# smolGura/fish-tts

Measured on AMD Instinct MI355X. Metric: semantic tokens/sec, higher is better.
Workload: dtype bf16; 1 GPU; openaudio-s1-mini shapes (BASELINE configs[1]): batch=1 per GPU, 48-token prompt, 215 frames (10 s), top-p sampling, hipGraph-captured frame step, + DAC codec decode; prompt_len=48, parallelism=replica x1, frame_engine=3

## Files before the change

### fish-tts_amd/csrc/engine.hip

```cpp
#include "engine.h"
#include "ar_kernels.h"
#include "frame_engine.h"
#include "wide_kernels.h"
#include "gemm_kernels.h"
#include "codec_kernels.h"
#include "stage_kernels.h"

#include <math.h>

#include <algorithm>
#include <mutex>
#include <stdarg.h>
#include <stdio.h>
#include <stdlib.h>
#include <string.h>

using namespace ft;

static std::string g_create_err;
static void eng_release(ft_ctx* ctx);

ft_status ft_fail(ft_ctx* ctx, ft_status code, const std::string& msg) {
    if (ctx) ctx->err = msg; else g_create_err = msg;
    return code;
// ... 134 lines not shown
    FT_TRY(dmalloc(ctx, &ctx->part_o, M * c.n_head * ctx->nsplit_max * c.head_dim));
    FT_TRY(dmalloc(ctx, &ctx->part_ml, M * c.n_head * ctx->nsplit_max * 2));
    ctx->cache_m_stride = (size_t)c.n_local_heads * ctx->n_slots * c.head_dim;
    ctx->fcache_m_stride = (size_t)c.fast_n_local_heads * c.num_codebooks * c.fast_head_dim;
    ctx->layers.resize(c.n_layer);
    ctx->flayers.resize(c.n_fast_layer);
    for (auto& l : ctx->layers) {
        FT_TRY(dmalloc(ctx, (char**)&l.kc, M * ctx->cache_m_stride * ctx->esz));
        FT_TRY(dmalloc(ctx, (char**)&l.vc, M * ctx->cache_m_stride * ctx->esz));
    }
    for (auto& l : ctx->flayers) {
        FT_TRY(dmalloc(ctx, (char**)&l.kc, M * ctx->fcache_m_stride * ctx->esz));
        FT_TRY(dmalloc(ctx, (char**)&l.vc, M * ctx->fcache_m_stride * ctx->esz));
    }
    const size_t R = c.num_codebooks + 1;
    FT_TRY(dmalloc(ctx, &ctx->d_pos, M));
    FT_TRY(dmalloc(ctx, &ctx->d_tok, M * R));
    FT_TRY(dmalloc(ctx, &ctx->d_tokn, M * R));
    FT_TRY(dmalloc(ctx, &ctx->d_seq, M * R * ctx->cap));
    FT_TRY(dmalloc(ctx, &ctx->d_nf, M));
    FT_TRY(dmalloc(ctx, &ctx->d_done, M));
    FT_TRY(dmalloc(ctx, &ctx->d_prompt, R * (size_t)c.max_seq_len));
    FT_TRY(dmalloc(ctx, &ctx->d_ctl, M));
    ctx->prefill_gemm_mode = getenv("FT_PREFILL_GEMM") ? atoi(getenv("FT_PREFILL_GEMM")) : 2;
    ctx->prefill_v0 = getenv("FT_PREFILL_V0") != nullptr || c.dtype != FT_BF16 || c.dim % 32 || (c.n_head * c.head_dim) % 32 ||
                      c.intermediate_size % 32;
    if (!ctx->prefill_v0) {
        const size_t S = c.max_seq_len;
        FT_TRY(dmalloc(ctx, &ctx->pf_x, S * c.dim));
        FT_TRY(dmalloc(ctx, &ctx->pf_qkv, S * qkvN));
        FT_TRY(dmalloc(ctx, &ctx->pf_y, S * c.n_head * c.head_dim));
        FT_TRY(dmalloc(ctx, &ctx->pf_xn, S * c.dim));
        FT_TRY(dmalloc(ctx, &ctx->pf_ybf, S * c.n_head * c.head_dim));
        FT_TRY(dmalloc(ctx, &ctx->pf_g, S * c.intermediate_size));
        FT_TRY(dmalloc(ctx, &ctx->pf_qbf, S * c.n_head * c.head_dim));
        FT_TRY(dmalloc(ctx, &ctx->pf_seqs, M));
        FT_TRY(dmalloc(ctx, &ctx->pf_rows, S));
    }
    if (c.dtype == FT_F16 || !ctx->prefill_v0) {
        const int HD = c.n_head * c.head_dim, HDf = c.fast_n_head * c.fast_head_dim;
        ctx->wide_ok = !getenv("FT_NO_WIDE") && !c.fast_attention_qkv_bias && !c.fast_attention_o_bias && c.fast_dim == c.dim &&
                       wide_k_ok(c.dim) && wide_k_ok(HD) && wide_k_ok(c.intermediate_size) && wide_k_ok(HDf) && wide_k_ok(c.fast_intermediate_size) &&
                       qkvN % 32 == 0 && fqkvN % 32 == 0 && c.intermediate_size % 16 == 0 && c.fast_intermediate_size % 16 == 0 &&
                       c.dim % 16 == 0 && c.vocab_size % 32 == 0 && ctx->fastV % 16 == 0;
        if (ctx->wide_ok) {
            ctx->xo_pair = (int)((M + 15) / 16 * 16);
            ctx->no_pair = getenv("FT_NO_PAIR") != nullptr;
            ctx->no_attn_wide = getenv("FT_NO_ATTN_WIDE") != nullptr;
            ctx->no_head_stream = getenv("FT_NO_HEAD_STREAM") != nullptr;
            ctx->xo_ldm = 2 * ctx->xo_pair;
            const size_t P = ctx->xo_ldm;
            FT_TRY(dmalloc(ctx, &ctx->xo_x, P * c.dim));
            FT_TRY(dmalloc(ctx, &ctx->xo_xf, P * c.fast_dim));
            FT_TRY(dmalloc(ctx, &ctx->xo_femb, P * c.fast_dim));
            FT_TRY(dmalloc(ctx, &ctx->xo_y, P * (size_t)std::max(HD, HDf)));
            FT_TRY(dmalloc(ctx, &ctx->xo_g, P * (size_t)std::max(c.intermediate_size, c.fast_intermediate_size)));
        }
    }
    const size_t nchunk = ((size_t)c.vocab_size + 1023) / 1024;
    FT_TRY(dmalloc(ctx, &ctx->samp_cut, M));
    FT_TRY(dmalloc(ctx, &ctx->samp_chunk_cnt, M * nchunk));
    FT_TRY(dmalloc(ctx, &ctx->samp_part_score, M * nchunk));
    FT_TRY(dmalloc(ctx, &ctx->samp_part_idx, M * nchunk));
    FT_HIP(ctx, hipHostMalloc((void**)&ctx->h_pin, (3 * M + 8) * sizeof(int), hipHostMallocDefault));
    return FT_OK;
}

extern "C" ft_status ft_create(const ft_ar_config* ar, const ft_codec_config* codec, int32_t device, ft_ctx** out) {
    if (!out || (!ar && !codec)) return ft_fail(nullptr, FT_ERR_ARG, "ft_create: need a config and an out pointer");
    int ndev = 0;
    if (hipGetDeviceCount(&ndev) != hipSuccess || ndev == 0)
        return ft_fail(nullptr, FT_ERR_HIP, "ft_create: no HIP device visible (the MI355X path has no CPU fallback)");
    if (device < 0 || device >= ndev) return ft_fail(nullptr, FT_ERR_ARG, "ft_create: bad device index");
    ft_ctx* ctx = new ft_ctx();
    ctx->device = device;
    ft_status st = FT_OK;
    do {
        if (hipSetDevice(device) != hipSuccess) { st = ft_fail(ctx, FT_ERR_HIP, "hipSetDevice failed"); break; }
        if (hipStreamCreateWithFlags(&ctx->stream, hipStreamNonBlocking) != hipSuccess) {
            st = ft_fail(ctx, FT_ERR_HIP, "hipStreamCreate failed"); break;
        }
        if (ar) {
            ctx->c = *ar;
            ctx->has_ar = true;
            if ((st = ar_validate(ctx)) != FT_OK) break;
            if ((st = ar_alloc(ctx)) != FT_OK) break;
            ar_expected(ctx);
        }
        if (codec) {
            ctx->cc = *codec;
            ctx->has_codec = true;
            if ((st = codec_create(ctx)) != FT_OK) break;
            codec_expected(ctx);
        }
    } while (0);
    if (st != FT_OK) {
        g_create_err = ctx->err;
        ft_destroy(ctx);
        return st;
    }
    *out = ctx;
    return FT_OK;
}

extern "C" void ft_destroy(ft_ctx* ctx) {
    if (!ctx) return;
    hipSetDevice(ctx->device);
    if (ctx->stream) hipStreamSynchronize(ctx->stream);
    for (auto& kv : ctx->graphs) hipGraphExecDestroy(kv.second);
    for (auto& kv : ctx->expected) if (kv.second.p) hipFree(kv.second.p);
    for (auto& l : ctx->layers) { hipFree(l.kc); hipFree(l.vc); if (l.w13) hipFree(l.w13); }
    for (auto& l : ctx->flayers) { hipFree(l.kc); hipFree(l.vc); if (l.w13) hipFree(l.w13); }
    float* bufs[] = {ctx->x, ctx->qkv, ctx->y, ctx->g, ctx->logits, ctx->femb, ctx->xf, ctx->qkvf, ctx->gf,
                     ctx->flog, ctx->part_o, ctx->part_ml, ctx->noise};
    for (float* b : bufs) if (b) hipFree(b);
    if (ctx->hid && ctx->hid != ctx->x) hipFree(ctx->hid);
    int* ibufs[] = {ctx->d_pos, ctx->d_tok, ctx->d_tokn, ctx->d_seq, ctx->d_nf, ctx->d_done, ctx->d_prompt};
    for (int* b : ibufs) if (b) hipFree(b);
    if (ctx->d_ctl) hipFree(ctx->d_ctl);
    if (ctx->wide_qkv0_tab) hipFree(ctx->wide_qkv0_tab);
    { void* pf[] = {ctx->pf_x, ctx->pf_qkv, ctx->pf_y, ctx->pf_xn, ctx->pf_ybf, ctx->pf_g, ctx->xo_x, ctx->xo_xf, ctx->xo_femb, ctx->xo_y, ctx->xo_g, ctx->pf_qbf}; for (void* q : pf) if (q) hipFree(q); }
    for (auto& l : ctx->layers) { if (l.bqkv_f32) hipFree(l.bqkv_f32); if (l.bo_f32) hipFree(l.bo_f32); }
    if (ctx->samp_cut) hipFree(ctx->samp_cut);
    if (ctx->samp_chunk_cnt) hipFree(ctx->samp_chunk_cnt);
    if (ctx->samp_part_score) hipFree(ctx->samp_part_score);
    if (ctx->samp_part_idx) hipFree(ctx->samp_part_idx);
    eng_release(ctx);
    if (ctx->h_pin) hipHostFree(ctx->h_pin);
    for (auto e : ctx->prof_ev) hipEventDestroy(e);
    codec_destroy(ctx);
    if (ctx->stream) hipStreamDestroy(ctx->stream);
    delete ctx;
}

extern "C" const char* ft_last_error(const ft_ctx* ctx) { return ctx ? ctx->err.c_str() : g_create_err.c_str(); }

extern "C" ft_status ft_sync(ft_ctx* ctx) {
    if (!ctx) return FT_ERR_ARG;
    FT_HIP(ctx, hipSetDevice(ctx->device));
    FT_HIP(ctx, hipStreamSynchronize(ctx->stream));
    return FT_OK;
}

extern "C" ft_status ft_load_weight(ft_ctx* ctx, const char* name, const void* src, int32_t src_dtype,
                                    const int64_t* shape, int32_t ndim) {
    if (!ctx || !name || !src || !shape) return ft_fail(ctx, FT_ERR_ARG, "ft_load_weight: null argument");
    if (ctx->finalized) return ft_fail(ctx, FT_ERR_STATE, "ft_load_weight: weights already finalized");
    auto it = ctx->expected.find(name);
    if (it == ctx->expected.end()) return ft_fail(ctx, FT_ERR_ARG, std::string("unknown weight name: ") + name);
    FtTensor& t = it->second;
    if ((int)t.shape.size() != ndim) return ft_fail(ctx, FT_ERR_ARG, std::string("rank mismatch for ") + name);
    for (int i = 0; i < ndim; ++i)
        if (t.shape[i] != shape[i]) {
            char buf[256];
            snprintf(buf, sizeof buf, "shape mismatch for %s: dim %d is %lld, expected %lld", name, i,
                     (long long)shape[i], (long long)t.shape[i]);
            return ft_fail(ctx, FT_ERR_ARG, buf);
        }
    if (src_dtype != FT_F32 && src_dtype != FT_BF16 && src_dtype != FT_F16)
        return ft_fail(ctx, FT_ERR_ARG, "src_dtype must be FT_F32, FT_BF16 or FT_F16");
    FT_HIP(ctx, hipSetDevice(ctx->device));
    const int64_t n = t.numel();
    const size_t ssz = src_dtype == FT_F32 ? 4 : 2, dsz = t.dtype == FT_F32 ? 4 : 2;
    if (!t.p) FT_HIP(ctx, hipMalloc(&t.p, (size_t)n * dsz + 64));
    if (src_dtype == t.dtype) {
        FT_HIP(ctx, hipMemcpy(t.p, src, (size_t)n * dsz, hipMemcpyDefault));
        return FT_OK;
    }
    void* stage = nullptr;
    FT_HIP(ctx, hipMalloc(&stage, (size_t)n * ssz));
    hipError_t e = hipMemcpy(stage, src, (size_t)n * ssz, hipMemcpyDefault);
    if (e == hipSuccess) {
        const int blocks = (int)((n + 255) / 256 < 4096 ? (n + 255) / 256 : 4096);
        auto to = [&](auto* sp) {
            if (t.dtype == FT_F32) convert_kernel<<<blocks, 256, 0, ctx->stream>>>(sp, (float*)t.p, n);
            else if (t.dtype == FT_BF16) convert_kernel<<<blocks, 256, 0, ctx->stream>>>(sp, (bf16_t*)t.p, n);
            else convert_kernel<<<blocks, 256, 0, ctx->stream>>>(sp, (f16_t*)t.p, n);
        };
        if (src_dtype == FT_F32) to((const float*)stage);
        else if (src_dtype == FT_BF16) to((const bf16_t*)stage);
        else to((const f16_t*)stage);
        e = hipStreamSynchronize(ctx->stream);
    }
    hipFree(stage);
    if (e != hipSuccess) return ft_fail(ctx, FT_ERR_HIP, std::string("ft_load_weight copy: ") + hipGetErrorString(e));
    return FT_OK;
}

static void* wp(ft_ctx* ctx, const std::string& n) {
    auto it = ctx->expected.find(n);
    return it == ctx->expected.end() ? nullptr : it->second.p;
}

static ft_status eng_setup(ft_ctx* ctx);
static ft_status wide_qkv0_build(ft_ctx* ctx);

static ft_status ar_finalize(ft_ctx* ctx) {
    const ft_ar_config& c = ctx->c;
    ctx->emb = wp(ctx, "embeddings.weight");
    ctx->cb_emb = wp(ctx, "codebook_embeddings.weight");
    ctx->norm = wp(ctx, "norm.weight");
    ctx->head = c.tie_word_embeddings ? ctx->emb : wp(ctx, "output.weight");
    ctx->fproj_w = wp(ctx, "fast_project_in.weight");
    ctx->fproj_b = wp(ctx, "fast_project_in.bias");
    ctx->fast_emb = wp(ctx, "fast_embeddings.weight");
    ctx->fast_norm = wp(ctx, "fast_norm.weight");
    ctx->fast_out = wp(ctx, "fast_output.weight");
    ctx->rope = (float*)wp(ctx, "rope.slow");
    ctx->frope = (float*)wp(ctx, "rope.fast");
    auto fill = [&](std::vector<FtLayer>& ls, const char* pre, int ffn, int dim) -> ft_status {
        for (size_t i = 0; i < ls.size(); ++i) {
            const std::string p = std::string(pre) + std::to_string(i);
            FtLayer& l = ls[i];
            l.attn_norm = wp(ctx, p + ".attention_norm.weight");
            l.wqkv = wp(ctx, p + ".attention.wqkv.weight");
            l.bqkv = wp(ctx, p + ".attention.wqkv.bias");
            l.qn = wp(ctx, p + ".attention.q_norm.weight");
            l.kn = wp(ctx, p + ".attention.k_norm.weight");
            l.wo = wp(ctx, p + ".attention.wo.weight");
            l.bo = wp(ctx, p + ".attention.wo.bias");
            l.ffn_norm = wp(ctx, p + ".ffn_norm.weight");
            l.w2 = wp(ctx, p + ".feed_forward.w2.weight");
            FtTensor& w1 = ctx->expected[p + ".feed_forward.w1.weight"];
            FtTensor& w3 = ctx->expected[p + ".feed_forward.w3.weight"];
            FT_HIP(ctx, hipMalloc(&l.w13, (size_t)2 * ffn * dim * ctx->esz));
            const int64_t n = (int64_t)ffn * dim;
            const int blocks = (int)((n + 255) / 256 < 4096 ? (n + 255) / 256 : 4096);
            if (ctx->esz == 2)
                interleave_rows_kernel<bf16_t><<<blocks, 256, 0, ctx->stream>>>((bf16_t*)w1.p, (bf16_t*)w3.p, (bf16_t*)l.w13, ffn, dim);
            else
                interleave_rows_kernel<float><<<blocks, 256, 0, ctx->stream>>>((float*)w1.p, (float*)w3.p, (float*)l.w13, ffn, dim);
            FT_HIP(ctx, hipStreamSynchronize(ctx->stream));
            hipFree(w1.p); w1.p = nullptr;
            hipFree(w3.p); w3.p = nullptr;
        }
        return FT_OK;
    };
    FT_TRY(fill(ctx->layers, "layers.", c.intermediate_size, c.dim));
    if (!ctx->prefill_v0 || ctx->wide_ok) {
        const int qkvN = (c.n_head + 2 * c.n_local_heads) * c.head_dim;
        auto to_f32 = [&](const void* b, float* o, int n) {
            if (c.dtype == FT_F16) convert_kernel<f16_t, float><<<(n + 255) / 256, 256, 0, ctx->stream>>>((const f16_t*)b, o, n);
            else convert_kernel<bf16_t, float><<<(n + 255) / 256, 256, 0, ctx->stream>>>((const bf16_t*)b, o, n);
        };
        for (auto& l : ctx->layers) {
            if (l.bqkv) {
                FT_HIP(ctx, hipMalloc((void**)&l.bqkv_f32, qkvN * sizeof(float)));
                to_f32(l.bqkv, l.bqkv_f32, qkvN);
            }
            if (l.bo) {
                FT_HIP(ctx, hipMalloc((void**)&l.bo_f32, c.dim * sizeof(float)));
                to_f32(l.bo, l.bo_f32, c.dim);
            }
        }
        FT_HIP(ctx, hipStreamSynchronize(ctx->stream));
    }
    FT_TRY(fill(ctx->flayers, "fast_layers.", c.fast_intermediate_size, c.fast_dim));
    FT_TRY(eng_setup(ctx));
    FT_TRY(wide_qkv0_build(ctx));
    return FT_OK;
}

constexpr int ENG_MAX_STRIKES = 2;
static std::mutex g_eng_mu;
static std::map<int, ft_ctx*> g_eng_owner;

static void eng_release(ft_ctx* ctx) {
    void* eb[] = {ctx->eng_layers, ctx->eng_flayers, ctx->eng_gx ,
                  ctx->eng_gpart, ctx->eng_fast_g, ctx->eng_ctl, ctx->eng_qkv0_tab};
    for (void* q : eb) if (q) hipFree(q);
    ctx->eng_layers = ctx->eng_flayers = nullptr;
    ctx->eng_gx = ctx->eng_gqkv = ctx->eng_gy = ctx->eng_gxb = ctx->eng_gg = ctx->eng_fast_g = ctx->eng_ctl = nullptr;
    ctx->eng_gpart = nullptr;
    ctx->eng_qkv0_tab = nullptr;
    ctx->eng_on = ctx->eng_fast_on = false;
    if (ctx->eng_owner) {
        std::lock_guard<std::mutex> lk(g_eng_mu);
        auto it = g_eng_owner.find(ctx->device);
        if (it != g_eng_owner.end() && it->second == ctx) g_eng_owner.erase(it);
        ctx->eng_owner = false;
    }
}

static bool eng_fits_cu(const void* fn, size_t lds, size_t lds_cap, const char* name, std::string& why) {
    hipFuncAttributes fa{};
    const hipError_t fe = hipFuncGetAttributes(&fa, fn);
    if (fe != hipSuccess) { (void)hipGetLastError(); why = std::string("hipFuncGetAttributes: ") + hipGetErrorString(fe); return false; }
    const int regs = std::max(fa.numRegs, 1), per_simd = 512 / (((regs + 7) / 8) * 8);
    const bool fits = per_simd * 4 >= ENG_THREADS / 64 && lds + fa.sharedSizeBytes <= lds_cap && fa.maxThreadsPerBlock >= ENG_THREADS;
    if (getenv("FT_LOG")) {
        int occ = -1;
        const hipError_t oe = hipOccupancyMaxActiveBlocksPerMultiprocessor(&occ, fn, ENG_THREADS, lds);
        if (oe != hipSuccess) (void)hipGetLastError();
        fprintf(stderr, "fish_tts_amd: %s engine kernel: %d registers (%d waves per SIMD), %zu B of LDS of %zu: %s (the occupancy query says %d)\n",
                name, fa.numRegs, per_simd, lds + fa.sharedSizeBytes, lds_cap, fits ? "fits a CU" : "does not fit a CU", occ);
    }
    if (!fits) why = std::string("a ") + name + " workgroup does not fit one CU (registers / LDS)";
    return fits;
}

typedef void (*eng_slow_fn_t)(SlowEngP);
typedef void (*eng_fast_fn_t)(FastEngP);
typedef void (*eng_qkv0_fn_t)(const bf16_t*, const bf16_t*, const bf16_t*, const bf16_t*, bf16_t*, int, int, int, float);
struct EngSlowEntry { int D, H, HKV, HDIM, F, SQ, SF, SO; eng_slow_fn_t xl, plain; };
struct EngFastEntry { int D, H, HKV, HDIM, F, V, SQ, SF, SO; eng_fast_fn_t loop; eng_qkv0_fn_t qkv0; eng_fast_fn_t resident; int resf, resl; };
template <typename S, bool WITH_XL>
static EngSlowEntry eng_slow_entry() {
    eng_slow_fn_t xl = nullptr;
    if constexpr (WITH_XL) xl = slow_engine_kernel<S, true>;
    return EngSlowEntry{S::D, S::H, S::HKV, S::HDIM, S::F, S::SQ, S::SF, S::SO, xl, slow_engine_kernel<S, false>};
}
template <typename S>
static EngFastEntry eng_fast_entry() {
    eng_fast_fn_t res = nullptr;
    if constexpr (S::RESF > 0) res = fast_engine_kernel<S, 10, true>;
    return EngFastEntry{S::D, S::H, S::HKV, S::HDIM, S::F, S::V, S::SQ, S::SF, S::SO, fast_engine_kernel<S, 10, false>, eng_qkv0_table_kernel<S>,
                        res, S::RESF, S::RESL};
}
static const EngSlowEntry* eng_slow_shapes(int* n) {
    static const EngSlowEntry tab[] = {eng_slow_entry<EngSlowS1, true>(), eng_slow_entry<EngSlowShape<1024, 16, 8, 128, 4096>, true>(),
                                       eng_slow_entry<EngSlowShape<1024, 16, 4, 128, 3072>, false>()};
    *n = (int)(sizeof tab / sizeof tab[0]);
    return tab;
}
static const EngFastEntry* eng_fast_shapes(int* n) {
    static const EngFastEntry tab[] = {eng_fast_entry<EngFastS1>(), eng_fast_entry<EngFastShape<1024, 16, 8, 64, 4096, 1024>>()};
    *n = (int)(sizeof tab / sizeof tab[0]);
    return tab;
}

static bool eng_setup_try(ft_ctx* ctx, std::string& why) {
    const ft_ar_config& c = ctx->c;
    auto hip_ok = [&](hipError_t e, const char* what) {
        if (e == hipSuccess) return true;
        why = std::string(what) + ": " + hipGetErrorString(e);
        (void)hipGetLastError();
        return false;
    };
    if (getenv("FT_NO_ENGINE")) { why = "FT_NO_ENGINE is set"; return false; }
    if (c.dtype != FT_BF16) { why = "precision is not bf16"; return false; }
    hipDeviceProp_t prop;
    if (!hip_ok(hipGetDeviceProperties(&prop, ctx->device), "hipGetDeviceProperties")) return false;
    const int nb = prop.multiProcessorCount;
    const int HD = c.n_head * c.head_dim;
    const int qkvN = (c.n_head + 2 * c.n_local_heads) * c.head_dim;
    auto per = [&](int units) { return (units + nb - 1) / nb; };
    const EngSlowEntry* se = nullptr;
    {
        int n = 0;
        const EngSlowEntry* tab = eng_slow_shapes(&n);
        for (int i = 0; i < n && !se; ++i)
            if (c.dim == tab[i].D && c.n_head == tab[i].H && c.n_local_heads == tab[i].HKV && c.head_dim == tab[i].HDIM && c.intermediate_size == tab[i].F)
                se = &tab[i];
    }
    const bool shape_ok = se && c.fast_dim == c.dim && c.n_layer >= 1 && c.n_layer < ENG_EPOCH_STEP &&
                          per(qkvN) <= se->SQ * ENG_CW && per(c.dim) <= se->SO * ENG_CW && per(c.intermediate_size) <= se->SF * ENG_CW &&
                          qkvN % (4 * nb) == 0 && c.dim % (4 * nb) == 0 && c.intermediate_size % (4 * nb) == 0 && per(qkvN) <= ENG_LINE &&
                          per(c.intermediate_size) <= ENG_LINE && c.n_local_heads * ctx->nsplit_max <= nb && c.head_dim % (4 * ctx->nsplit_max) == 0 && nb == ENG_NB;
    if (!shape_ok) {
        char buf[320];
        snprintf(buf, sizeof buf, "widths outside the engine's instantiations (dim %d, heads %d / %d x %d, ffn %d, fast_dim %d on %d CUs; "
                 "built for dim 1024, 16 heads x 128 with 8 kv heads and ffn 3072 or 4096, or 4 kv heads and ffn 3072, on 256 CUs)", c.dim, c.n_head,
                 c.n_local_heads, c.head_dim, c.intermediate_size, c.fast_dim, nb);
        why = buf;
        return false;
    }
    {
        std::lock_guard<std::mutex> lk(g_eng_mu);
        auto it = g_eng_owner.find(ctx->device);
        if (it != g_eng_owner.end() && it->second != ctx) {
            why = "another context of this process already runs the frame engine on this device (its workgroups need every CU)";
            return false;
        }
        g_eng_owner[ctx->device] = ctx;
        ctx->eng_owner = true;
    }
    ctx->eng_nb = nb;
    std::vector<EngLayer> h(c.n_layer);
    for (int i = 0; i < c.n_layer; ++i) {
        const FtLayer& l = ctx->layers[i];
        h[i] = EngLayer{(const bf16_t*)l.wqkv, (const bf16_t*)l.bqkv, (const bf16_t*)l.attn_norm, (const bf16_t*)l.qn,
                        (const bf16_t*)l.kn, (const bf16_t*)l.wo, (const bf16_t*)l.bo, (const bf16_t*)l.ffn_norm,
                        (const bf16_t*)l.w13, (const bf16_t*)l.w2, (bf16_t*)l.kc, (bf16_t*)l.vc};
    }
    if (!hip_ok(hipMalloc((void**)&ctx->eng_layers, h.size() * sizeof(EngLayer)), "hipMalloc(engine layer table)")) return false;
    if (!hip_ok(hipMemcpy(ctx->eng_layers, h.data(), h.size() * sizeof(EngLayer), hipMemcpyHostToDevice), "hipMemcpy(engine layer table)")) return false;
    auto zalloc = [&](void** q, size_t bytes, const char* what) {
        return hip_ok(hipMalloc(q, bytes), what) && hip_ok(hipMemset(*q, 0, bytes), what);
    };
    const size_t L = c.n_layer;
    const size_t VB = (size_t)nb * ENG_LINE * 4;
    const size_t pool_words = ((L + 1) * VB + 3 * L * VB + L * HD * 4) / 4;
    ctx->eng_relay = getenv("FT_NO_RELAY") == nullptr;
    ctx->eng_pool_bytes = pool_words * 4 * (ctx->eng_relay ? 9 : 1);
    if (!zalloc((void**)&ctx->eng_gx, ctx->eng_pool_bytes, "hipMalloc(engine hand-off pool)")) return false;
    ctx->eng_pool_words = pool_words;
    ctx->eng_gxb = ctx->eng_gx + (L + 1) * (VB / 4);
    ctx->eng_gg = ctx->eng_gxb + L * (VB / 4);
    ctx->eng_gy = ctx->eng_gg + L * (VB / 4);
    ctx->eng_gqkv = ctx->eng_gy + L * HD;
    ctx->eng_gpart_bytes = L * c.n_head * ctx->nsplit_max * (size_t)(c.head_dim + 2) * 8;
    if (!zalloc((void**)&ctx->eng_gpart, ctx->eng_gpart_bytes, "hipMalloc(engine split partials)")) return false;
    if (!zalloc((void**)&ctx->eng_ctl, ENG_CTL_WORDS * 4, "hipMalloc(engine control words)")) return false;
    const int G = c.n_head / c.n_local_heads, hd = c.head_dim, NSLOT = 4 * (64 / (hd >> 3));
    size_t fl = (size_t)c.dim * 2 + HD + c.intermediate_size + (size_t)(G + 2) * hd + (size_t)G * hd + 2 * hd +
                (size_t)NSLOT * G * 2 + (size_t)NSLOT * G * hd + 64 * 6 + ENG_MAX_OUT + 8;
    ctx->eng_lds_slow = std::max(fl * sizeof(float), (size_t)82 * 1024);
    const size_t lds_cap = prop.maxSharedMemoryPerMultiProcessor;
    if (ctx->eng_lds_slow > lds_cap) { why = "the slow stack's LDS need exceeds the CU's"; return false; }
    ctx->eng_xl = ctx->xl_shape && nb == 256 && ctx->nsplit_max == 32 && c.n_local_heads * 32 == nb;
    ctx->eng_xl = ctx->eng_xl && se->xl != nullptr;
    ctx->eng_slow_fn = (const void*)(ctx->eng_xl ? se->xl : se->plain);
    const void* slow_fn = ctx->eng_slow_fn;
    if (!hip_ok(hipFuncSetAttribute(slow_fn, hipFuncAttributeMaxDynamicSharedMemorySize, (int)ctx->eng_lds_slow),
                "hipFuncSetAttribute(slow_engine_kernel)")) return false;
    if (!eng_fits_cu(slow_fn, ctx->eng_lds_slow, lds_cap, "slow-stack", why)) return false;
    ctx->eng_on = true;
    why = ctx->eng_xl ? "slow stack on the frame engine (one kv head per XCD)" : "slow stack on the frame engine";

    const int HDf = c.fast_n_head * c.fast_head_dim;
    const int fqkvN = (c.fast_n_head + 2 * c.fast_n_local_heads) * c.fast_head_dim;
    const EngFastEntry* fe = nullptr;
    {
        int n = 0;
        const EngFastEntry* tab = eng_fast_shapes(&n);
        for (int i = 0; i < n && !fe; ++i)
            if (c.fast_dim == tab[i].D && c.fast_n_head == tab[i].H && c.fast_n_local_heads == tab[i].HKV && c.fast_head_dim == tab[i].HDIM &&
                c.fast_intermediate_size == tab[i].F && ctx->fastV == tab[i].V)
                fe = &tab[i];
    }
    const bool fast_ok = !getenv("FT_NO_FAST_ENGINE") && fe && HDf == c.fast_dim && c.n_fast_layer >= 1 &&
                         c.num_codebooks >= 2 && c.num_codebooks <= 10 && fqkvN % (4 * nb) == 0 && ctx->fastV % (4 * nb) == 0 &&
                         per(fqkvN) <= fe->SQ * ENG_CW && per(c.fast_dim) <= fe->SO * ENG_CW && per(c.fast_intermediate_size) <= fe->SF * ENG_CW &&
                         per(ctx->fastV) <= fe->SO * ENG_CW && per(fqkvN) <= ENG_LINE && per(c.fast_intermediate_size) <= ENG_LINE && ctx->fastV <= 1024 &&
                         c.codebook_size <= 65536;
    if (!fast_ok) { why += "; fast loop on launches (FT_NO_FAST_ENGINE, or fast widths outside the instantiations: 1024 / 16 + 8 heads x 64 / ffn 3072 or 4096 / 1024 codes used, <= 10 codebooks)"; return true; }
    const bool fast_res = fe->resident != nullptr && c.n_fast_layer <= fe->resl && getenv("FT_NO_RESIDENT") == nullptr;
    ctx->eng_fast_fn = (const void*)(fast_res ? fe->resident : fe->loop);
    auto fast_off = [&](const std::string& w2) { why += "; fast loop on launches (" + w2 + ")"; return true; };
    std::vector<EngLayer> hf(c.n_fast_layer);
    for (int i = 0; i < c.n_fast_layer; ++i) {
        const FtLayer& l = ctx->flayers[i];
        hf[i] = EngLayer{(const bf16_t*)l.wqkv, (const bf16_t*)l.bqkv, (const bf16_t*)l.attn_norm, (const bf16_t*)l.qn,
                         (const bf16_t*)l.kn, (const bf16_t*)l.wo, (const bf16_t*)l.bo, (const bf16_t*)l.ffn_norm,
                         (const bf16_t*)l.w13, (const bf16_t*)l.w2, nullptr, nullptr};
    }
    std::string w2;
    auto hip_ok2 = [&](hipError_t e, const char* what) {
        if (e == hipSuccess) return true;
        w2 = std::string(what) + ": " + hipGetErrorString(e);
        (void)hipGetLastError();
        return false;
    };
    if (!hip_ok2(hipMalloc((void**)&ctx->eng_flayers, hf.size() * sizeof(EngLayer)), "hipMalloc(fast layer table)")) return fast_off(w2);
    if (!hip_ok2(hipMemcpy(ctx->eng_flayers, hf.data(), hf.size() * sizeof(EngLayer), hipMemcpyHostToDevice), "hipMemcpy(fast layer table)")) return fast_off(w2);
    const size_t nLf = c.n_fast_layer;
    ctx->eng_fast_words = (2 * ((nLf + 1) + 3 * nLf + 1)) * (VB / 4) + (size_t)c.num_codebooks * ENG_LINE;
    ctx->eng_fast_bytes = ctx->eng_fast_words * 4 * (ctx->eng_relay ? 9 : 1);
    if (!hip_ok2(hipMalloc((void**)&ctx->eng_fast_g, ctx->eng_fast_bytes), "hipMalloc(fast hand-off pool)") ||
        !hip_ok2(hipMemset(ctx->eng_fast_g, 0, ctx->eng_fast_bytes), "hipMemset(fast hand-off pool)")) return fast_off(w2);
    const int kvw = c.fast_n_local_heads * c.fast_head_dim;
    ctx->eng_pair = getenv("FT_NO_PAIR") == nullptr &&
                    eng_fast_lds_bytes(c.fast_dim, fqkvN, HDf, c.fast_intermediate_size, ctx->fastV, (int)nLf, c.num_codebooks, kvw, true) <= lds_cap;
    ctx->eng_lds_fast = eng_fast_lds_bytes(c.fast_dim, fqkvN, HDf, c.fast_intermediate_size, ctx->fastV, (int)nLf, c.num_codebooks, kvw, ctx->eng_pair);
    if (ctx->eng_lds_fast > lds_cap) return fast_off("the codebook loop's LDS need exceeds the CU's");
    ctx->eng_lds_fast = std::max(ctx->eng_lds_fast, (size_t)82 * 1024);
    if (!hip_ok2(hipFuncSetAttribute(ctx->eng_fast_fn, hipFuncAttributeMaxDynamicSharedMemorySize,
                                     (int)ctx->eng_lds_fast), "hipFuncSetAttribute(fast_engine_kernel)")) return fast_off(w2);
    if (!eng_fits_cu(ctx->eng_fast_fn, ctx->eng_lds_fast, lds_cap, "codebook-loop", w2)) return fast_off(w2);
    if (getenv("FT_NO_QKV0") == nullptr && c.num_codebooks > 2) {
        const size_t tb = (size_t)ctx->fastV * fqkvN * sizeof(bf16_t);
        if (!hip_ok2(hipMalloc((void**)&ctx->eng_qkv0_tab, tb), "hipMalloc(layer-0 q k v table)")) return fast_off(w2);
        const FtLayer& l0 = ctx->flayers[0];
        const size_t lds = ((size_t)c.fast_dim + ENG_MAX_OUT) * sizeof(float);
        fe->qkv0<<<dim3(fqkvN / (fe->SQ * ENG_CW), 16), ENG_CW * 64, lds, ctx->stream>>>(
            (const bf16_t*)l0.wqkv, (const bf16_t*)l0.bqkv, (const bf16_t*)l0.attn_norm, (const bf16_t*)ctx->fast_emb,
            (bf16_t*)ctx->eng_qkv0_tab, c.fast_dim, fqkvN, ctx->fastV, c.norm_eps);
        if (!hip_ok2(hipGetLastError(), "eng_qkv0_table_kernel") || !hip_ok2(hipStreamSynchronize(ctx->stream), "eng_qkv0_table_kernel")) {
            hipFree(ctx->eng_qkv0_tab); ctx->eng_qkv0_tab = nullptr;
            return fast_off(w2);
        }
    }
    ctx->eng_fast_on = true;
    why = ctx->eng_xl ? "slow stack (one kv head per XCD) and codebook loop on the frame engine" : "slow stack and codebook loop on the frame engine";
    {
        char buf[160];
        if (fast_res)
            snprintf(buf, sizeof buf, "; codebook loop: %d of %d W13 pairs per CU of %d layers resident in the gathering waves' registers",
                     fe->resf * ENG_GW, per(c.fast_intermediate_size), c.n_fast_layer);
        else
            snprintf(buf, sizeof buf, "; codebook loop: all weights streamed (%s)", fe->resident == nullptr ? "no resident set fits this shape class" :
                     c.n_fast_layer > fe->resl ? "more layers than the resident set holds" : "FT_NO_RESIDENT is set");
        why += buf;
    }
    return true;
}

static ft_status eng_setup(ft_ctx* ctx) {
    ctx->eng_on = ctx->eng_fast_on = false;
    std::string why;
    if (!eng_setup_try(ctx, why)) {
        eng_release(ctx);
        ctx->eng_why = "launch path: " + why;
    } else {
        char buf[64];
        snprintf(buf, sizeof buf, " (%d workgroups)", ctx->eng_nb);
        ctx->eng_why = why + buf;
    }
    if (getenv("FT_LOG")) fprintf(stderr, "fish_tts_amd: batch-1 decode frames: %s\n", ctx->eng_why.c_str());
    return FT_OK;
}

extern "C" ft_status ft_finalize_weights(ft_ctx* ctx) {
    if (!ctx) return FT_ERR_ARG;
    if (ctx->finalized) return FT_OK;
    FT_HIP(ctx, hipSetDevice(ctx->device));
    for (auto& kv : ctx->expected)
        if (!kv.second.p) return ft_fail(ctx, FT_ERR_MISSING_WEIGHT, "missing weight: " + kv.first);
    if (ctx->has_ar) FT_TRY(ar_finalize(ctx));
    if (ctx->has_codec) FT_TRY(codec_finalize(ctx));
    ctx->finalized = true;
    return FT_OK;
}

struct Launch {
    ft_ctx* ctx;
    hipStream_t s;
    int m0, M;
    int pos_off;
    hipError_t err = hipSuccess;
    bool gemv_only = false;
    bool tail_only = false;
    void chk() { hipError_t e = hipGetLastError(); if (e != hipSuccess && err == hipSuccess) err = e; }
};

template <typename W, int R> struct DType { typedef W WT; static constexpr int ROUND = R; };
template <typename F>
static auto by_dtype(const ft_ctx* ctx, F&& f) {
    if (ctx->c.dtype == FT_BF16) return f(DType<bf16_t, RND_BF16>{});
    if (ctx->c.dtype == FT_F16) return f(DType<f16_t, RND_F16>{});
    return f(DType<float, RND_NONE>{});
}

enum { TB_X = 0, TB_QKV, TB_Y, TB_G, TB_LOGITS, TB_HID, TB_FEMB, TB_XF, TB_QKVF, TB_GF, TB_FLOG, TB_PART_O, TB_PART_ML,
       TB_PF_X = 13, TB_PF_QKV, TB_PF_Y,
       TB_XO_X = 20, TB_XO_XF, TB_XO_FEMB, TB_XO_Y, TB_XO_G,
       TB_PF_XN = 25, TB_PF_YBF, TB_PF_QBF, TB_PF_G,
       TB_TOKN = 30, TB_TOK, TB_POS, TB_NF, TB_DONE, TB_SEQ, TB_CUT, TB_CHUNK_CNT, TB_PART_IDX,
       TB_PROMPT = 39, TB_PF_SEQS, TB_PF_ROWS };
static const void* tr_buf(const ft_ctx* ctx, int id, int* esz, int* rows, int* cols) {
    const ft_ar_config& c = ctx->c;
    const int MB = c.max_batch, R = c.num_codebooks + 1, ldm = ctx->xo_ldm;
    const int qkvN = (c.n_head + 2 * c.n_local_heads) * c.head_dim, fqkvN = (c.fast_n_head + 2 * c.fast_n_local_heads) * c.fast_head_dim;
    const int HD = c.n_head * c.head_dim, HDf = c.fast_n_head * c.fast_head_dim, nchunk = (c.vocab_size + 1023) / 1024;
    *esz = 4;
    auto f = [&](const void* p, int r, int k) { *rows = r; *cols = k; return p; };
    auto o = [&](const void* p, int width) { *esz = 2; *rows = width / 8; *cols = ldm * 8; return p; };
    switch (id) {
        case TB_X: return f(ctx->x, MB, c.dim);
        case TB_QKV: return f(ctx->qkv, MB, qkvN);
        case TB_Y: return f(ctx->y, MB, ctx->y_ld);
        case TB_G: return f(ctx->g, MB, c.intermediate_size);
        case TB_LOGITS: return f(ctx->logits, MB, c.vocab_size);
        case TB_HID: return f(ctx->hid, MB, c.fast_dim);
        case TB_FEMB: return f(ctx->femb, MB, c.fast_dim);
        case TB_XF: return f(ctx->xf, MB, c.fast_dim);
        case TB_QKVF: return f(ctx->qkvf, 2 * ((MB + 15) / 16 * 16), fqkvN);
        case TB_GF: return f(ctx->gf, MB, c.fast_intermediate_size);
        case TB_FLOG: return f(ctx->flog, MB, ctx->fastV);
        case TB_PART_O: return f(ctx->part_o, 1, MB * c.n_head * ctx->nsplit_max * c.head_dim);
        case TB_PART_ML: return f(ctx->part_ml, 1, MB * c.n_head * ctx->nsplit_max * 2);
        case TB_XO_X: return o(ctx->xo_x, c.dim);
        case TB_XO_XF: return o(ctx->xo_xf, c.fast_dim);
        case TB_XO_FEMB: return o(ctx->xo_femb, c.fast_dim);
        case TB_XO_Y: return o(ctx->xo_y, std::max(HD, HDf));
        case TB_XO_G: return o(ctx->xo_g, std::max(c.intermediate_size, c.fast_intermediate_size));
        case TB_TOKN: return f(ctx->d_tokn, MB, R);
        case TB_TOK: return f(ctx->d_tok, MB, R);
        case TB_POS: return f(ctx->d_pos, 1, MB);
        case TB_NF: return f(ctx->d_nf, 1, MB);
        case TB_DONE: return f(ctx->d_done, 1, MB);
        case TB_SEQ: return f(ctx->d_seq, MB, R * ctx->cap);
        case TB_CUT: return f(ctx->samp_cut, MB, (int)(sizeof(SampCut) / 4));
        case TB_CHUNK_CNT: return f(ctx->samp_chunk_cnt, 1, MB * nchunk);
        case TB_PART_IDX: return f(ctx->samp_part_idx, 1, MB * nchunk);
        case TB_PF_X: return f(ctx->pf_x, c.max_seq_len, c.dim);
        case TB_PF_QKV: return f(ctx->pf_qkv, c.max_seq_len, qkvN);
        case TB_PF_Y: return f(ctx->pf_y, c.max_seq_len, HD);
        case TB_PF_XN: *esz = 2; return f(ctx->pf_xn, c.max_seq_len, c.dim);
        case TB_PF_YBF: *esz = 2; return f(ctx->pf_ybf, c.max_seq_len, HD);
        case TB_PF_QBF: *esz = 2; return f(ctx->pf_qbf, c.max_seq_len, HD);
        case TB_PF_G: *esz = 2; return f(ctx->pf_g, c.max_seq_len, c.intermediate_size);
        case TB_PROMPT: return f(ctx->d_prompt, 1, R * c.max_seq_len);
        case TB_PF_SEQS: return f(ctx->pf_seqs, MB, 4);
        case TB_PF_ROWS: return f(ctx->pf_rows, c.max_seq_len, 2);
    }
    return nullptr;
}
struct TrCls { int a = -1, b = -1, c = -1, d = -1; };
static void tr_rec(Launch& L, const std::string& name, int rows, int cols, TrCls cls, std::initializer_list<int> bufs) {
    ft_ctx* ctx = L.ctx;
    ArTrace& t = *ctx->trace;
    const int idx = (int)t.recs.size();
    t.recs.emplace_back();
    ArTraceRec& r = t.recs.back();
    r.name = t.pass_prefix + (name == "embed" || name.compare(0, 5, "slow.") == 0 ? t.pos_prefix : std::string()) + name;
    r.m0 = L.m0; r.rows = rows; r.cols = cols; r.pos_off = L.pos_off;
    r.cls[0] = cls.a; r.cls[1] = cls.b; r.cls[2] = cls.c; r.cls[3] = cls.d;
    r.held = idx >= t.first && idx < t.first + t.count;
    std::vector<int> ids(bufs);
    ids.insert(ids.end(), t.uploaded.begin(), t.uploaded.end());
    t.uploaded.clear();
    for (int id : ids) {
        ArTraceBuf b;
        const void* p = tr_buf(ctx, id, &b.esz, &b.rows, &b.cols);
        if (!p) continue;
        b.id = id;
        if (r.held) {
            b.data.resize((size_t)b.rows * b.cols * b.esz);
            if (hipMemcpyAsync(b.data.data(), p, b.data.size(), hipMemcpyDeviceToHost, L.s) != hipSuccess) t.failed = true;
        }
        r.bufs.push_back(std::move(b));
    }
    if (r.held && hipStreamSynchronize(L.s) != hipSuccess) t.failed = true;
}
static std::string tr_name(const char* fmt, ...) {
    char buf[64];
    va_list ap;
    va_start(ap, fmt);
    vsnprintf(buf, sizeof buf, fmt, ap);
    va_end(ap);
    return buf;
}
struct TrName {
    const char* stack; int n; const char* op;
    std::string str() const { return stack ? tr_name("%s.%d.%s", stack, n, op) : std::string(op); }
};
struct RowBuf { float* p; int id; };
struct XoBuf { bf16_t* p; int id; };
static void tr_state(ft_ctx* ctx, int which) {
    ArTrace& t = *ctx->trace;
    ArTraceState& s = t.st[which];
    const size_t MB = ctx->c.max_batch, R = ctx->c.num_codebooks + 1;
    s.tok.resize(MB * R); s.pos.resize(MB); s.nf.resize(MB); s.done.resize(MB); s.seq.resize(MB * R * ctx->cap);
    bool ok = hipStreamSynchronize(ctx->stream) == hipSuccess;
    ok = ok && hipMemcpy(s.tok.data(), ctx->d_tok, s.tok.size() * 4, hipMemcpyDeviceToHost) == hipSuccess;
    ok = ok && hipMemcpy(s.pos.data(), ctx->d_pos, MB * 4, hipMemcpyDeviceToHost) == hipSuccess;
    ok = ok && hipMemcpy(s.nf.data(), ctx->d_nf, MB * 4, hipMemcpyDeviceToHost) == hipSuccess;
    ok = ok && hipMemcpy(s.done.data(), ctx->d_done, MB * 4, hipMemcpyDeviceToHost) == hipSuccess;
    ok = ok && hipMemcpy(s.seq.data(), ctx->d_seq, s.seq.size() * 4, hipMemcpyDeviceToHost) == hipSuccess;
    if (which == 0) {
        static const int ids[] = {TB_X, TB_QKV, TB_Y, TB_G, TB_LOGITS, TB_HID, TB_FEMB, TB_XF, TB_QKVF, TB_GF, TB_FLOG, TB_PART_O, TB_PART_ML,
                                  TB_XO_X, TB_XO_XF, TB_XO_FEMB, TB_XO_Y, TB_XO_G, TB_TOKN, TB_TOK, TB_POS, TB_NF, TB_DONE, TB_SEQ, TB_CUT,
                                  TB_CHUNK_CNT, TB_PART_IDX};
        static const int pf_ids[] = {TB_PF_X, TB_PF_QKV, TB_PF_Y, TB_PF_XN, TB_PF_YBF, TB_PF_QBF, TB_PF_G, TB_PROMPT, TB_PF_SEQS, TB_PF_ROWS};
        std::vector<int> all(std::begin(ids), std::end(ids));
        if (t.kind >= 3) all.insert(all.end(), std::begin(pf_ids), std::end(pf_ids));
        t.begin.clear();
        for (int id : all) {
            ArTraceBuf b;
            const void* p = tr_buf(ctx, id, &b.esz, &b.rows, &b.cols);
            if (!p) continue;
            b.id = id;
            b.data.resize((size_t)b.rows * b.cols * b.esz);
            ok = ok && hipMemcpy(b.data.data(), p, b.data.size(), hipMemcpyDeviceToHost) == hipSuccess;
            t.begin.push_back(std::move(b));
        }
    }
    if (!ok) t.failed = true;
}
struct ArTraceScope {
    ft_ctx* ctx;
    bool own = false;
    ArTraceScope(ft_ctx* c, bool eligible, int kind, int m0, int M) : ctx(c) {
        ArTrace& t = ctx->tstore;
        if (ctx->trace || !t.armed) return;
        t.armed = false;
        if (!eligible) return;
        t.recs.clear(); t.uploaded.clear(); t.pass_prefix.clear(); t.pos_prefix.clear();
        t.failed = false; t.kind = kind; t.m0 = m0; t.M = M;
        ctx->trace = &t;
        own = true;
    }
    ~ArTraceScope() { if (own) ctx->trace = nullptr; }
};
static void tr_uploaded(ft_ctx* ctx, std::initializer_list<int> ids) { if (ctx->trace) ctx->trace->uploaded.assign(ids); }
static void tr_pos(ft_ctx* ctx, int t) { if (ctx->trace) ctx->trace->pos_prefix = tr_name("t%d.", t); }

struct PfX {
    const void* gain = nullptr;
    const float* ss_in = nullptr;
    int nblk = 0;
    float* ss_out = nullptr;
};
enum { PF_ID_NONE = -1, PF_ID_SKINNY1 = 0, PF_ID_SKINNY2 = 1, PF_ID_SKINNY4 = 2, PF_ID_LIN128 = 3, PF_ID_LIN64 = 4, PF_ID_TAP64_128 = 5,
       PF_ID_TAP64_64 = 6, PF_ID_TAP_128 = 7, PF_ID_TAP_64 = 8 };
static int pf_gemm(Launch& L, const bf16_t* X, long ldx, int S, const void* W, const float* bias, int N, int K,
                   int act, const float* resid, float* out_f32, bf16_t* out_bf, long ldo, int round_out,
                   const PfX& fx = PfX());
static bool wide_batch(const Launch& L) {
    return L.ctx->wide_ok && L.M >= L.ctx->wide_min && L.M <= 64 && !L.gemv_only && !L.ctx->prof;
}

static bool wide_pair(const Launch& L) {
    const ft_ctx* ctx = L.ctx;
    return wide_batch(L) && !ctx->no_pair && ctx->c.num_codebooks >= 2 && ctx->c.n_fast_layer > 0 && ctx->xo_pair + L.M <= 64;
}

enum { WIDE_ID_S11 = 0, WIDE_ID_S12 = 1, WIDE_ID_S22 = 2, WIDE_ID_G12 = 3, WIDE_ID_G22 = 4, WIDE_ID_R11 = 5, WIDE_ID_HEAD = 6 };
template <typename WT>
static int wide_gemm(Launch& L, const bf16_t* X, const void* W, const float* bias, int N, int K, const void* gain, int epi,
                      float* out_f32, long ldo, bf16_t* out_xo, const bf16_t* resid_xo, int rows = 0, bool vocab_head = false) {
    const int M = rows > 0 ? rows : L.M;
    WidePT<WT> p{};
    p.X = (const WT*)X; p.ldm = L.ctx->xo_ldm; p.W = (const WT*)W; p.ldw = K; p.gain = (const WT*)gain; p.eps = L.ctx->c.norm_eps;
    p.bias = bias; p.M = M; p.N = N; p.K = K; p.out_f32 = out_f32; p.ldo = ldo; p.out_xo = (WT*)out_xo; p.ldm_o = L.ctx->xo_ldm;
    p.resid_xo = (const WT*)resid_xo;
    bool ok;
    int id;
    if (epi == WEPI_RESID) { id = WIDE_ID_R11; ok = wide_gemm_launch<1, 1, false, WEPI_RESID>(p, L.s); }
    else if (epi == WEPI_SWIGLU) {
        id = M > 16 ? WIDE_ID_G22 : WIDE_ID_G12;
        ok = M > 16 ? wide_gemm_launch<2, 2, true, WEPI_SWIGLU>(p, L.s) : wide_gemm_launch<1, 2, true, WEPI_SWIGLU>(p, L.s);
    }
    else if (vocab_head && M <= 32 && K == 1024 && N % 16 == 0 && N >= 4096 && !L.ctx->no_head_stream) {
        static DevOnce once;
        once.run([] { hipFuncSetAttribute((const void*)wide_head_kernel<1024, WT>, hipFuncAttributeMaxDynamicSharedMemorySize, (int)wide_head_lds<1024>()); });
        wide_head_kernel<1024, WT><<<256, 512, wide_head_lds<1024>(), L.s>>>(p);
        id = WIDE_ID_HEAD;
        ok = true;
    }
    else if (N >= 32768) {
        id = M > 16 ? WIDE_ID_S22 : WIDE_ID_S12;
        ok = M > 16 ? wide_gemm_launch<2, 2, true, WEPI_STORE>(p, L.s) : wide_gemm_launch<1, 2, true, WEPI_STORE>(p, L.s);
    }
    else if (N >= 4096 && M > 16) { id = WIDE_ID_S12; ok = wide_gemm_launch<1, 2, true, WEPI_STORE>(p, L.s); }
    else { id = WIDE_ID_S11; ok = wide_gemm_launch<1, 1, true, WEPI_STORE>(p, L.s); }
    if (!ok && L.err == hipSuccess) L.err = hipErrorInvalidValue;
    L.chk();
    return id;
}
template <typename WT>
static void wide_linear(Launch& L, const TrName& nm, const bf16_t* X, const void* W, const float* bias, const void* gain, int N, int K,
                        int epi, RowBuf out_f32, long ldo, XoBuf out_xo, const bf16_t* resid_xo, int rows = 0, bool vocab_head = false) {
    const int id = wide_gemm<WT>(L, X, W, bias, N, K, gain, epi, out_f32.p, ldo, out_xo.p, resid_xo, rows, vocab_head);
    if (L.ctx->trace) tr_rec(L, nm.str(), rows > 0 ? rows : L.M, epi == WEPI_SWIGLU ? N / 2 : N, TrCls{id}, {out_xo.p ? out_xo.id : out_f32.id});
}

template <typename WT>
static __global__ __launch_bounds__(256) void xo_from_rows_kernel(const float* x, int ldx, int D, bf16_t* xo, int ldm) {
    const int m = blockIdx.y;
    for (int d = blockIdx.x * 256 + threadIdx.x; d < D; d += gridDim.x * 256) xo[xo_index(m, d, ldm)] = h16_bits<WT>(x[(size_t)m * ldx + d]);
}

static __global__ __launch_bounds__(256) void xo_from_h16_rows_kernel(const bf16_t* x, int D, bf16_t* xo, int ldm, int rows) {
    const int m = blockIdx.y;
    if (m >= rows) return;
    for (int d = blockIdx.x * 256 + threadIdx.x; d < D; d += gridDim.x * 256) xo[xo_index(m, d, ldm)] = x[(size_t)m * D + d];
}
template <typename WT>
static __global__ void f32_to_h16_kernel(const float* x, bf16_t* o, long n) {
    for (long i = (long)blockIdx.x * blockDim.x + threadIdx.x; i < n; i += (long)gridDim.x * blockDim.x) o[i] = h16_bits<WT>(x[i]);
}

template <typename WT>
static ft_status wide_qkv0_build_t(ft_ctx* ctx) {
    const ft_ar_config& c = ctx->c;
    if (!ctx->wide_ok || getenv("FT_NO_QKV0") || c.num_codebooks <= 2 || c.n_fast_layer < 1) return FT_OK;
    const int Df = c.fast_dim, qkvN = (c.fast_n_head + 2 * c.fast_n_local_heads) * c.fast_head_dim, V = ctx->fastV;
    const FtLayer& l0 = ctx->flayers[0];
    if (l0.bqkv) return FT_OK;
    constexpr int CH = 64;
    bf16_t* xo = nullptr; float* out = nullptr;
    if (hipMalloc((void**)&xo, (size_t)Df * CH * sizeof(bf16_t)) != hipSuccess || hipMalloc((void**)&out, (size_t)CH * qkvN * sizeof(float)) != hipSuccess ||
        hipMalloc((void**)&ctx->wide_qkv0_tab, (size_t)V * qkvN * sizeof(bf16_t)) != hipSuccess) {
        (void)hipGetLastError();
        if (xo) hipFree(xo);
        if (out) hipFree(out);
        if (ctx->wide_qkv0_tab) { hipFree(ctx->wide_qkv0_tab); ctx->wide_qkv0_tab = nullptr; }
        return FT_OK;
    }
    bool ok = true;
    for (int c0 = 0; c0 < V && ok; c0 += CH) {
        const int rows = std::min(CH, V - c0);
        xo_from_h16_rows_kernel<<<dim3((Df + 255) / 256, rows), 256, 0, ctx->stream>>>((const bf16_t*)ctx->fast_emb + (size_t)c0 * Df, Df, xo, CH, rows);
        WidePT<WT> p{};
        p.X = (const WT*)xo; p.ldm = CH; p.W = (const WT*)l0.wqkv; p.ldw = Df; p.gain = (const WT*)l0.attn_norm; p.eps = c.norm_eps;
// ... 2444 lines not shown
```

### fish-tts_amd/csrc/frame_engine.h

```cpp
#pragma once
#include "ar_kernels.h"

namespace ft {

constexpr int ENG_NB = 256;
constexpr int ENG_WAVES = 8;
constexpr int ENG_THREADS = ENG_WAVES * 64;
constexpr int ENG_CW = 4;
constexpr int ENG_GW = 4;

template <int D_, int H_, int HKV_, int HDIM_, int F_>
struct EngSlowShape {
    static constexpr int D = D_, H = H_, HKV = HKV_, HDIM = HDIM_, F = F_;
    static constexpr int HD = H * HDIM, QKVN = (H + 2 * HKV) * HDIM, G = H / HKV;
    static constexpr int NTD = D / 512, NTA = HD / 512, NTF = F / 512;
    static constexpr int SQ = (QKVN / ENG_NB + ENG_CW - 1) / ENG_CW, SF = (F / ENG_NB + ENG_CW - 1) / ENG_CW, SO = (D / ENG_NB + ENG_CW - 1) / ENG_CW;
    static constexpr bool PK3 = F % 384 == 0 && (F / ENG_NB) % 3 == 0;
    static_assert(D % 512 == 0 && HD % 512 == 0 && F % 512 == 0, "weight rows are read as whole 16-byte pieces by 64 lanes");
    static_assert(QKVN % (4 * ENG_NB) == 0 && D % (4 * ENG_NB) == 0 && F % (4 * ENG_NB) == 0, "whole 16-byte granule groups per workgroup");
    static_assert(H % HKV == 0 && HDIM % 8 == 0 && HDIM <= 128, "grouped-query attention, 16-byte K/V pieces");
};
template <int D_, int H_, int HKV_, int HDIM_, int F_, int V_>
struct EngFastShape {
    static constexpr int D = D_, H = H_, HKV = HKV_, HDIM = HDIM_, F = F_, V = V_;
// ... 35 lines not shown
    bf16_t *kc, *vc;
};

__device__ __forceinline__ void eng_barrier() {
    __builtin_amdgcn_fence(__ATOMIC_RELEASE, "workgroup", "local");
    __builtin_amdgcn_s_barrier();
    __builtin_amdgcn_fence(__ATOMIC_ACQUIRE, "workgroup", "local");
}

typedef const __attribute__((address_space(1))) U4* eng_gU4;
template <bool NT> __device__ __forceinline__ U4 eng_ldg16(const void* p) {
    if constexpr (NT) return __builtin_nontemporal_load((eng_gU4)p);
    else return *(eng_gU4)p;
}
__device__ __forceinline__ float eng_ldg_bf16(const bf16_t* p, size_t i) {
    return bf16_bits_to_f32(((const __attribute__((address_space(1))) bf16_t*)p)[i]);
}
typedef const __attribute__((address_space(4))) unsigned long long* eng_c64;
__device__ __forceinline__ EngLayer eng_layer(const EngLayer* table, int i) {
    static_assert(sizeof(EngLayer) == 12 * sizeof(unsigned long long), "EngLayer is twelve pointers");
    eng_c64 q = (eng_c64)(unsigned long long)(table + i);
    EngLayer l;
    l.wqkv = (const bf16_t*)q[0]; l.bqkv = (const bf16_t*)q[1]; l.attn_norm = (const bf16_t*)q[2]; l.qn = (const bf16_t*)q[3];
    l.kn = (const bf16_t*)q[4]; l.wo = (const bf16_t*)q[5]; l.bo = (const bf16_t*)q[6]; l.ffn_norm = (const bf16_t*)q[7];
    l.w13 = (const bf16_t*)q[8]; l.w2 = (const bf16_t*)q[9]; l.kc = (bf16_t*)q[10]; l.vc = (bf16_t*)q[11];
    return l;
}

__device__ __forceinline__ unsigned eng_tag16(unsigned e) { return (e & 0x7fffu) | 0x8000u; }
__device__ __forceinline__ unsigned eng_tag32(unsigned e) { return e | 0x80000000u; }
__device__ __forceinline__ unsigned long long eng_rt() { return __builtin_amdgcn_s_memrealtime(); }

__device__ __forceinline__ void eng_put(unsigned* g, int i, float v, unsigned tag16) {
    __hip_atomic_store((eng_gu32*)(g + i), (tag16 << 16) | (__float_as_uint(v) >> 16), ENG_RLX);
}
__device__ __forceinline__ void eng_put_raw(unsigned* g, int i, unsigned v16, unsigned tag16) {
    __hip_atomic_store((eng_gu32*)(g + i), (tag16 << 16) | (v16 & 0xffffu), ENG_RLX);
}
__device__ __forceinline__ void eng_put4(unsigned* g, float v0, float v1, float v2, float v3, unsigned tag16) {
    U4 w;
    w.x = (tag16 << 16) | (__float_as_uint(v0) >> 16); w.y = (tag16 << 16) | (__float_as_uint(v1) >> 16);
    w.z = (tag16 << 16) | (__float_as_uint(v2) >> 16); w.w = (tag16 << 16) | (__float_as_uint(v3) >> 16);
    asm volatile("global_store_dwordx4 %0, %1, off sc1" :: "v"(g), "v"(w) : "memory");
}
__device__ __forceinline__ void eng_put64(unsigned long long* g, size_t i, float v, unsigned tag32) {
    __hip_atomic_store((eng_gu64*)(g + i), ((unsigned long long)tag32 << 32) | __float_as_uint(v), ENG_RLX);
}

template <int FL = 0>
__device__ __forceinline__ void eng_ld3_sc1(const void* p0, const void* p1, const void* p2, U4& a, U4& b, U4& c) {
    asm volatile("global_load_dwordx4 %0, %3, off sc1\n\tglobal_load_dwordx4 %1, %4, off sc1\n\t"
                 "global_load_dwordx4 %2, %5, off sc1\n\ts_waitcnt vmcnt(0)"
                 : "=&v"(a), "=&v"(b), "=&v"(c) : "v"(p0), "v"(p1), "v"(p2) : "memory");
}
template <int FL = 0>
__device__ __forceinline__ void eng_ld1_sc1(const void* p0, U4& a) {
    asm volatile("global_load_dwordx4 %0, %1, off sc1\n\ts_waitcnt vmcnt(0)" : "=&v"(a) : "v"(p0) : "memory");
}

__device__ __forceinline__ bool eng_tags_ok(const U4& v, unsigned tag) {
    return (v.x >> 16) == tag && (v.y >> 16) == tag && (v.z >> 16) == tag && (v.w >> 16) == tag;
}
__device__ __forceinline__ void eng_unpack_to_lds(float* dst, const U4& v) {
    float4 f;
    f.x = __uint_as_float(v.x << 16); f.y = __uint_as_float(v.y << 16);
    f.z = __uint_as_float(v.z << 16); f.w = __uint_as_float(v.w << 16);
    *reinterpret_cast<float4*>(dst) = f;
}

struct EngSpin {
    unsigned* ctl;
    int* dead;
    unsigned spins = 0;
    unsigned long long t0 = 0;
    int where;
    __device__ __forceinline__ bool give_up(int lane) {
        if ((++spins & 255u) != 0u) return false;
        const unsigned long long t = eng_rt();
        if (t0 == 0) t0 = t;
        if (t - t0 > ENG_TIMEOUT_TICKS || __hip_atomic_load((eng_gu32*)(ctl + ENG_CTL_ABORT), ENG_RLX)) {
            if (lane == 0) {
                if (!__hip_atomic_load((eng_gu32*)(ctl + ENG_CTL_ABORT), ENG_RLX))
                    __hip_atomic_store((eng_gu32*)(ctl + ENG_CTL_WHERE), (unsigned)where, ENG_RLX);
                __hip_atomic_store((eng_gu32*)(ctl + ENG_CTL_ABORT), 1u, ENG_RLX);
                *dead = 1;
            }
            return true;
        }
        return false;
    }
};

constexpr int ENG_LINE = 32;
__device__ __forceinline__ size_t eng_pub(int b, int u_lo) { (void)b; return (size_t)u_lo; }
struct EngLayout {
    int per;
    __device__ __forceinline__ int off(int u) const { return u; }
};
struct EngIdent { __device__ __forceinline__ int operator()(int i) const { return i; } };

template <typename DMap = EngIdent, int FL = 0>
__device__ __forceinline__ void eng_gather(const unsigned* g, EngLayout lay, int u0, int n, unsigned tag, float* dst, int gw, int ngw,
                                           int lane, unsigned* ctl, int* dead, int where, DMap dmap = DMap(),
                                           unsigned long long* dbg = nullptr) {
    const int npiece = (n + 255) >> 8;
    EngSpin sp{ctl, dead, 0, 0, where};
    unsigned long long n_full = 0, t_first = 0;
    for (int p0 = gw; p0 < npiece; p0 += 3 * ngw) {
        const int c0 = p0;
        const int c1 = p0 + ngw < npiece ? p0 + ngw : c0;
        const int c2 = p0 + 2 * ngw < npiece ? p0 + 2 * ngw : c0;
        const int i0 = c0 * 256 + lane * 4 < n ? c0 * 256 + lane * 4 : c0 * 256;
        const int i1 = c1 * 256 + lane * 4 < n ? c1 * 256 + lane * 4 : c1 * 256;
        const int i2 = c2 * 256 + lane * 4 < n ? c2 * 256 + lane * 4 : c2 * 256;
        const int o0 = lay.off(u0 + i0), o1 = lay.off(u0 + i1), o2 = lay.off(u0 + i2);
        U4 a, b, c;
        for (;;) {
            if (c1 == c0) { eng_ld1_sc1<FL>(g + o0, a); b = a; c = a; }
            else eng_ld3_sc1<FL>(g + o0, g + o1, g + o2, a, b, c);
            const bool oa = eng_tags_ok(a, tag), ob = eng_tags_ok(b, tag), oc = eng_tags_ok(c, tag);
            if (dbg && n_full == 0) t_first = eng_rt();
            ++n_full;
            if (__all(oa && ob && oc)) break;
            if (sp.give_up(lane)) return;
        }
        if (c0 * 256 + lane * 4 < n) eng_unpack_to_lds(dst + dmap(i0), a);
        if (c1 != c0 && c1 * 256 + lane * 4 < n) eng_unpack_to_lds(dst + dmap(i1), b);
        if (c2 != c0 && c2 * 256 + lane * 4 < n) eng_unpack_to_lds(dst + dmap(i2), c);
    }
    if (dbg && lane == 0) { dbg[0] = t_first; dbg[1] = n_full; dbg[2] = 0; }
}

struct EngRelay {
    int on;
    int rank, nr;
    long delta;
};

__device__ __forceinline__ void eng_register(unsigned* ctl, int nb, int* r, int* dead) {
    const int xcd = (int)(__builtin_amdgcn_s_getreg(20 | (0 << 6) | (3 << 11)) & 7u);
    const unsigned rank = atomicAdd(ctl + ENG_CTL_XCD + xcd, 1u);
    atomicAdd(ctl + ENG_CTL_ARRIVED, 1u);
    EngSpin sp{ctl, dead, 0, 0, 9999};
    bool ok = true;
    while (__hip_atomic_load((eng_gu32*)(ctl + ENG_CTL_ARRIVED), ENG_RLX) < (unsigned)nb) {
        if (sp.give_up(0)) { ok = false; break; }
        __builtin_amdgcn_s_sleep(2);
    }
    r[0] = xcd; r[1] = (int)rank;
    r[2] = ok ? (int)__hip_atomic_load((eng_gu32*)(ctl + ENG_CTL_XCD + xcd), ENG_RLX) : 1;
}

template <typename DMap = EngIdent>
__device__ __forceinline__ void eng_gather_x(const EngRelay& rl, const unsigned* g, EngLayout lay, int u0, int n, unsigned tag, float* dst,
                                             int gw, int ngw, int lane, unsigned* ctl, int* dead, int where, DMap dmap = DMap(),
                                             unsigned long long* dbg = nullptr) {
    if (!rl.on) { eng_gather(g, lay, u0, n, tag, dst, gw, ngw, lane, ctl, dead, where, dmap, dbg); return; }
    unsigned* rep = const_cast<unsigned*>(g) + rl.delta;
    const int npiece = (n + 255) >> 8;
    for (int p = rl.rank; p < npiece; p += rl.nr) {
        if (p % ngw != gw) continue;
        const int i = p * 256 + lane * 4 < n ? p * 256 + lane * 4 : p * 256;
        const int o = lay.off(u0 + i);
        EngSpin sp{ctl, dead, 0, 0, where};
        U4 a;
        for (;;) {
            eng_ld1_sc1(g + o, a);
            if (__all(eng_tags_ok(a, tag))) break;
            if (sp.give_up(lane)) return;
        }
        if (p * 256 + lane * 4 < n) *reinterpret_cast<U4*>(rep + o) = a;
    }
    eng_gather<DMap, 1>(rep, lay, u0, n, tag, dst, gw, ngw, lane, ctl, dead, where, dmap, dbg);
}

__device__ __forceinline__ bool eng_tags3_ok(const U4& v, unsigned tag) { return (v.y >> 16) == tag && (v.w >> 16) == tag; }
__device__ __forceinline__ void eng_unpack3_to_lds(float* dst, const U4& v) {
    float2 a, b, c;
    a.x = __uint_as_float(v.x << 16); a.y = __uint_as_float(v.x & 0xffff0000u);
    b.x = __uint_as_float(v.y << 16); b.y = __uint_as_float(v.z << 16);
    c.x = __uint_as_float(v.z & 0xffff0000u); c.y = __uint_as_float(v.w << 16);
    reinterpret_cast<float2*>(dst)[0] = a; reinterpret_cast<float2*>(dst)[1] = b; reinterpret_cast<float2*>(dst)[2] = c;
}
template <int FL = 0>
__device__ __forceinline__ void eng_gather3(const unsigned* g, int n, unsigned tag, float* dst, int gw, int ngw, int lane, unsigned* ctl,
                                            int* dead, int where) {
    const int npiece = n / 384;
    EngSpin sp{ctl, dead, 0, 0, where};
    for (int p0 = gw; p0 < npiece; p0 += 3 * ngw) {
        const int c0 = p0;
        const int c1 = p0 + ngw < npiece ? p0 + ngw : c0;
        const int c2 = p0 + 2 * ngw < npiece ? p0 + 2 * ngw : c0;
        const unsigned* a0 = g + c0 * 256 + lane * 4;
        const unsigned* a1 = g + c1 * 256 + lane * 4;
        const unsigned* a2 = g + c2 * 256 + lane * 4;
        U4 a, b, c;
        for (;;) {
            if (c1 == c0) { eng_ld1_sc1<FL>(a0, a); b = a; c = a; }
            else eng_ld3_sc1<FL>(a0, a1, a2, a, b, c);
            if (__all(eng_tags3_ok(a, tag) && eng_tags3_ok(b, tag) && eng_tags3_ok(c, tag))) break;
            if (sp.give_up(lane)) return;
        }
        eng_unpack3_to_lds(dst + c0 * 384 + lane * 6, a);
        if (c1 != c0) eng_unpack3_to_lds(dst + c1 * 384 + lane * 6, b);
        if (c2 != c0) eng_unpack3_to_lds(dst + c2 * 384 + lane * 6, c);
    }
}
__device__ __forceinline__ void eng_gather3_x(const EngRelay& rl, const unsigned* g, int n, unsigned tag, float* dst, int gw, int ngw,
                                              int lane, unsigned* ctl, int* dead, int where) {
    if (!rl.on) { eng_gather3(g, n, tag, dst, gw, ngw, lane, ctl, dead, where); return; }
    unsigned* rep = const_cast<unsigned*>(g) + rl.delta;
    const int npiece = n / 384;
    for (int p = rl.rank; p < npiece; p += rl.nr) {
        if (p % ngw != gw) continue;
        const int o = p * 256 + lane * 4;
        EngSpin sp{ctl, dead, 0, 0, where};
        U4 a;
        for (;;) {
            eng_ld1_sc1(g + o, a);
            if (__all(eng_tags3_ok(a, tag))) break;
            if (sp.give_up(lane)) return;
        }
        *reinterpret_cast<U4*>(rep + o) = a;
    }
    eng_gather3<1>(rep, n, tag, dst, gw, ngw, lane, ctl, dead, where);
}

struct EngSrc2 { const unsigned* g[2]; float* dst[2]; unsigned tag[2]; };
template <int FL = 0>
__device__ __forceinline__ void eng_gather2(const EngSrc2& S, long delta, int n, int gw, int ngw, int lane, unsigned* ctl, int* dead,
                                            int where) {
    const int npiece = n >> 8, NP = 2 * npiece;
    EngSpin sp{ctl, dead, 0, 0, where};
    for (int p0 = gw; p0 < NP; p0 += 3 * ngw) {
        const int c0 = p0;
        const int c1 = p0 + ngw < NP ? p0 + ngw : c0;
        const int c2 = p0 + 2 * ngw < NP ? p0 + 2 * ngw : c0;
        const int s0 = c0 >= npiece, s1 = c1 >= npiece, s2 = c2 >= npiece;
        const int i0 = (c0 - s0 * npiece) * 256 + lane * 4, i1 = (c1 - s1 * npiece) * 256 + lane * 4, i2 = (c2 - s2 * npiece) * 256 + lane * 4;
        const unsigned* a0 = S.g[s0] + delta + i0;
        const unsigned* a1 = S.g[s1] + delta + i1;
        const unsigned* a2 = S.g[s2] + delta + i2;
        const unsigned t0 = S.tag[s0], t1 = S.tag[s1], t2 = S.tag[s2];
        U4 a, b, c;
        for (;;) {
            if (c1 == c0) { eng_ld1_sc1<FL>(a0, a); b = a; c = a; }
            else eng_ld3_sc1<FL>(a0, a1, a2, a, b, c);
            const bool oa = eng_tags_ok(a, t0), ob = c1 == c0 || eng_tags_ok(b, t1), oc = c2 == c0 || eng_tags_ok(c, t2);
            if (__all(oa && ob && oc)) break;
            if (sp.give_up(lane)) return;
        }
        eng_unpack_to_lds(S.dst[s0] + i0, a);
        if (c1 != c0) eng_unpack_to_lds(S.dst[s1] + i1, b);
        if (c2 != c0) eng_unpack_to_lds(S.dst[s2] + i2, c);
    }
}
__device__ __forceinline__ void eng_gather_x2(const EngRelay& rl, const EngSrc2& S, int n, int gw, int ngw, int lane, unsigned* ctl,
                                              int* dead, int where) {
    if (!rl.on) { eng_gather2(S, 0, n, gw, ngw, lane, ctl, dead, where); return; }
    const int npiece = n >> 8, NP = 2 * npiece;
    for (int p = rl.rank; p < NP; p += rl.nr) {
        if (p % ngw != gw) continue;
        const int s = p >= npiece;
        const int i = (p - s * npiece) * 256 + lane * 4;
        const unsigned* src = S.g[s] + i;
        const unsigned tg = S.tag[s];
        EngSpin sp{ctl, dead, 0, 0, where};
        U4 a;
        for (;;) {
            eng_ld1_sc1(src, a);
            if (__all(eng_tags_ok(a, tg))) break;
            if (sp.give_up(lane)) return;
        }
        *reinterpret_cast<U4*>(const_cast<unsigned*>(src) + rl.delta) = a;
    }
    eng_gather2<1>(S, rl.delta, n, gw, ngw, lane, ctl, dead, where);
}

template <int NT, int RPU, int MAXS>
struct EngW {
    U4 w[MAXS][RPU][NT];
    U4 gain[NT];
};

struct EngRowIdent { __device__ __forceinline__ int operator()(int u) const { return u; } };
struct EngRowQkvX {
    int q0, k0, v0, nq, nk;
    __device__ __forceinline__ int operator()(int u) const { return u < nq ? q0 + u : (u < nq + nk ? k0 + (u - nq) : v0 + (u - nq - nk)); }
};

template <int NT, int RPU, int MAXS>
__device__ __forceinline__ void eng_res_pin(EngW<NT, RPU, MAXS>& r) {
#pragma unroll
    for (int s = 0; s < MAXS; ++s)
#pragma unroll
        for (int rr = 0; rr < RPU; ++rr)
#pragma unroll
            for (int t = 0; t < NT; ++t) {
                U4& w = r.w[s][rr][t];
                asm volatile("" : "+v"(w.x), "+v"(w.y), "+v"(w.z), "+v"(w.w));
            }
}

template <bool NTL = true, int NT, int RPU, int MAXS, typename RM = EngRowIdent>
__device__ __forceinline__ void eng_issue(EngW<NT, RPU, MAXS>& r, const bf16_t* W, const bf16_t* gain, int K, int u_lo, int u_hi,
                                          int cw, int lane, int nt, RM rm = RM()) {
#pragma unroll
    for (int s = 0; s < MAXS; ++s) {
        int u = u_lo + cw + s * ENG_CW;
        u = u < u_hi ? u : u_hi - 1;
#pragma unroll
        for (int rr = 0; rr < RPU; ++rr)
#pragma unroll
            for (int t = 0; t < NT; ++t) {
                r.w[s][rr][t] = (nt & 2) ? U4{0u, 0u, 0u, 0u} : eng_ldg16<NTL>(W + (size_t)(rm(u) * RPU + rr) * K + t * 512 + lane * 8);
            }
    }
    if (gain) {
#pragma unroll
        for (int t = 0; t < NT; ++t) r.gain[t] = eng_ldg16<false>(gain + t * 512 + lane * 8);
    }
}

struct EngOut {
    float* vals;
    int* count;
    int seq;
};
constexpr int ENG_MAX_OUT = 64;
typedef __attribute__((address_space(3))) int* eng_lds_int;

template <int NT, int RPU, int MAXS, int PRO, int EPI, typename RM = EngRowIdent>
__device__ __forceinline__ void eng_gemv_rows(const EngW<NT, RPU, MAXS>& r, const float* xs, int K, float eps, const bf16_t* bias,
                                              const float* resid, float* vals, int u_lo, int u_hi, int cw, int lane, RM rm = RM()) {
    static_assert(EPI == EPI_SWIGLU ? RPU == 2 : RPU == 1, "a unit is a (w1, w3) pair for SwiGLU, one row otherwise");
    if (u_lo + cw < u_hi) {
        float xv[NT][8];
#pragma unroll
        for (int t = 0; t < NT; ++t) {
            const float4 f0 = *reinterpret_cast<const float4*>(xs + t * 512 + lane * 8);
            const float4 f1 = *reinterpret_cast<const float4*>(xs + t * 512 + lane * 8 + 4);
            xv[t][0] = f0.x; xv[t][1] = f0.y; xv[t][2] = f0.z; xv[t][3] = f0.w;
            xv[t][4] = f1.x; xv[t][5] = f1.y; xv[t][6] = f1.z; xv[t][7] = f1.w;
        }
        if (PRO == PRO_RMSNORM) {
            float ss = 0.f;
#pragma unroll
            for (int t = 0; t < NT; ++t)
#pragma unroll
                for (int j = 0; j < 8; ++j) ss = fmaf(xv[t][j], xv[t][j], ss);
            ss = wave_sum(ss);
            const float inv = rsqrt_exact(ss / (float)K + eps);
#pragma unroll
            for (int t = 0; t < NT; ++t) {
                float gv[8];
                Vec<bf16_t>::unpack(r.gain[t], gv);
#pragma unroll
                for (int j = 0; j < 8; ++j) xv[t][j] = round_bf16(round_bf16(xv[t][j] * inv) * gv[j]);
            }
        }
#pragma unroll
        for (int s = 0; s < MAXS; ++s) {
            const int u = u_lo + cw + s * ENG_CW;
            if (u >= u_hi) break;
            float acc[RPU];
#pragma unroll
            for (int rr = 0; rr < RPU; ++rr) {
                float a = 0.f;
#pragma unroll
                for (int t = 0; t < NT; ++t) {
                    float wv[8];
                    Vec<bf16_t>::unpack(r.w[s][rr][t], wv);
#pragma unroll
                    for (int j = 0; j < 8; ++j) a = fmaf(wv[j], xv[t][j], a);
                }
                acc[rr] = wave_sum(a);
            }
            float o;
            if (EPI == EPI_SWIGLU) {
                const float a = round_bf16(acc[0]);
                const float b = round_bf16(acc[RPU - 1]);
                const float sg = round_bf16(a / (1.0f + expf(-a)));
                o = round_bf16(sg * b);
            } else {
                float v = acc[0];
                if (bias) v += eng_ldg_bf16(bias, rm(u));
                v = round_bf16(v);
                if (EPI == EPI_RESID) v = round_bf16(resid[rm(u)] + v);
                o = v;
            }
            if (lane == 0) vals[u - u_lo] = o;
        }
    }
}

__device__ __forceinline__ void eng_put_local(unsigned* g, int i, float v, unsigned tag16) {
    __hip_atomic_store((eng_gu32*)(g + i), (tag16 << 16) | (__float_as_uint(v) >> 16), __ATOMIC_RELAXED, __HIP_MEMORY_SCOPE_WORKGROUP);
}
__device__ __forceinline__ void eng_put64_local(unsigned long long* g, size_t i, float v, unsigned tag32) {
    __hip_atomic_store((eng_gu64*)(g + i), ((unsigned long long)tag32 << 32) | __float_as_uint(v), __ATOMIC_RELAXED, __HIP_MEMORY_SCOPE_WORKGROUP);
}

template <int NT, int MAXS, typename RM>
__device__ __forceinline__ void eng_gemv_qkv_local(const EngW<NT, 1, MAXS>& r, const float* xs, int K, float eps, const bf16_t* bias,
                                                   unsigned* gvec, unsigned tag, int n, int cw, int lane, EngOut& eo, RM rm) {
    eng_gemv_rows<NT, 1, MAXS, PRO_RMSNORM, EPI_STORE>(r, xs, K, eps, bias, nullptr, eo.vals, 0, n, cw, lane, rm);
    __builtin_amdgcn_fence(__ATOMIC_RELEASE, "workgroup", "local");
    int old = 0;
    if (lane == 0) old = __hip_atomic_fetch_add((eng_lds_int)eo.count, 1, __ATOMIC_RELAXED, __HIP_MEMORY_SCOPE_WORKGROUP);
    old = __builtin_amdgcn_readfirstlane(old);
    eo.seq += 1;
    if (old + 1 == eo.seq * ENG_CW) {
        __builtin_amdgcn_fence(__ATOMIC_ACQUIRE, "workgroup", "local");
        if (lane < n) eng_put_local(gvec, rm(lane), eo.vals[lane], tag);
    }
}

template <int NT, int RPU, int MAXS, int PRO, int EPI, bool PK3 = false, int ARR = ENG_CW>
__device__ __forceinline__ void eng_gemv_part(const EngW<NT, RPU, MAXS>& r, const float* xs, int K, float eps, const bf16_t* bias,
                                              const float* resid, unsigned* gout, unsigned tag, float* plain, int u_lo, int u_hi,
                                              int r_lo, int r_hi, int cw, int lane, EngOut& eo) {
    eng_gemv_rows<NT, RPU, MAXS, PRO, EPI>(r, xs, K, eps, bias, resid, eo.vals + (r_lo - u_lo), r_lo, r_hi, cw, lane);
    __builtin_amdgcn_fence(__ATOMIC_RELEASE, "workgroup", "local");
    int old = 0;
    if (lane == 0) old = __hip_atomic_fetch_add((eng_lds_int)eo.count, 1, __ATOMIC_RELAXED, __HIP_MEMORY_SCOPE_WORKGROUP);
    old = __builtin_amdgcn_readfirstlane(old);
    eo.seq += 1;
    if (old + 1 == eo.seq * ARR) {
        __builtin_amdgcn_fence(__ATOMIC_ACQUIRE, "workgroup", "local");
        const int n = u_hi - u_lo;
        if constexpr (PK3) {
            if (lane * 3 < n) {
                const unsigned w0 = (__float_as_uint(eo.vals[3 * lane]) >> 16) | (__float_as_uint(eo.vals[3 * lane + 1]) & 0xffff0000u);
                const unsigned w1 = (__float_as_uint(eo.vals[3 * lane + 2]) >> 16) | (tag << 16);
                __hip_atomic_store((eng_gu64*)(reinterpret_cast<unsigned long long*>(gout) + (u_lo / 3 + lane)),
                                   ((unsigned long long)w1 << 32) | w0, ENG_RLX);
            }
        } else if (lane < n) {
            const float o = eo.vals[lane];
            eng_put(gout, lane, o, tag);
            if (plain) plain[u_lo + lane] = o;
        }
    }
}
template <int NT, int RPU, int MAXS, int PRO, int EPI, bool PK3 = false>
__device__ __forceinline__ void eng_gemv(const EngW<NT, RPU, MAXS>& r, const float* xs, int K, float eps, const bf16_t* bias,
                                         const float* resid, unsigned* gout, unsigned tag, float* plain, int u_lo, int u_hi,
                                         int cw, int lane, EngOut& eo) {
    eng_gemv_part<NT, RPU, MAXS, PRO, EPI, PK3, ENG_CW>(r, xs, K, eps, bias, resid, gout, tag, plain, u_lo, u_hi, u_lo, u_hi, cw, lane, eo);
}

template <int NT, int RPU, int MAXS, int PRO, int EPI>
__device__ __forceinline__ void eng_gemv_rows2(const EngW<NT, RPU, MAXS>& r, const float* xs0, const float* xs1, int K, float eps,
                                               const bf16_t* bias, const float* resid0, const float* resid1, float* vals0, float* vals1,
                                               int u_lo, int u_hi, int cw, int lane) {
    static_assert(EPI == EPI_SWIGLU ? RPU == 2 : RPU == 1, "a unit is a (w1, w3) pair for SwiGLU, one row otherwise");
    if (u_lo + cw < u_hi) {
        float xv[2][NT][8];
#pragma unroll
        for (int q = 0; q < 2; ++q) {
            const float* xs = q ? xs1 : xs0;
#pragma unroll
            for (int t = 0; t < NT; ++t) {
                const float4 f0 = *reinterpret_cast<const float4*>(xs + t * 512 + lane * 8);
                const float4 f1 = *reinterpret_cast<const float4*>(xs + t * 512 + lane * 8 + 4);
                xv[q][t][0] = f0.x; xv[q][t][1] = f0.y; xv[q][t][2] = f0.z; xv[q][t][3] = f0.w;
                xv[q][t][4] = f1.x; xv[q][t][5] = f1.y; xv[q][t][6] = f1.z; xv[q][t][7] = f1.w;
            }
        }
        if (PRO == PRO_RMSNORM) {
#pragma unroll
            for (int q = 0; q < 2; ++q) {
                float ss = 0.f;
#pragma unroll
                for (int t = 0; t < NT; ++t)
#pragma unroll
                    for (int j = 0; j < 8; ++j) ss = fmaf(xv[q][t][j], xv[q][t][j], ss);
                ss = wave_sum(ss);
                const float inv = rsqrt_exact(ss / (float)K + eps);
#pragma unroll
                for (int t = 0; t < NT; ++t) {
                    float gv[8];
                    Vec<bf16_t>::unpack(r.gain[t], gv);
#pragma unroll
                    for (int j = 0; j < 8; ++j) xv[q][t][j] = round_bf16(round_bf16(xv[q][t][j] * inv) * gv[j]);
                }
            }
        }
#pragma unroll
        for (int s = 0; s < MAXS; ++s) {
            const int u = u_lo + cw + s * ENG_CW;
            if (u >= u_hi) break;
            float acc[2][RPU];
#pragma unroll
            for (int rr = 0; rr < RPU; ++rr) {
                float a0 = 0.f, a1 = 0.f;
#pragma unroll
                for (int t = 0; t < NT; ++t) {
                    float wv[8];
                    Vec<bf16_t>::unpack(r.w[s][rr][t], wv);
#pragma unroll
                    for (int j = 0; j < 8; ++j) { a0 = fmaf(wv[j], xv[0][t][j], a0); a1 = fmaf(wv[j], xv[1][t][j], a1); }
                }
                acc[0][rr] = wave_sum(a0);
                acc[1][rr] = wave_sum(a1);
            }
#pragma unroll
            for (int q = 0; q < 2; ++q) {
                float o;
                if (EPI == EPI_SWIGLU) {
                    const float a = round_bf16(acc[q][0]);
                    const float bb = round_bf16(acc[q][RPU - 1]);
                    const float sg = round_bf16(a / (1.0f + expf(-a)));
                    o = round_bf16(sg * bb);
                } else {
                    float v = acc[q][0];
                    if (bias) v += eng_ldg_bf16(bias, u);
                    v = round_bf16(v);
                    if (EPI == EPI_RESID) v = round_bf16((q ? resid1 : resid0)[u] + v);
                    o = v;
                }
                if (lane == 0) (q ? vals1 : vals0)[u - u_lo] = o;
            }
        }
    }
}

template <int NT, int RPU, int MAXS, int PRO, int EPI, int ARR = ENG_CW>
__device__ __forceinline__ void eng_gemv2_part(const EngW<NT, RPU, MAXS>& r, const float* xs0, const float* xs1, int K, float eps,
                                               const bf16_t* bias, const float* resid0, const float* resid1, unsigned* gout0, unsigned* gout1,
                                               unsigned tag0, unsigned tag1, int u_lo, int u_hi, int r_lo, int r_hi, int cw, int lane, EngOut& eo) {
    float* const v0 = eo.vals + (r_lo - u_lo);
    if (NT <= 2) {
        eng_gemv_rows2<NT, RPU, MAXS, PRO, EPI>(r, xs0, xs1, K, eps, bias, resid0, resid1, v0, v0 + 32, r_lo, r_hi, cw, lane);
    } else {
        eng_gemv_rows<NT, RPU, MAXS, PRO, EPI>(r, xs0, K, eps, bias, resid0, v0, r_lo, r_hi, cw, lane);
        __builtin_amdgcn_sched_barrier(0);
        eng_gemv_rows<NT, RPU, MAXS, PRO, EPI>(r, xs1, K, eps, bias, resid1, v0 + 32, r_lo, r_hi, cw, lane);
    }
    __builtin_amdgcn_fence(__ATOMIC_RELEASE, "workgroup", "local");
    int old = 0;
    if (lane == 0) old = __hip_atomic_fetch_add((eng_lds_int)eo.count, 1, __ATOMIC_RELAXED, __HIP_MEMORY_SCOPE_WORKGROUP);
    old = __builtin_amdgcn_readfirstlane(old);
    eo.seq += 1;
    if (old + 1 == eo.seq * ARR) {
        __builtin_amdgcn_fence(__ATOMIC_ACQUIRE, "workgroup", "local");
        const int n = u_hi - u_lo;
        const int i = lane & 31;
        if (i < n) {
            const float o = eo.vals[lane];
            eng_put(lane < 32 ? gout0 : gout1, i, o, lane < 32 ? tag0 : tag1);
        }
    }
}
template <int NT, int RPU, int MAXS, int PRO, int EPI>
__device__ __forceinline__ void eng_gemv2(const EngW<NT, RPU, MAXS>& r, const float* xs0, const float* xs1, int K, float eps,
                                          const bf16_t* bias, const float* resid0, const float* resid1, unsigned* gout0, unsigned* gout1,
                                          unsigned tag0, unsigned tag1, int u_lo, int u_hi, int cw, int lane, EngOut& eo) {
    eng_gemv2_part<NT, RPU, MAXS, PRO, EPI, ENG_CW>(r, xs0, xs1, K, eps, bias, resid0, resid1, gout0, gout1, tag0, tag1, u_lo, u_hi, u_lo, u_hi,
                                                    cw, lane, eo);
}

__device__ __forceinline__ void eng_units(int U, int b, int nb, int& lo, int& hi) {
    lo = (int)((long)U * b / nb);
    hi = (int)((long)U * (b + 1) / nb);
}

struct SlowEngP {
    const EngLayer* layers;
    int n_layer;
    int D, H, Hkv, hd, F, qkvN;
    float eps, scale;
    const bf16_t* emb; const bf16_t* cb_emb; const int* toks; long tok_row_stride;
    int ncb, cbsize, vocab, sem_begin, sem_end, scale_cb; float inv_div;
    const float* rope; const int* pos; int pos_off; int n_slots, nsplit;
    size_t cache_off;
    unsigned* gx;
    unsigned* gqkv;
    unsigned long long* gpart;
    unsigned* gy;
    unsigned* gxb;
    unsigned* gg;
    unsigned* ctl;
    long rep_delta0, rep_stride;
    float* x_out;
    int nt;
    unsigned long long* stamps;
};
#define ENG_STAMP(k) do { if (p.stamps && tid == 0) p.stamps[((size_t)b * p.n_layer + li) * 16 + (k)] = eng_rt(); } while (0)
#define ENG_ASTAMP(wv, k) do { if (p.stamps && gw == (wv) && lane == 0) \
    p.stamps[((size_t)nb * p.n_layer + (size_t)b * p.n_layer + li) * 16 + (k)] = eng_rt(); } while (0)

constexpr int ENG_KVST = 6;

__device__ __forceinline__ int eng_att_role(int b, int nb, int li, int natt) {
    int a = b - (int)(((unsigned)li * (unsigned)natt) % (unsigned)nb);
    if (a < 0) a += nb;
    return a < natt ? a : -1;
}

template <typename S, bool XL = false>
__global__ __launch_bounds__(ENG_THREADS) void slow_engine_kernel(SlowEngP p) {
    constexpr int NTD = S::NTD, NTA = S::NTA, NTF = S::NTF, G = S::G;
    constexpr int SQ = S::SQ, SF = S::SF, SO = S::SO;
    extern __shared__ __attribute__((aligned(16))) float smem[];
    const int tid = threadIdx.x, lane = tid & 63, wave = __builtin_amdgcn_readfirstlane(tid >> 6);
    const int b = blockIdx.x;
    constexpr int nb = ENG_NB;
    const int cw = wave;
    const int gw = wave - ENG_CW;
    const int atid = tid - ENG_CW * 64;
    constexpr int D = S::D, F = S::F, hd = S::HDIM, hp = hd >> 1, H = S::H, Hkv = S::HKV, HD = H * hd, QKVN = (H + 2 * Hkv) * hd;
    static_assert(!XL || (ENG_NB % Hkv == 0 && QKVN % ENG_NB == 0), "XCD-local attention: the workgroups of an XCD share one kv head's rows");
    float* xA = smem;
    float* yS = xA + D;
    float* xB = yS + HD;
    float* gS = xB + D;
    float* qS = gS + F;
    float* q_s = qS + (G + 2) * hd;
    float* k_new = q_s + G * hd;
    float* v_new = k_new + hd;
    constexpr int LPP = hd >> 3, PPW = 64 / LPP, NSLOT = 4 * PPW;
    float* ml_s = v_new + hd;
    float* acc_s = ml_s + NSLOT * G * 2;
    float* mscr = acc_s + NSLOT * G * hd;
    float* outS = mscr + 64 * 6;
    int* dead = reinterpret_cast<int*>(outS + ENG_MAX_OUT);
    int* out_count = dead + 1;
    int* reg_s = dead + 4;
    if (tid == 0) { *dead = eng_fault_here(p.ctl, 0u, b) ? 1 : 0; *out_count = 0; }
    if (tid == ENG_CW * 64) {
        reg_s[0] = 0; reg_s[1] = 0; reg_s[2] = 1;
        if (XL || p.rep_stride) eng_register(p.ctl, nb, reg_s, dead);
        if (XL && (reg_s[2] * Hkv != nb || reg_s[0] >= Hkv || reg_s[1] >= reg_s[2] || p.nsplit != reg_s[2])) {
            if (!__hip_atomic_load((eng_gu32*)(p.ctl + ENG_CTL_ABORT), ENG_RLX)) __hip_atomic_store((eng_gu32*)(p.ctl + ENG_CTL_WHERE), 9998u, ENG_RLX);
            __hip_atomic_store((eng_gu32*)(p.ctl + ENG_CTL_ABORT), 1u, ENG_RLX);
            reg_s[0] = 0; reg_s[1] = 0;
            *dead = 1;
        }
    }
    const unsigned epoch = __hip_atomic_load((eng_gu32*)(p.ctl + ENG_CTL_EPOCH), ENG_RLX);
    const int pos = p.pos[0] + p.pos_off;
    unsigned long long clk0 = 0, rt0 = 0;
    if (p.stamps) { clk0 = __builtin_amdgcn_s_memtime(); rt0 = eng_rt(); }
    const size_t VSTR = (size_t)nb * ENG_LINE;
    const EngLayout layD{D / nb}, layF{F / nb}, layQ{QKVN / nb}, layLin{0};
    const int nsplit = XL ? nb / Hkv : p.nsplit;
    const int natt = Hkv * nsplit;
    const int chunk = (pos + nsplit) / nsplit;
    const int grp = lane / LPP, gl = lane % LPP;

    {
        const int* tk = p.toks;
        int t0 = tk[0];
        const bool is_vq = t0 >= p.sem_begin && t0 <= p.sem_end;
        t0 = min(max(t0, 0), p.vocab - 1);
        for (int d = tid; d < D; d += ENG_THREADS) {
            float vq = 0.f;
            if (is_vq) {
                constexpr int MAXCB = 16;
                for (int i0 = 0; i0 < p.ncb; i0 += MAXCB) {
                    int c[MAXCB];
                    float e[MAXCB];
#pragma unroll
                    for (int i = 0; i < MAXCB; ++i) c[i] = i0 + i < p.ncb ? tk[(size_t)(i0 + i + 1) * p.tok_row_stride] : 0;
#pragma unroll
                    for (int i = 0; i < MAXCB; ++i) {
                        const int cc = min(max(c[i], 0), p.cbsize - 1);
                        e[i] = i0 + i < p.ncb ? ld_elem(p.cb_emb, (size_t)(cc + (i0 + i) * p.cbsize) * D + d) : 0.f;
                    }
#pragma unroll
                    for (int i = 0; i < MAXCB; ++i) if (i0 + i < p.ncb) vq += e[i];
                }
                vq = round_bf16(vq);
            }
            float x = round_bf16(ld_elem(p.emb, (size_t)t0 * D + d) + vq);
            if (p.scale_cb && is_vq) x = round_bf16(x / p.inv_div);
            xA[d] = x;
        }
    }

    if (wave < ENG_CW) {
        int q_lo, q_hi, o_lo, o_hi, f_lo, f_hi, d_lo, d_hi;
        eng_units(QKVN, b, nb, q_lo, q_hi);
        if (XL) { q_lo = 0; q_hi = QKVN / nb; }
        eng_units(D, b, nb, o_lo, o_hi);
        eng_units(F, b, nb, f_lo, f_hi);
        eng_units(D, b, nb, d_lo, d_hi);
        EngW<NTD, 1, SQ> wq;
        EngW<NTA, 1, SO> wo;
        EngW<NTD, 2, SF> wf;
        EngW<NTF, 1, SO> wd;
        EngOut eo{outS, out_count, 0};
        {
            const EngLayer l0 = eng_layer(p.layers, 0);
            if (!XL) eng_issue(wq, l0.wqkv, l0.attn_norm, D, q_lo, q_hi, cw, lane, p.nt);
            eng_issue(wo, l0.wo, (const bf16_t*)nullptr, HD, o_lo, o_hi, cw, lane, p.nt);
            eng_issue(wf, l0.w13, l0.ffn_norm, D, f_lo, f_hi, cw, lane, p.nt);
            eng_issue(wd, l0.w2, (const bf16_t*)nullptr, F, d_lo, d_hi, cw, lane, p.nt);
            __builtin_amdgcn_sched_barrier(0);
        }
        eng_barrier();
        const int xnq = G * hd * Hkv / nb, xnk = hd * Hkv / nb;
        const EngRowQkvX rmq{reg_s[0] * G * hd + reg_s[1] * xnq, (H + reg_s[0]) * hd + reg_s[1] * xnk,
                             (H + Hkv + reg_s[0]) * hd + reg_s[1] * xnk, xnq, xnk};
        if (XL) {
            const EngLayer l0 = eng_layer(p.layers, 0);
            eng_issue(wq, l0.wqkv, l0.attn_norm, D, q_lo, q_hi, cw, lane, p.nt, rmq);
            __builtin_amdgcn_sched_barrier(0);
        }
        eng_barrier();
        for (int li = 0; li < p.n_layer; ++li) {
            const int par = li & 1, parn = (li + 1) & 1;
            const unsigned tag = eng_tag16(epoch + (unsigned)li);
            const unsigned tagn = eng_tag16(epoch + (unsigned)li + 1u);
            const EngLayer l = eng_layer(p.layers, li);
            const bool more = li + 1 < p.n_layer;
            const EngLayer ln = eng_layer(p.layers, more ? li + 1 : li);
            if (li > 0) { eng_barrier(); if (*dead) break; }
            ENG_STAMP(0);
            if (XL)
                eng_gemv_qkv_local<NTD, SQ>(wq, xA, D, p.eps, l.bqkv, p.gqkv + (size_t)par * VSTR, tag, q_hi, cw, lane, eo, rmq);
            else
                eng_gemv<NTD, 1, SQ, PRO_RMSNORM, EPI_STORE>(wq, xA, D, p.eps, l.bqkv, nullptr, p.gqkv + (size_t)par * VSTR + eng_pub(b, q_lo), tag, nullptr,
                                                             q_lo, q_hi, cw, lane, eo);
            __builtin_amdgcn_sched_barrier(0);
            ENG_STAMP(1);
            if (more) {
                if (XL) eng_issue(wq, ln.wqkv, ln.attn_norm, D, q_lo, q_hi, cw, lane, p.nt, rmq);
                else eng_issue(wq, ln.wqkv, ln.attn_norm, D, q_lo, q_hi, cw, lane, p.nt);
            }
            __builtin_amdgcn_sched_barrier(0);
            if (XL || eng_att_role(b, nb, li, natt) >= 0) {
                eng_barrier(); if (*dead) break;
                eng_barrier();
                eng_barrier();
            }
            ENG_STAMP(2);
            eng_barrier(); if (*dead) break;
            ENG_STAMP(3);
            eng_gemv<NTA, 1, SO, PRO_NONE, EPI_RESID>(wo, yS, HD, p.eps, l.bo, xA, p.gxb + (size_t)par * VSTR + eng_pub(b, o_lo), tag, nullptr, o_lo, o_hi, cw, lane, eo);
            __builtin_amdgcn_sched_barrier(0);
            ENG_STAMP(4);
            if (p.stamps && (p.nt & 2)) { asm volatile("s_waitcnt vmcnt(0)" ::: "memory"); ENG_STAMP(9); }
            if (more) eng_issue(wo, ln.wo, (const bf16_t*)nullptr, HD, o_lo, o_hi, cw, lane, p.nt);
            __builtin_amdgcn_sched_barrier(0);
            eng_barrier(); if (*dead) break;
            ENG_STAMP(5);
            eng_gemv<NTD, 2, SF, PRO_RMSNORM, EPI_SWIGLU, S::PK3>(wf, xB, D, p.eps, nullptr, nullptr,
                                                                   p.gg + (size_t)par * VSTR + (S::PK3 ? 0 : eng_pub(b, f_lo)), tag, nullptr, f_lo, f_hi, cw, lane, eo);
            __builtin_amdgcn_sched_barrier(0);
            ENG_STAMP(6);
            if (more) eng_issue(wf, ln.w13, ln.ffn_norm, D, f_lo, f_hi, cw, lane, p.nt);
            __builtin_amdgcn_sched_barrier(0);
            eng_barrier(); if (*dead) break;
            ENG_STAMP(7);
            eng_gemv<NTF, 1, SO, PRO_NONE, EPI_RESID>(wd, gS, F, p.eps, nullptr, xB, p.gx + (size_t)parn * VSTR + eng_pub(b, d_lo), tagn,
                                                      li == p.n_layer - 1 ? p.x_out : nullptr, d_lo, d_hi, cw, lane, eo);
            __builtin_amdgcn_sched_barrier(0);
            ENG_STAMP(8);
            if (more) eng_issue(wd, ln.w2, (const bf16_t*)nullptr, F, d_lo, d_hi, cw, lane, p.nt);
            __builtin_amdgcn_sched_barrier(0);
            if (!(p.nt & 2)) ENG_STAMP(9);
        }
    } else {
        U4 kpf[ENG_KVST], vpf[ENG_KVST];
        float gq0 = 1.f, gq1 = 1.f, gk0 = 1.f, gk1 = 1.f;
        int att_next = -1;
        int plan_layer = -1;
        const bf16_t *plan_kc = nullptr, *plan_vc = nullptr, *plan_qn = nullptr, *plan_kn = nullptr;
        const int period = (natt > 0 && nb % natt == 0) ? nb / natt : 0;
        int x_role = 0;
        auto role = [&](int layer) { return XL ? x_role : eng_att_role(b, nb, layer, natt); };
        auto kv_plan = [&](int from_layer) {
            plan_layer = -1;
            if (from_layer >= p.n_layer) return;
            if (XL) {
                plan_layer = from_layer;
            } else if (period > 0) {
                const int phase = b / natt;
                int d = phase - from_layer % period;
                if (d < 0) d += period;
                if (from_layer + d < p.n_layer) plan_layer = from_layer + d;
            } else {
                for (int l2 = from_layer; l2 < p.n_layer; ++l2)
                    if (role(l2) >= 0) { plan_layer = l2; break; }
            }
            if (plan_layer < 0) return;
            const EngLayer l2 = eng_layer(p.layers, plan_layer);
            plan_kc = l2.kc; plan_vc = l2.vc; plan_qn = l2.qn; plan_kn = l2.kn;
        };
        auto kv_issue = [&]() {
            att_next = plan_layer;
#pragma unroll
            for (int st = 0; st < ENG_KVST; ++st) { kpf[st] = U4{0u, 0u, 0u, 0u}; vpf[st] = U4{0u, 0u, 0u, 0u}; }
            if (att_next < 0) return;
            const int a = role(att_next);
            const int kvh = a / nsplit, split = a % nsplit;
            const int lo = split * chunk, hi = min(lo + chunk, pos + 1);
            if (lane < hp) {
                if (plan_qn) { gq0 = eng_ldg_bf16(plan_qn, 2 * lane); gq1 = eng_ldg_bf16(plan_qn, 2 * lane + 1); }
                if (plan_kn) { gk0 = eng_ldg_bf16(plan_kn, 2 * lane); gk1 = eng_ldg_bf16(plan_kn, 2 * lane + 1); }
            }
            const bf16_t* kc = plan_kc + p.cache_off + (size_t)kvh * p.n_slots * hd;
            const bf16_t* vc = plan_vc + p.cache_off + (size_t)kvh * p.n_slots * hd;
#pragma unroll
            for (int st = 0; st < ENG_KVST; ++st) {
                const int j = lo + st * NSLOT + gw * PPW + grp;
                if (j < hi && j != pos) {
                    kpf[st] = eng_ldg16<false>(kc + (size_t)j * hd + gl * 8);
                    vpf[st] = eng_ldg16<false>(vc + (size_t)j * hd + gl * 8);
                }
            }
        };
        if (!XL) { kv_plan(0); kv_issue(); }
        eng_barrier();
        const EngRelay rl{p.rep_stride != 0, reg_s[1], reg_s[2], p.rep_delta0 + (long)reg_s[0] * p.rep_stride};
        if (XL) { x_role = reg_s[0] * nsplit + reg_s[1]; kv_plan(0); kv_issue(); }
        float rope_c = 1.f, rope_s = 0.f;
        if (lane < hp) { rope_c = p.rope[((size_t)pos * hp + lane) * 2]; rope_s = p.rope[((size_t)pos * hp + lane) * 2 + 1]; }
        eng_barrier();
        for (int li = 0; li < p.n_layer; ++li) {
            const int par = li & 1;
            const unsigned tag = eng_tag16(epoch + (unsigned)li), tag32 = eng_tag32(epoch + (unsigned)li);
            const EngLayer l = eng_layer(p.layers, li);
            if (li > 0) {
                eng_gather_x(rl, p.gx + (size_t)par * VSTR, layD, 0, D, tag, xA, gw, ENG_GW, lane, p.ctl, dead, li * 8 + 0);
                eng_barrier(); if (*dead) break;
            }
            const int a = role(li);
            if (a >= 0) {
                kv_plan(li + 1);
                const int kvh = a / nsplit, split = a % nsplit;
                const int lo = split * chunk;
                const int hi = min(lo + chunk, pos + 1);
                bf16_t* kc = l.kc + p.cache_off + (size_t)kvh * p.n_slots * hd;
                bf16_t* vc = l.vc + p.cache_off + (size_t)kvh * p.n_slots * hd;
                const int slot = gw * PPW + grp;
                const unsigned* gq = p.gqkv + (size_t)par * VSTR;
                ENG_ASTAMP(0, 0);
                constexpr int QFL = XL ? 2 : 0;
                if (gw == 0) eng_gather<EngIdent, QFL>(gq, layQ, kvh * G * hd, G * hd, tag, qS, 0, 1, lane, p.ctl, dead, li * 8 + 1);
                if (gw == 1) eng_gather<EngIdent, QFL>(gq, layQ, (H + kvh) * hd, hd, tag, qS + G * hd, 0, 1, lane, p.ctl, dead, li * 8 + 1);
                if (gw == 2) eng_gather<EngIdent, QFL>(gq, layQ, (H + Hkv + kvh) * hd, hd, tag, qS + (G + 1) * hd, 0, 1, lane, p.ctl, dead, li * 8 + 1);
                eng_barrier(); if (*dead) break;
                ENG_ASTAMP(0, 1);
                if (gw >= 0) {
                    for (int item = gw; item < G + 2; item += 4) {
                        const float* src = qS + item * hd;
                        const bf16_t* gain = item < G ? l.qn : (item == G ? l.kn : nullptr);
                        float* dst = item < G ? q_s + item * hd : (item == G ? k_new : v_new);
                        if (item == G + 1) {
                            for (int e = lane; e < hd; e += 64) dst[e] = src[e];
                        } else {
                            float x0 = 0.f, x1 = 0.f;
                            if (lane < hp) { x0 = src[2 * lane]; x1 = src[2 * lane + 1]; }
                            if (gain) {
                                const float ss = wave_sum(x0 * x0 + x1 * x1);
                                const float inv = rsqrt_exact(ss / (float)hd + p.eps);
                                if (lane < hp) {
                                    const bool have = att_next == li;
                                    const float g0 = have ? (item < G ? gq0 : gk0) : eng_ldg_bf16(gain, 2 * lane);
                                    const float g1 = have ? (item < G ? gq1 : gk1) : eng_ldg_bf16(gain, 2 * lane + 1);
                                    x0 = round_bf16((x0 * inv) * g0);
                                    x1 = round_bf16((x1 * inv) * g1);
                                }
                            }
                            if (lane < hp) {
                                dst[2 * lane] = round_bf16(x0 * rope_c - x1 * rope_s);
                                dst[2 * lane + 1] = round_bf16(x1 * rope_c + x0 * rope_s);
                            }
                        }
                    }
                }
                eng_barrier();
                ENG_ASTAMP(0, 2);
                if (gw >= 0) {
                    if (pos >= lo && pos < hi) {
                        for (int e = atid; e < hd; e += 256) {
                            st_elem(kc, (size_t)pos * hd + e, k_new[e]);
                            st_elem(vc, (size_t)pos * hd + e, v_new[e]);
                        }
                    }
                    float qr[G][8];
#pragma unroll
                    for (int g = 0; g < G; ++g)
#pragma unroll
                        for (int e = 0; e < 8; ++e) qr[g][e] = q_s[g * hd + gl * 8 + e];
                    float mrun[G], lrun[G], acc[G][8];
#pragma unroll
                    for (int g = 0; g < G; ++g) {
                        mrun[g] = -INFINITY; lrun[g] = 0.f;
#pragma unroll
                        for (int e = 0; e < 8; ++e) acc[g][e] = 0.f;
                    }
                    auto step = [&](const int j, const float (&kv)[8], const float (&vv)[8]) {
                        const bool valid = j < hi;
#pragma unroll
                        for (int g = 0; g < G; ++g) {
                            float d = 0.f;
#pragma unroll
                            for (int e = 0; e < 8; ++e) d = fmaf(qr[g][e], kv[e], d);
                            if (LPP > 1) d = group_sum_rt(d, LPP);
                            if (valid) {
                                const float s = d * p.scale;
                                const float mn = fmaxf(mrun[g], s);
                                const float corr = expf(mrun[g] - mn);
                                const float pj = expf(s - mn);
                                lrun[g] = lrun[g] * corr + pj;
#pragma unroll
                                for (int e = 0; e < 8; ++e) acc[g][e] = acc[g][e] * corr + pj * vv[e];
                                mrun[g] = mn;
                            }
                        }
                    };
                    const bool pre = att_next == li;
                    for (int blk = 0; lo + gw * PPW + blk * (ENG_KVST * NSLOT) < hi; ++blk) {
#pragma unroll
                        for (int st = 0; st < ENG_KVST; ++st) {
                            const int base = lo + gw * PPW + (blk * ENG_KVST + st) * NSLOT;
                            if (base < hi) {
                                const int j = base + grp;
                                float kv[8], vv[8];
                                if (j < hi && j == pos) {
#pragma unroll
                                    for (int e = 0; e < 8; ++e) { kv[e] = k_new[gl * 8 + e]; vv[e] = v_new[gl * 8 + e]; }
                                } else if (pre || blk > 0) {
                                    Vec<bf16_t>::unpack(kpf[st], kv); Vec<bf16_t>::unpack(vpf[st], vv);
                                } else if (j < hi) {
                                    Vec<bf16_t>::unpack(eng_ldg16<false>(kc + (size_t)j * hd + gl * 8), kv);
                                    Vec<bf16_t>::unpack(eng_ldg16<false>(vc + (size_t)j * hd + gl * 8), vv);
                                } else {
#pragma unroll
                                    for (int e = 0; e < 8; ++e) { kv[e] = 0.f; vv[e] = 0.f; }
                                }
                                const int jn = j + ENG_KVST * NSLOT;
                                if (jn < hi && jn != pos) {
                                    kpf[st] = eng_ldg16<false>(kc + (size_t)jn * hd + gl * 8);
                                    vpf[st] = eng_ldg16<false>(vc + (size_t)jn * hd + gl * 8);
                                } else {
                                    kpf[st] = U4{0u, 0u, 0u, 0u}; vpf[st] = U4{0u, 0u, 0u, 0u};
                                }
                                step(j, kv, vv);
                            }
                        }
                    }
                    ENG_ASTAMP(0, 7);
#pragma unroll
                    for (int g = 0; g < G; ++g) {
                        if (gl == 0) { ml_s[(slot * G + g) * 2] = mrun[g]; ml_s[(slot * G + g) * 2 + 1] = lrun[g]; }
#pragma unroll
                        for (int e = 0; e < 8; ++e) acc_s[(size_t)(slot * G + g) * hd + gl * 8 + e] = acc[g][e];
                    }
                    ENG_ASTAMP(0, 8);
                }
                eng_barrier();
                ENG_ASTAMP(0, 3);
                if (gw >= 0) {
                    const bool quick = NSLOT == 16 && (hd & 63) == 0;
                    for (int idx0 = gw * 64; idx0 < G * hd; idx0 += 256) {
                        const int idx = idx0 + lane;
                        const int g = quick ? idx0 / hd : idx / hd, e = idx % hd;
                        float M = -INFINITY, L = 0.f, O = 0.f;
                        if (quick) {
                            const int sl = lane & 15;
                            const float m_l = ml_s[(sl * G + g) * 2], l_l = ml_s[(sl * G + g) * 2 + 1];
                            M = m_l;
                            M = fmaxf(M, dpp_f<DPP_XOR1>(M));
                            M = fmaxf(M, dpp_f<DPP_XOR2>(M));
                            M = fmaxf(M, dpp_f<DPP_HALF_MIRROR>(M));
                            M = fmaxf(M, dpp_f<DPP_MIRROR>(M));
                            if (M > -INFINITY) {
                                const float w_l = expf(m_l - M);
#pragma unroll
                                for (int s2 = 0; s2 < 16; ++s2) {
                                    const float w = lane_f(w_l, s2);
                                    L += lane_f(l_l, s2) * w;
                                    O += acc_s[(size_t)(s2 * G + g) * hd + e] * w;
                                }
                            }
                        } else if (idx < G * hd) {
                            for (int s2 = 0; s2 < NSLOT; ++s2) M = fmaxf(M, ml_s[(s2 * G + g) * 2]);
                            if (M > -INFINITY) {
                                for (int s2 = 0; s2 < NSLOT; ++s2) {
                                    const float w = expf(ml_s[(s2 * G + g) * 2] - M);
                                    L += ml_s[(s2 * G + g) * 2 + 1] * w;
                                    O += acc_s[(size_t)(s2 * G + g) * hd + e] * w;
                                }
                            }
                        }
                        if (idx < G * hd) {
                            const int head = kvh * G + g;
                            if (nsplit == 1) {
                                eng_put(p.gy + (size_t)par * HD, head * hd + e, round_bf16(O / L), tag);
                            } else {
                                unsigned long long* gp = p.gpart + (((size_t)par * H + head) * nsplit + split) * (hd + 2);
                                if (XL) {
                                    eng_put64_local(gp, e, O, tag32);
                                    if (e == 0) { eng_put64_local(gp, hd, M, tag32); eng_put64_local(gp, hd + 1, L, tag32); }
                                } else {
                                    eng_put64(gp, e, O, tag32);
                                    if (e == 0) { eng_put64(gp, hd, M, tag32); eng_put64(gp, hd + 1, L, tag32); }
                                }
                            }
                        }
                    }
                }
                ENG_ASTAMP(0, 4);
                if (XL && gw == 3 && nsplit == 32 && hd == 128 && G == 2) {
                    const int item = lane >> 5, s = lane & 31, e = split * 4;
                    const int head = kvh * G + item;
                    const unsigned long long* gs = p.gpart + (((size_t)par * H + head) * nsplit + s) * (hd + 2);
                    EngSpin sp{p.ctl, dead, 0, 0, li * 8 + 2};
                    U4 A, B, C;
                    bool alive = true;
                    for (;;) {
                        eng_ld3_sc1<2>(gs + e, gs + e + 2, gs + hd, A, B, C);
                        const bool ok = A.y == tag32 && A.w == tag32 && B.y == tag32 && B.w == tag32 && C.y == tag32 && C.w == tag32;
                        if (__all(ok)) break;
                        if (sp.give_up(lane)) { alive = false; break; }
                    }
                    ENG_ASTAMP(3, 5);
                    if (alive) {
                        const float m_ = __uint_as_float(C.x), l_ = __uint_as_float(C.z);
                        float Mc = m_;
                        Mc = fmaxf(Mc, dpp_f<DPP_XOR1>(Mc));
                        Mc = fmaxf(Mc, dpp_f<DPP_XOR2>(Mc));
                        Mc = fmaxf(Mc, dpp_f<DPP_HALF_MIRROR>(Mc));
                        float* mx = mscr;
                        float* pr = mscr + 8;
                        if ((lane & 7) == 0) mx[lane >> 3] = Mc;
                        __builtin_amdgcn_wave_barrier();
                        __builtin_amdgcn_fence(__ATOMIC_ACQ_REL, "wavefront");
                        float Mrun = -INFINITY;
                        const int ch = s >> 3;
#pragma unroll
                        for (int c = 0; c < 4; ++c) if (c <= ch) Mrun = fmaxf(Mrun, mx[item * 4 + c]);
                        const float w = m_ > -INFINITY ? expf(m_ - Mrun) : 0.f;
                        float* q5 = pr + (size_t)(item * 32 + s) * 5;
                        q5[0] = l_ * w;
                        q5[1] = __uint_as_float(A.x) * w; q5[2] = __uint_as_float(A.z) * w;
                        q5[3] = __uint_as_float(B.x) * w; q5[4] = __uint_as_float(B.z) * w;
                        __builtin_amdgcn_wave_barrier();
                        __builtin_amdgcn_fence(__ATOMIC_ACQ_REL, "wavefront");
                        const int ci = (lane >> 3) & 1, cq = lane & 7;
                        float acc = 0.f;
                        {
                            const float* src = pr + (size_t)ci * 32 * 5 + (cq < 5 ? cq : 0);
                            float v[32];
#pragma unroll
                            for (int k = 0; k < 32; ++k) v[k] = src[k * 5];
                            float mc[4], rr[4];
#pragma unroll
                            for (int c = 0; c < 4; ++c) mc[c] = mx[ci * 4 + c];
                            float M = -INFINITY;
#pragma unroll
                            for (int c = 0; c < 4; ++c) {
                                const float Mn = fmaxf(M, mc[c]);
                                rr[c] = (c > 0 && M > -INFINITY && mc[c] > -INFINITY) ? expf(M - Mn) : 1.0f;
                                M = Mn;
                            }
#pragma unroll
                            for (int c = 0; c < 4; ++c) {
                                acc *= rr[c];
#pragma unroll
                                for (int k = 0; k < 8; ++k) acc += v[c * 8 + k];
                            }
                        }
                        const float a0 = dpp_f<0x101>(acc), a1 = dpp_f<0x102>(acc), a2 = dpp_f<0x103>(acc), a3 = dpp_f<0x104>(acc);
                        if (lane == 0 || lane == 8) {
                            unsigned* gy = p.gy + (size_t)par * HD + (size_t)a * (G * 4) + ci * 4;
                            eng_put4(gy, round_bf16(a0 / acc), round_bf16(a1 / acc), round_bf16(a2 / acc), round_bf16(a3 / acc), tag);
                        }
                    }
                    ENG_ASTAMP(3, 6);
                } else
                if (nsplit > 1 && gw == 3) {
                    const int epb = hd / nsplit;
                    const int e4n = epb >> 2;
                    const int nitem = G * e4n;
                    EngSpin sp{p.ctl, dead, 0, 0, li * 8 + 2};
                    bool alive = true;
                    for (int ib = 0; ib < nitem && alive; ib += 8) {
                        const int it = ib + (lane >> 3), s8 = lane & 7;
                        const bool item_on = it < nitem;
                        const int g = item_on ? it / e4n : 0;
                        const int e = split * epb + (item_on ? (it % e4n) * 4 : 0);
                        const int head = kvh * G + g;
                        const unsigned long long* gp = p.gpart + ((size_t)par * H + head) * nsplit * (hd + 2);
                        float M = -INFINITY, L = 0.f, a0 = 0.f, a1 = 0.f, a2 = 0.f, a3 = 0.f;
                        for (int c0 = 0; c0 < nsplit && alive; c0 += 8) {
                            const bool son = item_on && c0 + s8 < nsplit;
                            const unsigned long long* gs = gp + (size_t)(son ? c0 + s8 : 0) * (hd + 2);
                            U4 A, B, C;
                            for (;;) {
                                eng_ld3_sc1(gs + e, gs + e + 2, gs + hd, A, B, C);
                                const bool ok = !son || (A.y == tag32 && A.w == tag32 && B.y == tag32 && B.w == tag32 &&
                                                         C.y == tag32 && C.w == tag32);
                                if (__all(ok)) break;
                                if (sp.give_up(lane)) { alive = false; break; }
                            }
                            if (!alive) break;
                            if (ib + 8 >= nitem && c0 + 8 >= nsplit) ENG_ASTAMP(3, 5);
                            const float m_ = son ? __uint_as_float(C.x) : -INFINITY;
                            const float l_ = son ? __uint_as_float(C.z) : 0.f;
                            float Mc = m_;
                            Mc = fmaxf(Mc, dpp_f<DPP_XOR1>(Mc));
                            Mc = fmaxf(Mc, dpp_f<DPP_XOR2>(Mc));
                            Mc = fmaxf(Mc, dpp_f<DPP_HALF_MIRROR>(Mc));
                            if (Mc > -INFINITY) {
                                const float Mn = fmaxf(M, Mc);
                                if (c0 > 0 && M > -INFINITY) {
                                    const float rr = expf(M - Mn);
                                    L *= rr; a0 *= rr; a1 *= rr; a2 *= rr; a3 *= rr;
                                }
                                M = Mn;
                                const float w = m_ > -INFINITY ? expf(m_ - M) : 0.f;
                                const float pl = l_ * w;
                                const float p0 = __uint_as_float(A.x) * w, p1 = __uint_as_float(A.z) * w;
                                const float p2 = __uint_as_float(B.x) * w, p3 = __uint_as_float(B.z) * w;
                                L += pl; a0 += p0; a1 += p1; a2 += p2; a3 += p3;
#define ENG_MSTEP(n) L += dpp_f<0x100 + n>(pl); a0 += dpp_f<0x100 + n>(p0); a1 += dpp_f<0x100 + n>(p1); \
                     a2 += dpp_f<0x100 + n>(p2); a3 += dpp_f<0x100 + n>(p3);
                                ENG_MSTEP(1) ENG_MSTEP(2) ENG_MSTEP(3) ENG_MSTEP(4) ENG_MSTEP(5) ENG_MSTEP(6) ENG_MSTEP(7)
#undef ENG_MSTEP
                            }
                        }
                        if (alive && s8 == 0 && item_on) {
                            unsigned* gy = p.gy + (size_t)par * HD + (size_t)a * (G * epb) + g * epb + (e - split * epb);
                            eng_put4(gy, round_bf16(a0 / L), round_bf16(a1 / L), round_bf16(a2 / L), round_bf16(a3 / L), tag);
                        }
                    }
                    ENG_ASTAMP(3, 6);
                }
            }
            {
                const int epb = hd / nsplit, ns = nsplit;
                auto ymap = [=](int i) { const int a2 = i / (G * epb), r2 = i % (G * epb), g2 = r2 / epb, eo = r2 % epb;
                                         return ((a2 / ns) * G + g2) * hd + (a2 % ns) * epb + eo; };
                eng_gather_x(rl, p.gy + (size_t)par * HD, layLin, 0, HD, tag, yS, gw, ENG_GW, lane, p.ctl, dead, li * 8 + 3, ymap);
            }
            eng_barrier(); if (*dead) break;
            if (a >= 0) kv_issue();
            const unsigned long long t_poll0 = p.stamps ? eng_rt() : 0ull;
            eng_gather_x(rl, p.gxb + (size_t)par * VSTR, layD, 0, D, tag, xB, gw, ENG_GW, lane, p.ctl, dead, li * 8 + 4, EngIdent(),
                       (p.stamps && gw == 0) ? p.stamps + ((size_t)b * p.n_layer + li) * 16 + 13 : nullptr);
            const unsigned long long t_poll1 = p.stamps ? eng_rt() : 0ull;
            eng_barrier(); if (*dead) break;
            if (p.stamps && tid == ENG_CW * 64) {
                unsigned long long* q = p.stamps + ((size_t)b * p.n_layer + li) * 16;
                q[10] = t_poll0; q[11] = t_poll1; q[12] = eng_rt();
            }
            if constexpr (S::PK3) eng_gather3_x(rl, p.gg + (size_t)par * VSTR, F, tag, gS, gw, ENG_GW, lane, p.ctl, dead, li * 8 + 5);
            else eng_gather_x(rl, p.gg + (size_t)par * VSTR, layF, 0, F, tag, gS, gw, ENG_GW, lane, p.ctl, dead, li * 8 + 5);
            eng_barrier(); if (*dead) break;
        }
    }

    eng_barrier();
    if (p.stamps && tid == 0 && b == 0) {
        p.stamps[14] = __builtin_amdgcn_s_memtime() - clk0; p.stamps[15] = eng_rt() - rt0;
    }
    if (tid == 0) {
        const unsigned old = atomicAdd(p.ctl + ENG_CTL_EXIT, 1u);
        if (old + 1 == (unsigned)nb) {
            __hip_atomic_store((eng_gu32*)(p.ctl + ENG_CTL_EXIT), 0u, ENG_RLX);
            __hip_atomic_store((eng_gu32*)(p.ctl + ENG_CTL_ARRIVED), 0u, ENG_RLX);
            for (int x = 0; x < 8; ++x) __hip_atomic_store((eng_gu32*)(p.ctl + ENG_CTL_XCD + x), 0u, ENG_RLX);
            __hip_atomic_store((eng_gu32*)(p.ctl + ENG_CTL_EPOCH), epoch + ENG_EPOCH_STEP, ENG_RLX);
        }
    }
}

struct FastEngP {
    const EngLayer* layers;
    int n_layer, ncb;
    int D, H, Hkv, hd, F, qkvN, V;
    float eps, scale;
    const float* rope;
    const bf16_t* fast_norm; const bf16_t* fast_out; const bf16_t* fast_emb;
    const float* hid;
    const float* femb;
    unsigned* gx;
    unsigned* gqkv;
    unsigned* gxb;
    unsigned* gg;
    unsigned* glog;
    unsigned* gcode;
    unsigned* ctl;
    long rep_delta0, rep_stride;
    SampP samp;
    long noise_cb_stride;
    long noise_off1;
    int pair;
    const bf16_t* qkv0_tab;
    unsigned long long* stamps;
    int nt;
};
#define ENG_FSTAMP(k) do { if (p.stamps && tid == 0) p.stamps[(((size_t)b * p.ncb + cb) * nL + li) * 16 + (k)] = eng_rt(); } while (0)

#define ENG_GSTAMP(k) do { if (p.stamps && atid == 0) p.stamps[(((size_t)b * p.ncb + cb) * nL + nL - 1) * 16 + (k)] = eng_rt(); } while (0)
constexpr int ENG_FV = 1024;

struct EngSub {
    int* end_at;
    int n;
    __device__ __forceinline__ void sync(int) { ++n; eng_barrier(); }
};
__device__ __forceinline__ void eng_draw_follow(const int* end_at) {
    for (int c = 1;; ++c) {
        eng_barrier();
        if (*reinterpret_cast<const volatile int*>(end_at) == c) break;
    }
}

template <int MAXCB, int HD>
__device__ __forceinline__ void eng_fast_attn(const float* qkvS, bf16_t* kS, bf16_t* vS, float* yS, const bf16_t* qn, const bf16_t* kn,
                                              const float (&cs)[2], const float (&sn)[2], int c, int ncb, int H, int Hkv, float eps, float scale,
                                              int w, int nw, int lane) {
    constexpr int EPL = HD > 64 ? 2 : 1;
    const int G = H / Hkv;
    for (int h = w; h < H; h += nw) {
        const int kvh = h / G;
        bf16_t* kh = kS + (size_t)kvh * ncb * HD + lane;
        bf16_t* vh = vS + (size_t)kvh * ncb * HD + lane;
        const float* qp = qkvS + h * HD + lane;
        const float* kp = qkvS + (H + kvh) * HD + lane;
        const float* vp = qkvS + (H + Hkv + kvh) * HD + lane;
        float q[EPL], kx[EPL], vx[EPL];
#pragma unroll
        for (int e = 0; e < EPL; ++e) { q[e] = qp[64 * e]; kx[e] = kp[64 * e]; vx[e] = vp[64 * e]; }
        if (c == 0) {
            if (h % G == 0) {
                if (kn) {
                    float ss = kx[0] * kx[0];
                    if (EPL > 1) ss = kx[0] * kx[0] + kx[EPL - 1] * kx[EPL - 1];
                    ss = wave_sum(ss);
                    const float inv = rsqrt_exact(ss / (float)HD + eps);
#pragma unroll
                    for (int e = 0; e < EPL; ++e) kx[e] = round_bf16((kx[e] * inv) * eng_ldg_bf16(kn, lane + 64 * e));
                }
#pragma unroll
                for (int e = 0; e < EPL; ++e) {
                    const float ko = dpp_f<DPP_XOR1>(kx[e]);
                    kx[e] = round_bf16((lane & 1) == 0 ? kx[e] * cs[e] - ko * sn[e] : kx[e] * cs[e] + ko * sn[e]);
                    kh[64 * e] = f32_to_bf16_bits(kx[e]); vh[64 * e] = f32_to_bf16_bits(vx[e]);
                }
            }
#pragma unroll
            for (int e = 0; e < EPL; ++e) yS[h * HD + lane + 64 * e] = round_bf16(vx[e]);
            continue;
        }
        if (qn) {
            float ss = q[0] * q[0];
            if (EPL > 1) ss = q[0] * q[0] + q[EPL - 1] * q[EPL - 1];
            ss = wave_sum(HD < 64 ? (lane < HD ? ss : 0.f) : ss);
            const float inv = rsqrt_exact(ss / (float)HD + eps);
#pragma unroll
            for (int e = 0; e < EPL; ++e) q[e] = round_bf16((q[e] * inv) * eng_ldg_bf16(qn, lane + 64 * e));
        }
        if (kn) {
            float ss = kx[0] * kx[0];
            if (EPL > 1) ss = kx[0] * kx[0] + kx[EPL - 1] * kx[EPL - 1];
            ss = wave_sum(ss);
            const float inv = rsqrt_exact(ss / (float)HD + eps);
#pragma unroll
            for (int e = 0; e < EPL; ++e) kx[e] = round_bf16((kx[e] * inv) * eng_ldg_bf16(kn, lane + 64 * e));
        }
#pragma unroll
        for (int e = 0; e < EPL; ++e) {
            const float qo = dpp_f<DPP_XOR1>(q[e]), ko = dpp_f<DPP_XOR1>(kx[e]);
            const bool even = (lane & 1) == 0;
            q[e] = round_bf16(even ? q[e] * cs[e] - qo * sn[e] : q[e] * cs[e] + qo * sn[e]);
            kx[e] = round_bf16(even ? kx[e] * cs[e] - ko * sn[e] : kx[e] * cs[e] + ko * sn[e]);
        }
        if (h % G == 0) {
#pragma unroll
            for (int e = 0; e < EPL; ++e) { kh[c * HD + 64 * e] = f32_to_bf16_bits(kx[e]); vh[c * HD + 64 * e] = f32_to_bf16_bits(vx[e]); }
        }
        float sl = -INFINITY;
        float mx = -INFINITY;
#pragma unroll
        for (int j = 0; j < MAXCB; ++j) {
            if (j <= c) {
                float pr;
                if (EPL > 1) {
                    const float k0 = j == c ? kx[0] : bf16_bits_to_f32(kh[j * HD]), k1 = j == c ? kx[EPL - 1] : bf16_bits_to_f32(kh[j * HD + 64 * (EPL - 1)]);
                    pr = fmaf(q[EPL - 1], k1, q[0] * k0);
                } else {
                    const float k0 = j == c ? kx[0] : bf16_bits_to_f32(kh[j * HD]);
                    pr = fmaf(0.f, 0.f, q[0] * k0);
                }
                const float d = wave_sum(pr);
                const float sj = round_bf16(round_bf16(d) * scale);
                mx = fmaxf(mx, sj);
                if (lane == j) sl = sj;
            }
        }
        const float el = lane <= c ? expf(sl - mx) : 0.f;
        float sum = 0.f;
#pragma unroll
        for (int j = 0; j < MAXCB; ++j)
            if (j <= c) sum += lane_f(el, j);
        const float pl = lane <= c ? round_bf16(el / sum) : 0.f;
        float o[EPL];
#pragma unroll
        for (int e = 0; e < EPL; ++e) o[e] = 0.f;
#pragma unroll
        for (int j = 0; j < MAXCB; ++j) {
            if (j <= c) {
                const float pj = lane_f(pl, j);
#pragma unroll
                for (int e = 0; e < EPL; ++e) o[e] = fmaf(pj, j == c ? vx[e] : bf16_bits_to_f32(vh[j * HD + 64 * e]), o[e]);
            }
        }
#pragma unroll
        for (int e = 0; e < EPL; ++e) yS[h * HD + lane + 64 * e] = round_bf16(o[e]);
    }
}

constexpr int DPP_ROW_SHL4 = 0x104, DPP_ROW_SHL8 = 0x108, DPP_ROW_SHL12 = 0x10C;
template <int MAXCB, int GQ>
__device__ __forceinline__ void eng_fast_attn64(const float* qkvS, bf16_t* kS, bf16_t* vS, float* yS, const bf16_t* qn, const bf16_t* kn,
                                                float cs, float sn, int c, int ncb, int H, int Hkv, float eps, float scale,
                                                int w, int nw, int lane) {
    constexpr int HD = 64;
    const bool even = (lane & 1) == 0;
    const int r = lane >> 4, k4 = (lane & 15) * 4;
    for (int kvh = w; kvh < Hkv; kvh += nw) {
        bf16_t* kh = kS + (size_t)kvh * ncb * HD;
        bf16_t* vh = vS + (size_t)kvh * ncb * HD;
        float kx = qkvS[(H + kvh) * HD + lane];
        const float vx = qkvS[(H + Hkv + kvh) * HD + lane];
        float* slot = yS + (size_t)kvh * GQ * HD;
        float q[GQ];
#pragma unroll
        for (int g = 0; g < GQ; ++g) q[g] = qkvS[(kvh * GQ + g) * HD + lane];
        if (kn) {
            const float ss = wave_sum(kx * kx);
            const float inv = rsqrt_exact(ss / (float)HD + eps);
            kx = round_bf16((kx * inv) * eng_ldg_bf16(kn, lane));
        }
        {
            const float ko = dpp_f<DPP_XOR1>(kx);
            kx = round_bf16(even ? kx * cs - ko * sn : kx * cs + ko * sn);
        }
        kh[c * HD + lane] = f32_to_bf16_bits(kx);
        vh[c * HD + lane] = f32_to_bf16_bits(vx);
        if (c == 0) {
#pragma unroll
            for (int g = 0; g < GQ; ++g) slot[g * HD + lane] = round_bf16(vx);
            continue;
        }
#pragma unroll
        for (int g = 0; g < GQ; ++g) {
            if (qn) {
                const float ss = wave_sum(q[g] * q[g]);
                const float inv = rsqrt_exact(ss / (float)HD + eps);
                q[g] = round_bf16((q[g] * inv) * eng_ldg_bf16(qn, lane));
            }
            const float qo = dpp_f<DPP_XOR1>(q[g]);
            q[g] = round_bf16(even ? q[g] * cs - qo * sn : q[g] * cs + qo * sn);
            slot[g * HD + lane] = q[g];
        }
        __builtin_amdgcn_wave_barrier();
        float4 q4[GQ];
#pragma unroll
        for (int g = 0; g < GQ; ++g) q4[g] = *reinterpret_cast<const float4*>(slot + g * HD + k4);
        __builtin_amdgcn_wave_barrier();
#pragma unroll
        for (int ps = 0; ps < (MAXCB + 3) / 4; ++ps) {
            if (ps * 4 <= c) {
                const int j = ps * 4 + r;
                const int jj = j <= c ? j : c;
                const uint2 kb = *reinterpret_cast<const uint2*>(kh + jj * HD + k4);
                const float k0 = __uint_as_float(kb.x << 16), k1 = __uint_as_float(kb.x & 0xffff0000u);
                const float k2 = __uint_as_float(kb.y << 16), k3 = __uint_as_float(kb.y & 0xffff0000u);
#pragma unroll
                for (int g = 0; g < GQ; ++g) {
                    const float p0 = fmaf(0.f, 0.f, q4[g].x * k0), p1 = fmaf(0.f, 0.f, q4[g].y * k1);
                    const float p2 = fmaf(0.f, 0.f, q4[g].z * k2), p3 = fmaf(0.f, 0.f, q4[g].w * k3);
                    float sdot = (p0 + p1) + (p2 + p3);
                    sdot += dpp_f<DPP_XOR1>(sdot);
                    sdot += dpp_f<DPP_XOR2>(sdot);
                    float a = sdot + dpp_f<DPP_ROW_SHL4>(sdot);
                    a = a + dpp_f<DPP_ROW_SHL8>(sdot);
                    a = a + dpp_f<DPP_ROW_SHL12>(sdot);
                    const float sj = round_bf16(round_bf16(a) * scale);
                    if ((lane & 15) == 0 && j <= c) slot[g * HD + j] = sj;
                }
            }
        }
        __builtin_amdgcn_wave_barrier();
        float sl[GQ], el[GQ], sum[GQ], pl[GQ], o[GQ];
#pragma unroll
        for (int g = 0; g < GQ; ++g) sl[g] = lane <= c ? slot[g * HD + lane] : -INFINITY;
        __builtin_amdgcn_wave_barrier();
#pragma unroll
        for (int g = 0; g < GQ; ++g) {
            float mx = sl[g];
            mx = fmaxf(mx, dpp_f<DPP_XOR1>(mx));
            mx = fmaxf(mx, dpp_f<DPP_XOR2>(mx));
            mx = fmaxf(mx, dpp_f<DPP_HALF_MIRROR>(mx));
            mx = fmaxf(mx, dpp_f<DPP_MIRROR>(mx));
            mx = lane_f(mx, 0);
            el[g] = lane <= c ? expf(sl[g] - mx) : 0.f;
            sum[g] = 0.f; o[g] = 0.f;
        }
#pragma unroll
        for (int j = 0; j < MAXCB; ++j)
            if (j <= c) {
#pragma unroll
                for (int g = 0; g < GQ; ++g) sum[g] += lane_f(el[g], j);
            }
#pragma unroll
        for (int g = 0; g < GQ; ++g) pl[g] = lane <= c ? round_bf16(el[g] / sum[g]) : 0.f;
#pragma unroll
        for (int j = 0; j < MAXCB; ++j)
            if (j <= c) {
                const float vj = bf16_bits_to_f32(vh[j * HD + lane]);
#pragma unroll
                for (int g = 0; g < GQ; ++g) o[g] = fmaf(lane_f(pl[g], j), vj, o[g]);
            }
#pragma unroll
        for (int g = 0; g < GQ; ++g) slot[g * HD + lane] = round_bf16(o[g]);
    }
}
template <int MAXCB, int HD>
__device__ __forceinline__ void eng_fast_attn_any(const float* qkvS, bf16_t* kS, bf16_t* vS, float* yS, const bf16_t* qn, const bf16_t* kn,
                                                  const float (&cs)[2], const float (&sn)[2], int c, int ncb, int H, int Hkv, float eps,
                                                  float scale, int w, int nw, int lane) {
    if constexpr (HD == 64 && MAXCB <= 16) {
        const int G = H / Hkv;
        if (G == 2) { eng_fast_attn64<MAXCB, 2>(qkvS, kS, vS, yS, qn, kn, cs[0], sn[0], c, ncb, H, Hkv, eps, scale, w, nw, lane); return; }
        if (G == 1) { eng_fast_attn64<MAXCB, 1>(qkvS, kS, vS, yS, qn, kn, cs[0], sn[0], c, ncb, H, Hkv, eps, scale, w, nw, lane); return; }
    }
    eng_fast_attn<MAXCB, HD>(qkvS, kS, vS, yS, qn, kn, cs, sn, c, ncb, H, Hkv, eps, scale, w, nw, lane);
}

struct EngSampLds {
    float* redbuf;
    int* pen_id;
    float* pen_val;
    float* amv;
    int* ami;
    int* wcnt;
    float* prL;
    uint32_t* keyL;
    uint32_t* cut;
};
struct EngDrawPre {
    RowCtl ctl;
    int nfv;
    int pen;
    float q4[4];
};
__device__ __forceinline__ EngDrawPre eng_draw_pre(const SampP& p, int tid) {
    EngDrawPre d;
// ... 9 lines not shown
    if (p.noise && d.nfv < p.noise_rows) qrow = p.noise + (size_t)d.nfv * p.noise_row_len + p.noise_off;
    draw_noise4(p, d.ctl, qrow, 4 * tid, d.nfv, 0, ENG_FV, d.q4);
    return d;
}
__device__ __forceinline__ int eng_sample_small(const SampP& p, const EngDrawPre& pre, const float* L, const EngSampLds& S, EngSub& sub, int tid, int lane, int wave,
                                                unsigned long long* stp = nullptr) {
    constexpr int V = ENG_FV;
    const RowCtl ctl = pre.ctl;
    const int nfv = pre.nfv;
    const int R = p.ncb + 1;
    const int* seq = p.seq;
    int red_phase = 0;
    auto red_sum = [&](float v) {
        v = wave_sum(v);
        float* slot = S.redbuf + 4 * (red_phase & 1);
        ++red_phase;
        if (lane == 0) slot[wave] = v;
        sub.sync(lane);
        return ((slot[0] + slot[1]) + slot[2]) + slot[3];
    };
    const int i0 = 4 * tid;
    float l[4];
#pragma unroll
    for (int e = 0; e < 4; ++e) l[e] = (i0 + e) < V ? L[i0 + e] : -INFINITY;
    if (nfv > 0) {
        const int it = nfv - 1;
        const int ws = it < 16 ? 0 : it - 16;
        const int npen = p.cb == 0 ? R : 16;
        (void)ws;
        if (tid < npen) {
            const int id = p.cb == 0 ? seq[(size_t)tid * p.cap + ws + 1] : pre.pen;
            S.pen_id[tid] = -1;
            if (id >= 0 && id < V) {
                const float sv = L[id];
                S.pen_id[tid] = id;
                S.pen_val[tid] = sv < 0.f ? round_bf16(sv * ctl.rep) : round_bf16(sv / ctl.rep);
            }
        }
        sub.sync(lane);
        if (p.cb != 0) {
            int ids[16]; float nvs[16];
#pragma unroll
            for (int k = 0; k < 16; k += 4) {
                const int4 a = *reinterpret_cast<const int4*>(S.pen_id + k);
                const float4 v = *reinterpret_cast<const float4*>(S.pen_val + k);
                ids[k] = a.x; ids[k + 1] = a.y; ids[k + 2] = a.z; ids[k + 3] = a.w;
                nvs[k] = v.x; nvs[k + 1] = v.y; nvs[k + 2] = v.z; nvs[k + 3] = v.w;
            }
#pragma unroll
            for (int k = 0; k < 16; ++k) {
                const unsigned d = (unsigned)(ids[k] - i0);
#pragma unroll
                for (int e = 0; e < 4; ++e) if (d == (unsigned)e) l[e] = nvs[k];
            }
        } else {
            for (int k = 0; k < npen; ++k) {
                const int id = S.pen_id[k];
                if (id >= i0 && id < i0 + 4) {
                    const float nv = S.pen_val[k];
#pragma unroll
                    for (int e = 0; e < 4; ++e) if (i0 + e == id) l[e] = nv;
                }
            }
        }
    }
    if (p.cb == 0 && ctl.ban_eos && p.im_end < V) {
#pragma unroll
        for (int e = 0; e < 4; ++e) if (i0 + e == p.im_end) l[e] = -INFINITY;
    }
    int bb_phase = 0;
    auto block_best = [&](ArgMax a) {
        a = wave_argmax(a);
        float* av = S.amv + 4 * (bb_phase & 1);
        int* ai = S.ami + 4 * (bb_phase & 1);
        ++bb_phase;
        if (lane == 0) { av[wave] = a.v; ai[wave] = a.i; }
        sub.sync(lane);
        ArgMax t{av[0], ai[0]};
#pragma unroll
        for (int w = 1; w < 4; ++w) t = better(t, ArgMax{av[w], ai[w]});
        return t;
    };
    ArgMax am{-INFINITY, 0x7fffffff};
#pragma unroll
    for (int e = 0; e < 4; ++e) if (i0 + e < V) am = better(am, ArgMax{l[e], i0 + e});
    am = block_best(am);
    if (stp && tid == 0) stp[12] = eng_rt();
    const float Lmax = am.v;
    float ex[4], z = 0.f;
#pragma unroll
    for (int e = 0; e < 4; ++e) { ex[e] = (i0 + e) < V ? expf(l[e] - Lmax) : 0.f; z += ex[e]; }
    const float Z = red_sum(z);
    if (stp && tid == 0) stp[-16 + 10] = eng_rt();
    const float tp = round_bf16(ctl.top_p);
    auto removed = [&](float cum) { return round_bf16(cum) > tp; };
    constexpr uint32_t cmask = 0xffff0000u;
    uint32_t key[4];
#pragma unroll
    for (int e = 0; e < 4; ++e) {
        const bool v = (i0 + e) < V;
        key[e] = v ? (order_key(l[e]) & cmask) : 0u;
        S.prL[i0 + e] = v ? round_bf16(ex[e] / Z) : 0.f;
        S.keyL[i0 + e] = key[e];
    }
    const bool only_top = removed(round_bf16(1.0f / Z));
    int winner = am.i;
    if (!only_top) {
        sub.sync(lane);
        const float Tc = fmaxf(ctl.temperature, 1e-5f);
        const float Mt = round_bf16(Lmax / Tc);
        float etp[4];
        if (wave != 0) {
#pragma unroll
            for (int e = 0; e < 4; ++e) etp[e] = expf(round_bf16(l[e] / Tc) - Mt);
        }
        if (stp && tid == 0) stp[-16 + 11] = eng_rt();
        if (wave == 0) {
            float pr[16];
            uint32_t ky[16];
#pragma unroll
            for (int e = 0; e < 16; ++e) { pr[e] = S.prL[lane + 64 * e]; ky[e] = S.keyL[lane + 64 * e]; }
            float tot = 0.f;
#pragma unroll
            for (int e = 0; e < 16; ++e) tot += pr[e];
            tot = wave_sum(tot);
            if (stp && tid == 0) stp[-16 + 12] = eng_rt();
            uint32_t kstar = 0;
            int nk = 0, all_kept = 0;
            if (!removed(tot)) {
                all_kept = 1;
            } else {
                uint32_t kmx = 0u;
#pragma unroll
                for (int e = 0; e < 16; ++e) kmx = ky[e] > kmx ? ky[e] : kmx;
                {
                    int km = (int)(kmx >> 16);
                    km = max(km, dpp_i<DPP_XOR1>(km));
                    km = max(km, dpp_i<DPP_XOR2>(km));
                    km = max(km, dpp_i<DPP_HALF_MIRROR>(km));
                    km = max(km, dpp_i<DPP_MIRROR>(km));
                    km = max(max(__builtin_amdgcn_readlane(km, 0), __builtin_amdgcn_readlane(km, 16)),
                             max(__builtin_amdgcn_readlane(km, 32), __builtin_amdgcn_readlane(km, 48)));
                    kmx = (uint32_t)km << 16;
                }
                for (int bit = 31; bit >= 16; --bit) {
                    const uint32_t cand = kstar | (1u << bit);
                    if (cand > kmx) continue;
                    float ms = 0.f;
#pragma unroll
                    for (int e = 0; e < 16; ++e) ms += ky[e] >= cand ? pr[e] : 0.f;
                    if (removed(wave_sum(ms))) kstar = cand;
                }
                if (stp && tid == 0) stp[-16 + 13] = eng_rt();
                float above = 0.f, cnt = 0.f;
#pragma unroll
                for (int e = 0; e < 16; ++e) {
                    if (ky[e] > kstar) above += pr[e];
                    else if (ky[e] == kstar && (lane + 64 * e) < V) cnt += 1.f;
                }
                above = wave_sum(above);
                const int icnt = (int)wave_sum(cnt);
                const uint32_t ubits = (kstar & 0x80000000u) ? (kstar & 0x7fffffffu) : ~(kstar | ~cmask);
                const float pk = round_bf16(expf(__uint_as_float(ubits) - Lmax) / Z);
                int lo_n = 0, hi_n = icnt;
                while (lo_n < hi_n) {
                    const int mid = (lo_n + hi_n + 1) >> 1;
                    if (removed(fmaf((float)mid, pk, above))) hi_n = mid - 1; else lo_n = mid;
                }
                nk = lo_n;
            }
            if (stp && tid == 0) stp[-16 + 14] = eng_rt();
            if (lane == 0) { S.cut[0] = kstar; S.cut[1] = (uint32_t)nk; S.cut[2] = (uint32_t)all_kept; }
        }
        sub.sync(lane);
        if (stp && tid == 0) stp[13] = eng_rt();
        const uint32_t kstar = S.cut[0];
        const int nk = (int)S.cut[1];
        const bool all_kept = S.cut[2] != 0;
        if (wave == 0) {
#pragma unroll
            for (int e = 0; e < 4; ++e) etp[e] = expf(round_bf16(l[e] / Tc) - Mt);
        }
        bool mem[4];
        int mine = 0;
#pragma unroll
        for (int e = 0; e < 4; ++e) { mem[e] = (i0 + e) < V && !all_kept && key[e] == kstar; mine += mem[e] ? 1 : 0; }
        int below = 0, wtot = 0;
        const unsigned long long lower = (1ull << lane) - 1ull;
#pragma unroll
        for (int c = 1; c <= 4; ++c) {
            const unsigned long long bal = __ballot(mine >= c);
            below += __popcll(bal & lower);
            wtot += __popcll(bal);
        }
        if (lane == 0) S.wcnt[wave] = wtot;
        sub.sync(lane);
        int rank = below;
        for (int w = 0; w < wave; ++w) rank += S.wcnt[w];
        bool keep[4];
        float et[4], z2 = 0.f;
#pragma unroll
        for (int e = 0; e < 4; ++e) {
            keep[e] = (i0 + e) < V && (all_kept || key[e] > kstar || (mem[e] && rank < nk));
            rank += mem[e] ? 1 : 0;
            et[e] = keep[e] ? etp[e] : 0.f;
            z2 += et[e];
        }
        const float Z2 = red_sum(z2);
        ArgMax best{-1.f, 0x7fffffff};
#pragma unroll
        for (int e = 0; e < 4; ++e) {
            if (i0 + e < V) {
                const float prob = keep[e] ? round_bf16(et[e] / Z2) : 0.f;
                best = better(best, ArgMax{round_bf16(prob / round_bf16(pre.q4[e])), i0 + e});
            }
        }
        winner = block_best(best).i;
    }
    return winner;
}

template <typename S>
__global__ __launch_bounds__(ENG_CW * 64) void eng_qkv0_table_kernel(const bf16_t* wqkv, const bf16_t* bqkv, const bf16_t* attn_norm,
                                                                      const bf16_t* fast_emb, bf16_t* tab, int D, int qkvN, int ncodes,
                                                                      float eps) {
    extern __shared__ __attribute__((aligned(16))) float smem[];
    float* xs = smem;
    float* vals = xs + D;
    const int tid = threadIdx.x, lane = tid & 63, cw = tid >> 6;
    int q_lo, q_hi;
    eng_units(qkvN, blockIdx.x, gridDim.x, q_lo, q_hi);
    constexpr int NTD = S::NTD;
    EngW<NTD, 1, S::SQ> wq;
    eng_issue<false>(wq, wqkv, attn_norm, D, q_lo, q_hi, cw, lane, 0);
    const int per = (ncodes + gridDim.y - 1) / gridDim.y;
    const int c_lo = blockIdx.y * per, c_hi = min(c_lo + per, ncodes);
    for (int code = c_lo; code < c_hi; ++code) {
        for (int d = tid * 8; d < D; d += ENG_CW * 64 * 8) {
            float e8[8];
            Vec<bf16_t>::unpack(eng_ldg16<false>(fast_emb + (size_t)code * D + d), e8);
#pragma unroll
            for (int j = 0; j < 8; ++j) xs[d + j] = e8[j];
        }
        __syncthreads();
        eng_gemv_rows<NTD, 1, S::SQ, PRO_RMSNORM, EPI_STORE>(wq, xs, D, eps, bqkv, nullptr, vals, q_lo, q_hi, cw, lane);
        __syncthreads();
        if (tid < q_hi - q_lo) tab[(size_t)code * qkvN + q_lo + tid] = f32_to_bf16_bits(vals[tid]);
        __syncthreads();
    }
}

inline size_t eng_fast_lds_bytes(int D, int qkvN, int HD, int F, int V, int nL, int ncb, int KVW, bool pair) {
    size_t fl = (size_t)D * 2 + qkvN + HD + F + V + ENG_MAX_OUT + 8 + 32 + 32 + 20 + 2048 + 4 + 4 + 16;
    size_t by = fl * sizeof(float) + (size_t)nL * 2 * ncb * KVW * 2 + 64;
    if (pair) by += ((size_t)2 * D + (size_t)(F > qkvN + HD ? F : qkvN + HD)) * sizeof(float) + 16;
    return by;
}

template <typename FS, int MAXCB, bool RES>
__global__ __launch_bounds__(ENG_THREADS) void fast_engine_kernel(FastEngP p) {
    constexpr int NTD = FS::NTD, NTA = FS::NTA, NTF = FS::NTF, HDIM = FS::HDIM;
    constexpr int SQ = FS::SQ, SF = FS::SF, SO = FS::SO;
    static_assert(!RES || (FS::RESF > 0 && FS::RESL > 0), "this shape class has no resident set");
    constexpr int RF = RES ? FS::RESF : 0, RL = RES ? FS::RESL : 0, FRES = RF * ENG_GW;
    constexpr int SFC = RES ? (FS::F / ENG_NB - FRES + ENG_CW - 1) / ENG_CW : SF;
    constexpr int ARRF = RES ? ENG_WAVES : ENG_CW;
    static_assert(FS::F / ENG_NB > FRES, "the compute waves keep at least one pair");
    extern __shared__ __attribute__((aligned(16))) float smem[];
    const int tid = threadIdx.x, lane = tid & 63, wave = __builtin_amdgcn_readfirstlane(tid >> 6);
    const int b = blockIdx.x;
    constexpr int nb = ENG_NB;
    const int cw = wave, gw = wave - ENG_CW, atid = tid - ENG_CW * 64;
    constexpr int D = FS::D, F = FS::F, hd = HDIM, H = FS::H, Hkv = FS::HKV, HD = H * hd, KVW = Hkv * hd, QKVN = (H + 2 * Hkv) * hd, V = FS::V;
    float* xA = smem;
    float* qkvS = xA + D;
    float* yS = qkvS + QKVN;
    float* xB = yS + HD;
    float* gS = xB + D;
    float* logS = gS + F;
    float* outS = logS + V;
    float* redbuf = outS + ENG_MAX_OUT;
    int* pen_id = reinterpret_cast<int*>(redbuf + 8);
    float* pen_val = reinterpret_cast<float*>(pen_id + 32);
    float* amv = pen_val + 32;
    int* ami = reinterpret_cast<int*>(amv + 8);
    int* wcnt = ami + 8;
    float* prL = reinterpret_cast<float*>(wcnt + 4);
    uint32_t* keyL = reinterpret_cast<uint32_t*>(prL + 1024);
    uint32_t* cut = keyL + 1024;
    int* dead = reinterpret_cast<int*>(cut + 4);
    int* out_count = dead + 1;
    int* sub_count = dead + 2;
    int* codes_s = dead + 4;
    int* reg_s = codes_s + MAXCB;
    bf16_t* kvS = reinterpret_cast<bf16_t*>(reg_s + 4);
    float* xA1 = smem + ((((size_t)(reinterpret_cast<float*>(kvS + (size_t)p.n_layer * 2 * p.ncb * KVW) - smem)) + 3) & ~(size_t)3);
    float* xB1 = xA1 + D;
    float* gS1 = xB1 + D;
    float* qkvS1 = gS1;
    float* yS1 = gS1 + QKVN;
    int f_lo, f_hi;
    eng_units(F, b, nb, f_lo, f_hi);
    const int f_c_hi = f_hi - FRES;
    EngW<NTD, 2, (RF ? RF : 1)> res[RL ? RL : 1];
    if (p.stamps && tid == 0) p.stamps[(size_t)b * p.ncb * p.n_layer * 16 + 15] = eng_rt();
    if (tid == 0) { *dead = eng_fault_here(p.ctl, ENG_FAULT_FAST, b) ? 1 : 0; *out_count = 0; *sub_count = 0; dead[3] = 0; }
    if (tid == ENG_CW * 64) {
        reg_s[0] = 0; reg_s[1] = 0; reg_s[2] = 1;
        if (p.rep_stride) eng_register(p.ctl, nb, reg_s, dead);
    }
    const unsigned epoch = __hip_atomic_load((eng_gu32*)(p.ctl + ENG_CTL_EPOCH), ENG_RLX);
    const size_t VSTR = (size_t)nb * ENG_LINE;
    const EngLayout layD{D / nb}, layF{F / nb}, layQ{QKVN / nb}, layV{V / nb};
    const int nL = p.n_layer;
    auto bx = [&](int par, int l) { return p.gx + ((size_t)par * (nL + 1) + l) * VSTR; };
    auto bq = [&](int par, int l) { return p.gqkv + ((size_t)par * nL + l) * VSTR; };
    auto bxb = [&](int par, int l) { return p.gxb + ((size_t)par * nL + l) * VSTR; };
    auto bg = [&](int par, int l) { return p.gg + ((size_t)par * nL + l) * VSTR; };
    auto blog = [&](int par) { return p.glog + (size_t)par * VSTR; };
    auto drawer = [&](int cb) { return (cb * 37) % nb; };
    bool alive = true;
    const bool pair = p.pair != 0 && p.ncb >= 2;

    if (wave < ENG_CW) {
        int q_lo, q_hi, o_lo, o_hi, h_lo, h_hi;
        eng_units(QKVN, b, nb, q_lo, q_hi);
        eng_units(D, b, nb, o_lo, o_hi);
        eng_units(V, b, nb, h_lo, h_hi);
        EngW<NTD, 1, SQ> wq;
        EngW<NTA, 1, SO> wo;
        EngW<NTD, 2, SFC> wf;
        EngW<NTF, 1, SO> wd;
        EngW<NTD, 1, SO> wh;
        EngOut eo{outS, out_count, 0};
        EngOut eo13{outS, dead + 3, 0};
        EngOut& eoF = RES ? eo13 : eo;
        {
            const EngLayer l0 = eng_layer(p.layers, 0);
            eng_issue<false>(wq, l0.wqkv, l0.attn_norm, D, q_lo, q_hi, cw, lane, p.nt);
            eng_issue<false>(wo, l0.wo, (const bf16_t*)nullptr, HD, o_lo, o_hi, cw, lane, p.nt);
            eng_issue<false>(wf, l0.w13, l0.ffn_norm, D, f_lo, f_c_hi, cw, lane, p.nt);
            eng_issue<false>(wd, l0.w2, (const bf16_t*)nullptr, F, o_lo, o_hi, cw, lane, p.nt);
            __builtin_amdgcn_sched_barrier(0);
        }
        eng_barrier();
        eng_barrier();
        if (p.stamps && tid == 0) p.stamps[(size_t)b * p.ncb * p.n_layer * 16 + 14] = eng_rt();
        if (pair) {
            const unsigned tag0 = eng_tag16(epoch), tag1 = eng_tag16(epoch + 1u);
            float r0c[2], r0s[2], r1c[2], r1s[2];
#pragma unroll
            for (int e = 0; e < 2; ++e) {
                const int d = lane + 64 * e;
                r0c[e] = d < hd ? p.rope[((size_t)(d >> 1)) * 2] : 1.f;
                r0s[e] = d < hd ? p.rope[((size_t)(d >> 1)) * 2 + 1] : 0.f;
                r1c[e] = d < hd ? p.rope[((size_t)(hd >> 1) + (d >> 1)) * 2] : 1.f;
                r1s[e] = d < hd ? p.rope[((size_t)(hd >> 1) + (d >> 1)) * 2 + 1] : 0.f;
            }
            for (int li = 0; li < nL; ++li) {
                const int cb = 1;
                unsigned *gxL = p.gx, *gqL = p.gqkv, *gxbL = p.gxb, *ggL = p.gg;
                asm volatile("" : "+s"(gxL), "+s"(gqL), "+s"(gxbL), "+s"(ggL));
                auto bx = [&](int par, int l_) { return gxL + ((size_t)par * (nL + 1) + l_) * VSTR; };
                auto bq = [&](int par, int l_) { return gqL + ((size_t)par * nL + l_) * VSTR; };
                auto bxb = [&](int par, int l_) { return gxbL + ((size_t)par * nL + l_) * VSTR; };
                auto bg = [&](int par, int l_) { return ggL + ((size_t)par * nL + l_) * VSTR; };
                const EngLayer l = eng_layer(p.layers, li);
                const bool more = !(p.ncb == 2 && li == nL - 1);
                const bool tail0 = li + 1 < nL;
                const EngLayer ln = eng_layer(p.layers, li + 1 < nL ? li + 1 : 0);
                bf16_t* kL = kvS + (size_t)(li * 2) * p.ncb * KVW;
                bf16_t* vL = kvS + (size_t)(li * 2 + 1) * p.ncb * KVW;
                eng_barrier(); if (*dead) { alive = false; break; }
                ENG_FSTAMP(0);
                eng_gemv2<NTD, 1, SQ, PRO_RMSNORM, EPI_STORE>(wq, xA, xA1, D, p.eps, l.bqkv, nullptr, nullptr, bq(0, li) + eng_pub(b, q_lo),
                                                              bq(1, li) + eng_pub(b, q_lo), tag0, tag1, q_lo, q_hi, cw, lane, eo);
                __builtin_amdgcn_sched_barrier(0);
                ENG_FSTAMP(1);
                if (more && !(li == nL - 1 && p.qkv0_tab != nullptr)) eng_issue<false>(wq, ln.wqkv, ln.attn_norm, D, q_lo, q_hi, cw, lane, p.nt);
                __builtin_amdgcn_sched_barrier(0);
                eng_barrier(); if (*dead) { alive = false; break; }
                ENG_FSTAMP(2);
                eng_fast_attn_any<MAXCB, HDIM>(qkvS, kL, vL, yS, l.qn, l.kn, r0c, r0s, 0, p.ncb, H, Hkv, p.eps, p.scale, wave, ENG_WAVES, lane);
                eng_barrier();
                eng_fast_attn_any<MAXCB, HDIM>(qkvS1, kL, vL, yS1, l.qn, l.kn, r1c, r1s, 1, p.ncb, H, Hkv, p.eps, p.scale, wave, ENG_WAVES, lane);
                ENG_FSTAMP(9);
                eng_barrier();
                ENG_FSTAMP(3);
                if (tail0)
                    eng_gemv2<NTA, 1, SO, PRO_NONE, EPI_RESID>(wo, yS, yS1, HD, p.eps, l.bo, xA, xA1, bxb(0, li) + eng_pub(b, o_lo),
                                                               bxb(1, li) + eng_pub(b, o_lo), tag0, tag1, o_lo, o_hi, cw, lane, eo);
                else
                    eng_gemv<NTA, 1, SO, PRO_NONE, EPI_RESID>(wo, yS1, HD, p.eps, l.bo, xA1, bxb(1, li) + eng_pub(b, o_lo), tag1, nullptr,
                                                              o_lo, o_hi, cw, lane, eo);
                __builtin_amdgcn_sched_barrier(0);
                ENG_FSTAMP(4);
                if (more) eng_issue<false>(wo, ln.wo, (const bf16_t*)nullptr, HD, o_lo, o_hi, cw, lane, p.nt);
                __builtin_amdgcn_sched_barrier(0);
                eng_barrier(); if (*dead) { alive = false; break; }
                ENG_FSTAMP(5);
                if (tail0)
                    eng_gemv2_part<NTD, 2, SFC, PRO_RMSNORM, EPI_SWIGLU, ARRF>(wf, xB, xB1, D, p.eps, nullptr, nullptr, nullptr, bg(0, li) + eng_pub(b, f_lo),
                                                                               bg(1, li) + eng_pub(b, f_lo), tag0, tag1, f_lo, f_hi, f_lo, f_c_hi, cw, lane, eoF);
                else
                    eng_gemv_part<NTD, 2, SFC, PRO_RMSNORM, EPI_SWIGLU, FS::PK3, ARRF>(wf, xB1, D, p.eps, nullptr, nullptr, bg(1, li) + (FS::PK3 ? 0 : eng_pub(b, f_lo)), tag1, nullptr,
                                                                                f_lo, f_hi, f_lo, f_c_hi, cw, lane, eoF);
                __builtin_amdgcn_sched_barrier(0);
                ENG_FSTAMP(6);
                if (more) eng_issue<false>(wf, ln.w13, ln.ffn_norm, D, f_lo, f_c_hi, cw, lane, p.nt);
                __builtin_amdgcn_sched_barrier(0);
                eng_barrier(); if (*dead) { alive = false; break; }
                ENG_FSTAMP(7);
                if (tail0)
                    eng_gemv2<NTF, 1, SO, PRO_NONE, EPI_RESID>(wd, gS, gS1, F, p.eps, nullptr, xB, xB1, bx(0, li + 1) + eng_pub(b, o_lo),
                                                               bx(1, li + 1) + eng_pub(b, o_lo), tag0, tag1, o_lo, o_hi, cw, lane, eo);
                else
                    eng_gemv<NTF, 1, SO, PRO_NONE, EPI_RESID>(wd, gS1, F, p.eps, nullptr, xB1, bx(1, li + 1) + eng_pub(b, o_lo), tag1, nullptr,
                                                              o_lo, o_hi, cw, lane, eo);
                __builtin_amdgcn_sched_barrier(0);
                ENG_FSTAMP(8);
                if (more) eng_issue<false>(wd, ln.w2, (const bf16_t*)nullptr, F, o_lo, o_hi, cw, lane, p.nt);
                if (li == nL - 1) eng_issue<false>(wh, p.fast_out, p.fast_norm, D, h_lo, h_hi, cw, lane, p.nt);
                __builtin_amdgcn_sched_barrier(0);
            }
            if (alive) {
                eng_barrier();
                if (*dead) alive = false;
                else {
                    eng_gemv<NTD, 1, SO, PRO_RMSNORM, EPI_STORE>(wh, xA, D, p.eps, nullptr, nullptr, blog(1) + eng_pub(b, h_lo), tag1, nullptr,
                                                                 h_lo, h_hi, cw, lane, eo);
                    __builtin_amdgcn_sched_barrier(0);
                    eng_draw_follow(sub_count);
                }
            }
        }
        for (int cb = pair ? 2 : 0; cb < p.ncb && alive; ++cb) {
            const int par = cb & 1;
            const unsigned tag = eng_tag16(epoch + (unsigned)cb);
            float rcs[2], rsn[2];
#pragma unroll
            for (int e = 0; e < 2; ++e) {
                const int d = lane + 64 * e;
                rcs[e] = d < hd ? p.rope[((size_t)cb * (hd >> 1) + (d >> 1)) * 2] : 1.f;
                rsn[e] = d < hd ? p.rope[((size_t)cb * (hd >> 1) + (d >> 1)) * 2 + 1] : 0.f;
            }
            const bool tab0 = p.qkv0_tab != nullptr && cb >= 2;
            for (int li = 0; li < nL; ++li) {
                const EngLayer l = eng_layer(p.layers, li);
                const bool more = !(cb == p.ncb - 1 && li == nL - 1);
                const EngLayer ln = eng_layer(p.layers, li + 1 < nL ? li + 1 : 0);
                eng_barrier(); if (*dead) { alive = false; break; }
                ENG_FSTAMP(0);
                if (!(li == 0 && tab0))
                    eng_gemv<NTD, 1, SQ, PRO_RMSNORM, EPI_STORE>(wq, xA, D, p.eps, l.bqkv, nullptr, bq(par, li) + eng_pub(b, q_lo), tag,
                                                                 nullptr, q_lo, q_hi, cw, lane, eo);
                __builtin_amdgcn_sched_barrier(0);
                ENG_FSTAMP(1);
                if (more && !(li == nL - 1 && p.qkv0_tab != nullptr && cb + 1 >= 2))
                    eng_issue<false>(wq, ln.wqkv, ln.attn_norm, D, q_lo, q_hi, cw, lane, p.nt);
                __builtin_amdgcn_sched_barrier(0);
                eng_barrier(); if (*dead) { alive = false; break; }
                ENG_FSTAMP(2);
                eng_fast_attn_any<MAXCB, HDIM>(qkvS, kvS + (size_t)(li * 2) * p.ncb * KVW, kvS + (size_t)(li * 2 + 1) * p.ncb * KVW, yS, l.qn, l.kn,
                                         rcs, rsn, cb, p.ncb, H, Hkv, p.eps, p.scale, wave, ENG_WAVES, lane);
                ENG_FSTAMP(9);
                eng_barrier();
                ENG_FSTAMP(3);
                eng_gemv<NTA, 1, SO, PRO_NONE, EPI_RESID>(wo, yS, HD, p.eps, l.bo, xA, bxb(par, li) + eng_pub(b, o_lo), tag, nullptr,
                                                          o_lo, o_hi, cw, lane, eo);
                __builtin_amdgcn_sched_barrier(0);
                ENG_FSTAMP(4);
                if (more) eng_issue<false>(wo, ln.wo, (const bf16_t*)nullptr, HD, o_lo, o_hi, cw, lane, p.nt);
                __builtin_amdgcn_sched_barrier(0);
                eng_barrier(); if (*dead) { alive = false; break; }
                ENG_FSTAMP(5);
                eng_gemv_part<NTD, 2, SFC, PRO_RMSNORM, EPI_SWIGLU, FS::PK3, ARRF>(wf, xB, D, p.eps, nullptr, nullptr, bg(par, li) + (FS::PK3 ? 0 : eng_pub(b, f_lo)), tag, nullptr,
                                                                            f_lo, f_hi, f_lo, f_c_hi, cw, lane, eoF);
                __builtin_amdgcn_sched_barrier(0);
                ENG_FSTAMP(6);
                if (more) eng_issue<false>(wf, ln.w13, ln.ffn_norm, D, f_lo, f_c_hi, cw, lane, p.nt);
                __builtin_amdgcn_sched_barrier(0);
                eng_barrier(); if (*dead) { alive = false; break; }
                ENG_FSTAMP(7);
                eng_gemv<NTF, 1, SO, PRO_NONE, EPI_RESID>(wd, gS, F, p.eps, nullptr, xB, bx(par, li + 1) + eng_pub(b, o_lo), tag, nullptr,
                                                          o_lo, o_hi, cw, lane, eo);
                __builtin_amdgcn_sched_barrier(0);
                ENG_FSTAMP(8);
                if (more) eng_issue<false>(wd, ln.w2, (const bf16_t*)nullptr, F, o_lo, o_hi, cw, lane, p.nt);
                if (li == nL - 1 && cb >= 1) eng_issue<false>(wh, p.fast_out, p.fast_norm, D, h_lo, h_hi, cw, lane, p.nt);
                __builtin_amdgcn_sched_barrier(0);
            }
            if (!alive) break;
            if (cb >= 1) {
                eng_barrier(); if (*dead) { alive = false; break; }
                eng_gemv<NTD, 1, SO, PRO_RMSNORM, EPI_STORE>(wh, xA, D, p.eps, nullptr, nullptr, blog(par) + eng_pub(b, h_lo), tag, nullptr,
                                                             h_lo, h_hi, cw, lane, eo);
                __builtin_amdgcn_sched_barrier(0);
                eng_draw_follow(sub_count);
            }
        }
    } else {
        EngSub sub{sub_count, 0};
        SampP sp = p.samp;
        int prev_code = 0;
        EngOut eo13{outS, dead + 3, 0};
        U4 fgain[NTD];
        eng_barrier();
        const EngRelay rl{p.rep_stride != 0, reg_s[1], reg_s[2], p.rep_delta0 + (long)reg_s[0] * p.rep_stride};
        eng_barrier();
        if (pair) {
            const unsigned tag0 = eng_tag16(epoch), tag1 = eng_tag16(epoch + 1u);
            float r0c[2], r0s[2], r1c[2], r1s[2];
#pragma unroll
            for (int e = 0; e < 2; ++e) {
                const int d = lane + 64 * e;
                r0c[e] = d < hd ? p.rope[((size_t)(d >> 1)) * 2] : 1.f;
                r0s[e] = d < hd ? p.rope[((size_t)(d >> 1)) * 2 + 1] : 0.f;
                r1c[e] = d < hd ? p.rope[((size_t)(hd >> 1) + (d >> 1)) * 2] : 1.f;
                r1s[e] = d < hd ? p.rope[((size_t)(hd >> 1) + (d >> 1)) * 2 + 1] : 0.f;
            }
            for (int li = 0; li < nL; ++li) {
                const EngLayer l = eng_layer(p.layers, li);
                const bool tail0 = li + 1 < nL;
                int gl = lane;
                if constexpr (RES) asm volatile("" : "+v"(gl));
                const int wh = 1000 + 64 + li * 8;
                bf16_t* kL = kvS + (size_t)(li * 2) * p.ncb * KVW;
                bf16_t* vL = kvS + (size_t)(li * 2 + 1) * p.ncb * KVW;
                if (li > 0) {
                    eng_gather_x2(rl, EngSrc2{{bx(0, li), bx(1, li)}, {xA, xA1}, {tag0, tag1}}, D, gw, ENG_GW, gl, p.ctl, dead, wh + 0);
                } else {
                    for (int d = atid * 4; d < D; d += ENG_GW * 64 * 4) {
                        *reinterpret_cast<float4*>(xA + d) = *reinterpret_cast<const float4*>(p.hid + d);
                        *reinterpret_cast<float4*>(xA1 + d) = *reinterpret_cast<const float4*>(p.femb + d);
                    }
                }
                eng_barrier(); if (*dead) { alive = false; break; }
                eng_gather_x2(rl, EngSrc2{{bq(0, li), bq(1, li)}, {qkvS, qkvS1}, {tag0, tag1}}, QKVN, gw, ENG_GW, gl, p.ctl, dead, wh + 1);
                eng_barrier(); if (*dead) { alive = false; break; }
                if constexpr (RES) {
#pragma unroll
                    for (int r = 0; r < RL; ++r)
                        if (li == r) eng_issue<false>(res[r], l.w13, (const bf16_t*)nullptr, D, f_c_hi, f_hi, gw, lane, p.nt);
#pragma unroll
                    for (int t = 0; t < NTD; ++t) fgain[t] = eng_ldg16<false>(l.ffn_norm + t * 512 + lane * 8);
                    __builtin_amdgcn_sched_barrier(0);
                }
                eng_fast_attn_any<MAXCB, HDIM>(qkvS, kL, vL, yS, l.qn, l.kn, r0c, r0s, 0, p.ncb, H, Hkv, p.eps, p.scale, wave, ENG_WAVES, lane);
                eng_barrier();
                eng_fast_attn_any<MAXCB, HDIM>(qkvS1, kL, vL, yS1, l.qn, l.kn, r1c, r1s, 1, p.ncb, H, Hkv, p.eps, p.scale, wave, ENG_WAVES, lane);
                eng_barrier();
                if (tail0) eng_gather_x2(rl, EngSrc2{{bxb(0, li), bxb(1, li)}, {xB, xB1}, {tag0, tag1}}, D, gw, ENG_GW, gl, p.ctl, dead, wh + 2);
                else eng_gather_x(rl, bxb(1, li), layD, 0, D, tag1, xB1, gw, ENG_GW, gl, p.ctl, dead, wh + 2);
                eng_barrier(); if (*dead) { alive = false; break; }
                if constexpr (RES) {
#pragma unroll
                    for (int r = 0; r < RL; ++r)
                        if (li == r) {
                            eng_res_pin(res[r]);
#pragma unroll
                            for (int t = 0; t < NTD; ++t) res[r].gain[t] = fgain[t];
                            if (tail0)
                                eng_gemv2_part<NTD, 2, RF, PRO_RMSNORM, EPI_SWIGLU, ARRF>(res[r], xB, xB1, D, p.eps, nullptr, nullptr, nullptr, bg(0, li) + eng_pub(b, f_lo),
                                                                                          bg(1, li) + eng_pub(b, f_lo), tag0, tag1, f_lo, f_hi, f_c_hi, f_hi, gw, lane, eo13);
                            else
                                eng_gemv_part<NTD, 2, RF, PRO_RMSNORM, EPI_SWIGLU, FS::PK3, ARRF>(res[r], xB1, D, p.eps, nullptr, nullptr, bg(1, li) + (FS::PK3 ? 0 : eng_pub(b, f_lo)),
                                                                                           tag1, nullptr, f_lo, f_hi, f_c_hi, f_hi, gw, lane, eo13);
                        }
                    __builtin_amdgcn_sched_barrier(0);
                }
                if (tail0) eng_gather_x2(rl, EngSrc2{{bg(0, li), bg(1, li)}, {gS, gS1}, {tag0, tag1}}, F, gw, ENG_GW, gl, p.ctl, dead, wh + 3);
                else if constexpr (FS::PK3) eng_gather3_x(rl, bg(1, li), F, tag1, gS1, gw, ENG_GW, gl, p.ctl, dead, wh + 3);
                else eng_gather_x(rl, bg(1, li), layF, 0, F, tag1, gS1, gw, ENG_GW, gl, p.ctl, dead, wh + 3);
                eng_barrier(); if (*dead) { alive = false; break; }
            }
        }
        for (int cb = pair ? 1 : 0; cb < p.ncb && alive; ++cb) {
            const int par = cb & 1;
            const unsigned tag = eng_tag16(epoch + (unsigned)cb);
            float rcs[2], rsn[2];
#pragma unroll
            for (int e = 0; e < 2; ++e) {
                const int d = lane + 64 * e;
                rcs[e] = d < hd ? p.rope[((size_t)cb * (hd >> 1) + (d >> 1)) * 2] : 1.f;
                rsn[e] = d < hd ? p.rope[((size_t)cb * (hd >> 1) + (d >> 1)) * 2 + 1] : 0.f;
            }
            int at = atid, dl = lane;
            if constexpr (RES) asm volatile("" : "+v"(at), "+v"(dl));
            EngDrawPre pre{};
            if (cb >= 1) {
                sp.cb = cb;
                sp.noise_off = p.noise_off1 + (long)(cb - 1) * p.noise_cb_stride;
                pre = eng_draw_pre(sp, at);
            }
            for (int li = (pair && cb == 1) ? nL : 0; li < nL; ++li) {
                const EngLayer l = eng_layer(p.layers, li);
                int gl = lane;
                if constexpr (RES) asm volatile("" : "+v"(gl));
                if (li > 0) {
                    eng_gather_x(rl, bx(par, li), layD, 0, D, tag, xA, gw, ENG_GW, gl, p.ctl, dead, 1000 + cb * 64 + li * 8 + 0);
                } else if (cb <= 1) {
                    const float* src = cb == 0 ? p.hid : p.femb;
                    for (int d = atid * 4; d < D; d += ENG_GW * 64 * 4) *reinterpret_cast<float4*>(xA + d) = *reinterpret_cast<const float4*>(src + d);
                } else {
                    const int code = prev_code;
                    const int d0 = atid * 8;
                    if (p.qkv0_tab && D <= ENG_GW * 64 * 8 && QKVN <= ENG_GW * 64 * 8) {
                        const U4 ue = eng_ldg16<false>(p.fast_emb + (size_t)code * D + (d0 < D ? d0 : 0));
                        const U4 uq = eng_ldg16<false>(p.qkv0_tab + (size_t)code * QKVN + (d0 < QKVN ? d0 : 0));
                        float e8[8], q8[8];
                        Vec<bf16_t>::unpack(ue, e8);
                        Vec<bf16_t>::unpack(uq, q8);
                        if (d0 < D) {
#pragma unroll
                            for (int j = 0; j < 8; ++j) xA[d0 + j] = e8[j];
                        }
                        if (d0 < QKVN) {
#pragma unroll
                            for (int j = 0; j < 8; ++j) qkvS[d0 + j] = q8[j];
                        }
                    } else {
                        for (int d = d0; d < D; d += ENG_GW * 64 * 8) {
                            float e8[8];
                            Vec<bf16_t>::unpack(eng_ldg16<false>(p.fast_emb + (size_t)code * D + d), e8);
#pragma unroll
                            for (int j = 0; j < 8; ++j) xA[d + j] = e8[j];
                        }
                        if (p.qkv0_tab) {
                            for (int d = d0; d < QKVN; d += ENG_GW * 64 * 8) {
                                float e8[8];
                                Vec<bf16_t>::unpack(eng_ldg16<false>(p.qkv0_tab + (size_t)code * QKVN + d), e8);
#pragma unroll
                                for (int j = 0; j < 8; ++j) qkvS[d + j] = e8[j];
                            }
                        }
                    }
                }
                eng_barrier(); if (*dead) { alive = false; break; }
                if (!(li == 0 && cb >= 2 && p.qkv0_tab))
                    eng_gather_x(rl, bq(par, li), layQ, 0, QKVN, tag, qkvS, gw, ENG_GW, gl, p.ctl, dead, 1000 + cb * 64 + li * 8 + 1);
                eng_barrier(); if (*dead) { alive = false; break; }
                if constexpr (RES) {
                    if (!pair && cb == 0) {
#pragma unroll
                        for (int r = 0; r < RL; ++r)
                            if (li == r) eng_issue<false>(res[r], l.w13, (const bf16_t*)nullptr, D, f_c_hi, f_hi, gw, lane, p.nt);
                    }
#pragma unroll
                    for (int t = 0; t < NTD; ++t) fgain[t] = eng_ldg16<false>(l.ffn_norm + t * 512 + lane * 8);
                    __builtin_amdgcn_sched_barrier(0);
                }
                eng_fast_attn_any<MAXCB, HDIM>(qkvS, kvS + (size_t)(li * 2) * p.ncb * KVW, kvS + (size_t)(li * 2 + 1) * p.ncb * KVW, yS, l.qn, l.kn,
                                         rcs, rsn, cb, p.ncb, H, Hkv, p.eps, p.scale, wave, ENG_WAVES, lane);
                eng_barrier();
                eng_gather_x(rl, bxb(par, li), layD, 0, D, tag, xB, gw, ENG_GW, gl, p.ctl, dead, 1000 + cb * 64 + li * 8 + 2);
                eng_barrier(); if (*dead) { alive = false; break; }
                if constexpr (RES) {
#pragma unroll
                    for (int r = 0; r < RL; ++r)
                        if (li == r) {
                            eng_res_pin(res[r]);
#pragma unroll
                            for (int t = 0; t < NTD; ++t) res[r].gain[t] = fgain[t];
                            eng_gemv_part<NTD, 2, RF, PRO_RMSNORM, EPI_SWIGLU, FS::PK3, ARRF>(res[r], xB, D, p.eps, nullptr, nullptr, bg(par, li) + (FS::PK3 ? 0 : eng_pub(b, f_lo)),
                                                                                       tag, nullptr, f_lo, f_hi, f_c_hi, f_hi, gw, lane, eo13);
                        }
                    __builtin_amdgcn_sched_barrier(0);
                }
                if constexpr (FS::PK3) eng_gather3_x(rl, bg(par, li), F, tag, gS, gw, ENG_GW, gl, p.ctl, dead, 1000 + cb * 64 + li * 8 + 3);
                else eng_gather_x(rl, bg(par, li), layF, 0, F, tag, gS, gw, ENG_GW, gl, p.ctl, dead, 1000 + cb * 64 + li * 8 + 3);
                eng_barrier(); if (*dead) { alive = false; break; }
            }
            if (!alive) break;
            if (cb >= 1) {
                eng_gather_x(rl, bx(par, nL), layD, 0, D, tag, xA, gw, ENG_GW, dl, p.ctl, dead, 1000 + cb * 64 + 56);
                eng_barrier(); if (*dead) { alive = false; break; }
                ENG_GSTAMP(10);
                {
                    eng_gather_x(rl, blog(par), layV, 0, V, tag, logS, gw, ENG_GW, dl, p.ctl, dead, 1000 + cb * 64 + 57);
                    sub.n = 0;
                    if (at == 0) *sub_count = *dead ? 1 : 0;
                    sub.sync(dl);
                    ENG_GSTAMP(11);
                    if (*reinterpret_cast<volatile int*>(sub_count) == 0) {
                        const int last = cb == p.ncb - 1;
                        const int nfv = pre.nfv;
                        EngSampLds S{redbuf, pen_id, pen_val, amv, ami, wcnt, prL, keyL, cut};
                        const int code = eng_sample_small(sp, pre, logS, S, sub, at, dl, gw,
                                                          p.stamps ? p.stamps + (((size_t)b * p.ncb + cb) * nL + nL - 1) * 16 : nullptr);
                        ENG_GSTAMP(14);
                        const int R = p.ncb + 1;
                        if (atid == 0) { codes_s[cb] = code; *sub_count = sub.n + 1; }
                        sub.sync(lane);
                        prev_code = code;
                        if (b == drawer(cb)) {
                            if (atid == 0) sp.tokn[cb + 1] = code;
                            if (last) {
                                const int frozen = sp.done[0];
                                if (atid < R) {
                                    const int v = atid < 2 ? sp.tokn[atid] : (atid - 1 == cb ? code : codes_s[atid - 1]);
                                    sp.tok[atid] = v;
                                    if (nfv < sp.cap && !frozen) sp.seq[(size_t)atid * sp.cap + nfv] = v;
                                }
                                if (atid == 0 && !frozen) {
                                    sp.pos[0] += 1;
                                    sp.nf[0] = nfv + 1;
                                    if (sp.tokn[0] == sp.im_end) sp.done[0] = 1;
                                }
                            }
                        }
                    }
                }
            }
        }
    }

    eng_barrier();
    if (tid == 0) {
        const unsigned old = atomicAdd(p.ctl + ENG_CTL_EXIT, 1u);
        if (old + 1 == (unsigned)nb) {
            __hip_atomic_store((eng_gu32*)(p.ctl + ENG_CTL_EXIT), 0u, ENG_RLX);
            __hip_atomic_store((eng_gu32*)(p.ctl + ENG_CTL_ARRIVED), 0u, ENG_RLX);
            for (int x = 0; x < 8; ++x) __hip_atomic_store((eng_gu32*)(p.ctl + ENG_CTL_XCD + x), 0u, ENG_RLX);
            __hip_atomic_store((eng_gu32*)(p.ctl + ENG_CTL_EPOCH), epoch + ENG_EPOCH_STEP, ENG_RLX);
        }
    }
}

}
```

Before: 787.3 tokens/s.

## Share slow-stack QKV and W13 rows across all eight waves of the frame engine

Adds a shared-rows variant of the slow-stack engine kernel, used by default for the S1 shape. The QKV rows are split across all waves, and the non-compute (gather) waves take part of the W13 SwiGLU pairs. Each wave then holds fewer prefetched rows and the GEMV phase work is spread more evenly. It also clamps the rows computed by the first units when certain nt bits are set, in both the slow and fast kernels. The cost is more register pressure and more complex arrival counting on the gather waves, and the gather waves' other duties may be delayed.

Result: no change. 790.2 tokens/s, median of 6 (+0.4%).

```diff
diff --git a/fish-tts_amd/csrc/engine.hip b/fish-tts_amd/csrc/engine.hip
--- a/fish-tts_amd/csrc/engine.hip
+++ b/fish-tts_amd/csrc/engine.hip
@@ -460,13 +460,15 @@
 typedef void (*eng_slow_fn_t)(SlowEngP);
 typedef void (*eng_fast_fn_t)(FastEngP);
 typedef void (*eng_qkv0_fn_t)(const bf16_t*, const bf16_t*, const bf16_t*, const bf16_t*, bf16_t*, int, int, int, float);
-struct EngSlowEntry { int D, H, HKV, HDIM, F, SQ, SF, SO; eng_slow_fn_t xl, plain; };
+struct EngSlowEntry { int D, H, HKV, HDIM, F, SQ, SF, SO; eng_slow_fn_t xl, plain, xl_sh, plain_sh; };
 struct EngFastEntry { int D, H, HKV, HDIM, F, V, SQ, SF, SO; eng_fast_fn_t loop; eng_qkv0_fn_t qkv0; eng_fast_fn_t resident; int resf, resl; };
-template <typename S, bool WITH_XL>
+template <typename S, bool WITH_XL, bool WITH_SH = false>
 static EngSlowEntry eng_slow_entry() {
-    eng_slow_fn_t xl = nullptr;
+    eng_slow_fn_t xl = nullptr, xl_sh = nullptr, plain_sh = nullptr;
     if constexpr (WITH_XL) xl = slow_engine_kernel<S, true>;
-    return EngSlowEntry{S::D, S::H, S::HKV, S::HDIM, S::F, S::SQ, S::SF, S::SO, xl, slow_engine_kernel<S, false>};
+    if constexpr (WITH_SH) plain_sh = slow_engine_kernel<S, false, true>;
+    if constexpr (WITH_SH && WITH_XL) xl_sh = slow_engine_kernel<S, true, true>;
+    return EngSlowEntry{S::D, S::H, S::HKV, S::HDIM, S::F, S::SQ, S::SF, S::SO, xl, slow_engine_kernel<S, false>, xl_sh, plain_sh};
 }
 template <typename S>
 static EngFastEntry eng_fast_entry() {
@@ -476,7 +478,7 @@
                         res, S::RESF, S::RESL};
 }
 static const EngSlowEntry* eng_slow_shapes(int* n) {
-    static const EngSlowEntry tab[] = {eng_slow_entry<EngSlowS1, true>(), eng_slow_entry<EngSlowShape<1024, 16, 8, 128, 4096>, true>(),
+    static const EngSlowEntry tab[] = {eng_slow_entry<EngSlowS1, true, true>(), eng_slow_entry<EngSlowShape<1024, 16, 8, 128, 4096>, true>(),
                                        eng_slow_entry<EngSlowShape<1024, 16, 4, 128, 3072>, false>()};
     *n = (int)(sizeof tab / sizeof tab[0]);
     return tab;
@@ -568,13 +570,18 @@
     if (ctx->eng_lds_slow > lds_cap) { why = "the slow stack's LDS need exceeds the CU's"; return false; }
     ctx->eng_xl = ctx->xl_shape && nb == 256 && ctx->nsplit_max == 32 && c.n_local_heads * 32 == nb;
     ctx->eng_xl = ctx->eng_xl && se->xl != nullptr;
-    ctx->eng_slow_fn = (const void*)(ctx->eng_xl ? se->xl : se->plain);
+    const eng_slow_fn_t slow_sh_fn = ctx->eng_xl ? se->xl_sh : se->plain_sh;
+    const bool slow_sh = slow_sh_fn != nullptr && getenv("FT_NO_SHARED_ROWS") == nullptr;
+    const std::string sh_note = slow_sh ? "; slow stack: QKV and W13 rows shared out over all eight waves" :
+                                slow_sh_fn == nullptr ? "; slow stack: rows on the compute waves (no shared-rows form for this shape class)" :
+                                "; slow stack: rows on the compute waves (FT_NO_SHARED_ROWS is set)";
+    ctx->eng_slow_fn = (const void*)(slow_sh ? slow_sh_fn : ctx->eng_xl ? se->xl : se->plain);
     const void* slow_fn = ctx->eng_slow_fn;
     if (!hip_ok(hipFuncSetAttribute(slow_fn, hipFuncAttributeMaxDynamicSharedMemorySize, (int)ctx->eng_lds_slow),
                 "hipFuncSetAttribute(slow_engine_kernel)")) return false;
     if (!eng_fits_cu(slow_fn, ctx->eng_lds_slow, lds_cap, "slow-stack", why)) return false;
     ctx->eng_on = true;
-    why = ctx->eng_xl ? "slow stack on the frame engine (one kv head per XCD)" : "slow stack on the frame engine";
+    why = (ctx->eng_xl ? "slow stack on the frame engine (one kv head per XCD)" : "slow stack on the frame engine") + sh_note;
 
     const int HDf = c.fast_n_head * c.fast_head_dim;
     const int fqkvN = (c.fast_n_head + 2 * c.fast_n_local_heads) * c.fast_head_dim;
@@ -640,7 +647,7 @@
         }
     }
     ctx->eng_fast_on = true;
-    why = ctx->eng_xl ? "slow stack (one kv head per XCD) and codebook loop on the frame engine" : "slow stack and codebook loop on the frame engine";
+    why = (ctx->eng_xl ? "slow stack (one kv head per XCD) and codebook loop on the frame engine" : "slow stack and codebook loop on the frame engine") + sh_note;
     {
         char buf[160];
         if (fast_res)
diff --git a/fish-tts_amd/csrc/frame_engine.h b/fish-tts_amd/csrc/frame_engine.h
--- a/fish-tts_amd/csrc/frame_engine.h
+++ b/fish-tts_amd/csrc/frame_engine.h
@@ -361,12 +361,12 @@
             }
 }
 
-template <bool NTL = true, int NT, int RPU, int MAXS, typename RM = EngRowIdent>
+template <bool NTL = true, int WS = ENG_CW, int NT, int RPU, int MAXS, typename RM = EngRowIdent>
 __device__ __forceinline__ void eng_issue(EngW<NT, RPU, MAXS>& r, const bf16_t* W, const bf16_t* gain, int K, int u_lo, int u_hi,
                                           int cw, int lane, int nt, RM rm = RM()) {
 #pragma unroll
     for (int s = 0; s < MAXS; ++s) {
-        int u = u_lo + cw + s * ENG_CW;
+        int u = u_lo + cw + s * WS;
         u = u < u_hi ? u : u_hi - 1;
 #pragma unroll
         for (int rr = 0; rr < RPU; ++rr)
@@ -389,7 +389,7 @@
 constexpr int ENG_MAX_OUT = 64;
 typedef __attribute__((address_space(3))) int* eng_lds_int;
 
-template <int NT, int RPU, int MAXS, int PRO, int EPI, typename RM = EngRowIdent>
+template <int NT, int RPU, int MAXS, int PRO, int EPI, typename RM = EngRowIdent, int WS = ENG_CW>
 __device__ __forceinline__ void eng_gemv_rows(const EngW<NT, RPU, MAXS>& r, const float* xs, int K, float eps, const bf16_t* bias,
                                               const float* resid, float* vals, int u_lo, int u_hi, int cw, int lane, RM rm = RM()) {
     static_assert(EPI == EPI_SWIGLU ? RPU == 2 : RPU == 1, "a unit is a (w1, w3) pair for SwiGLU, one row otherwise");
@@ -420,7 +420,7 @@
         }
 #pragma unroll
         for (int s = 0; s < MAXS; ++s) {
-            const int u = u_lo + cw + s * ENG_CW;
+            const int u = u_lo + cw + s * WS;
             if (u >= u_hi) break;
             float acc[RPU];
 #pragma unroll
@@ -460,26 +460,26 @@
     __hip_atomic_store((eng_gu64*)(g + i), ((unsigned long long)tag32 << 32) | __float_as_uint(v), __ATOMIC_RELAXED, __HIP_MEMORY_SCOPE_WORKGROUP);
 }
 
-template <int NT, int MAXS, typename RM>
+template <int NT, int MAXS, int ARR = ENG_CW, int WS = ENG_CW, typename RM>
 __device__ __forceinline__ void eng_gemv_qkv_local(const EngW<NT, 1, MAXS>& r, const float* xs, int K, float eps, const bf16_t* bias,
-                                                   unsigned* gvec, unsigned tag, int n, int cw, int lane, EngOut& eo, RM rm) {
-    eng_gemv_rows<NT, 1, MAXS, PRO_RMSNORM, EPI_STORE>(r, xs, K, eps, bias, nullptr, eo.vals, 0, n, cw, lane, rm);
+                                                   unsigned* gvec, unsigned tag, int n, int nr, int cw, int lane, EngOut& eo, RM rm) {
+    eng_gemv_rows<NT, 1, MAXS, PRO_RMSNORM, EPI_STORE, RM, WS>(r, xs, K, eps, bias, nullptr, eo.vals, 0, nr, cw, lane, rm);
     __builtin_amdgcn_fence(__ATOMIC_RELEASE, "workgroup", "local");
     int old = 0;
     if (lane == 0) old = __hip_atomic_fetch_add((eng_lds_int)eo.count, 1, __ATOMIC_RELAXED, __HIP_MEMORY_SCOPE_WORKGROUP);
     old = __builtin_amdgcn_readfirstlane(old);
     eo.seq += 1;
-    if (old + 1 == eo.seq * ENG_CW) {
+    if (old + 1 == eo.seq * ARR) {
         __builtin_amdgcn_fence(__ATOMIC_ACQUIRE, "workgroup", "local");
         if (lane < n) eng_put_local(gvec, rm(lane), eo.vals[lane], tag);
     }
 }
 
-template <int NT, int RPU, int MAXS, int PRO, int EPI, bool PK3 = false, int ARR = ENG_CW>
+template <int NT, int RPU, int MAXS, int PRO, int EPI, bool PK3 = false, int ARR = ENG_CW, int WS = ENG_CW>
 __device__ __forceinline__ void eng_gemv_part(const EngW<NT, RPU, MAXS>& r, const float* xs, int K, float eps, const bf16_t* bias,
                                               const float* resid, unsigned* gout, unsigned tag, float* plain, int u_lo, int u_hi,
                                               int r_lo, int r_hi, int cw, int lane, EngOut& eo) {
-    eng_gemv_rows<NT, RPU, MAXS, PRO, EPI>(r, xs, K, eps, bias, resid, eo.vals + (r_lo - u_lo), r_lo, r_hi, cw, lane);
+    eng_gemv_rows<NT, RPU, MAXS, PRO, EPI, EngRowIdent, WS>(r, xs, K, eps, bias, resid, eo.vals + (r_lo - u_lo), r_lo, r_hi, cw, lane);
     __builtin_amdgcn_fence(__ATOMIC_RELEASE, "workgroup", "local");
     int old = 0;
     if (lane == 0) old = __hip_atomic_fetch_add((eng_lds_int)eo.count, 1, __ATOMIC_RELAXED, __HIP_MEMORY_SCOPE_WORKGROUP);
@@ -658,10 +658,14 @@
     return a < natt ? a : -1;
 }
 
-template <typename S, bool XL = false>
+template <typename S, bool XL = false, bool SH = false>
 __global__ __launch_bounds__(ENG_THREADS) void slow_engine_kernel(SlowEngP p) {
     constexpr int NTD = S::NTD, NTA = S::NTA, NTF = S::NTF, G = S::G;
     constexpr int SQ = S::SQ, SF = S::SF, SO = S::SO;
+    static_assert(!SH || (S::QKVN / ENG_NB == 2 * ENG_WAVES && S::F / ENG_NB == 3 * ENG_CW), "shared row phases: 16 QKV rows and 12 W13 pairs per workgroup");
+    constexpr int SQC = SH ? SQ / 2 : SQ, WSQ = SH ? ENG_WAVES : ENG_CW;
+    constexpr int SFC = SH ? 2 : SF;
+    constexpr int ARRS = SH ? ENG_WAVES : ENG_CW;
     extern __shared__ __attribute__((aligned(16))) float smem[];
     const int tid = threadIdx.x, lane = tid & 63, wave = __builtin_amdgcn_readfirstlane(tid >> 6);
     const int b = blockIdx.x;
@@ -686,8 +690,9 @@
     float* outS = mscr + 64 * 6;
     int* dead = reinterpret_cast<int*>(outS + ENG_MAX_OUT);
     int* out_count = dead + 1;
+    int* sh_count = dead + 2;
     int* reg_s = dead + 4;
-    if (tid == 0) { *dead = eng_fault_here(p.ctl, 0u, b) ? 1 : 0; *out_count = 0; }
+    if (tid == 0) { *dead = eng_fault_here(p.ctl, 0u, b) ? 1 : 0; *out_count = 0; *sh_count = 0; }
     if (tid == ENG_CW * 64) {
         reg_s[0] = 0; reg_s[1] = 0; reg_s[2] = 1;
         if (XL || p.rep_stride) eng_register(p.ctl, nb, reg_s, dead);
@@ -707,7 +712,7 @@
     const int nsplit = XL ? nb / Hkv : p.nsplit;
     const int natt = Hkv * nsplit;
     const int chunk = (pos + nsplit) / nsplit;
-    const int grp = lane / LPP, gl = lane % LPP;
+    int grp = lane / LPP, gl = lane % LPP;
 
     {
         const int* tk = p.toks;
@@ -739,23 +744,30 @@
         }
     }
 
+    int q_lo, q_hi, f_lo, f_hi;
+    eng_units(QKVN, b, nb, q_lo, q_hi);
+    if (XL) { q_lo = 0; q_hi = QKVN / nb; }
+    eng_units(F, b, nb, f_lo, f_hi);
+    const int f_c_hi = SH ? f_hi - ENG_GW : f_hi;
+    const int f_t_hi = (!SH && (p.nt & 4)) ? min(f_hi, f_lo + 2 * ENG_CW) : f_c_hi;
+    const int q_t_hi = (!SH && (p.nt & 8)) ? min(q_hi, q_lo + 2 * ENG_CW) : q_hi;
+
     if (wave < ENG_CW) {
-        int q_lo, q_hi, o_lo, o_hi, f_lo, f_hi, d_lo, d_hi;
-        eng_units(QKVN, b, nb, q_lo, q_hi);
-        if (XL) { q_lo = 0; q_hi = QKVN / nb; }
+        int o_lo, o_hi, d_lo, d_hi;
         eng_units(D, b, nb, o_lo, o_hi);
-        eng_units(F, b, nb, f_lo, f_hi);
         eng_units(D, b, nb, d_lo, d_hi);
-        EngW<NTD, 1, SQ> wq;
+        EngW<NTD, 1, SQC> wq;
         EngW<NTA, 1, SO> wo;
-        EngW<NTD, 2, SF> wf;
+        EngW<NTD, 2, SFC> wf;
         EngW<NTF, 1, SO> wd;
         EngOut eo{outS, out_count, 0};
+        EngOut es{outS, sh_count, 0};
+        EngOut& eoS = SH ? es : eo;
         {
             const EngLayer l0 = eng_layer(p.layers, 0);
-            if (!XL) eng_issue(wq, l0.wqkv, l0.attn_norm, D, q_lo, q_hi, cw, lane, p.nt);
+            if (!XL) eng_issue<true, WSQ>(wq, l0.wqkv, l0.attn_norm, D, q_lo, q_hi, cw, lane, p.nt);
             eng_issue(wo, l0.wo, (const bf16_t*)nullptr, HD, o_lo, o_hi, cw, lane, p.nt);
-            eng_issue(wf, l0.w13, l0.ffn_norm, D, f_lo, f_hi, cw, lane, p.nt);
+            eng_issue(wf, l0.w13, l0.ffn_norm, D, f_lo, f_c_hi, cw, lane, p.nt);
             eng_issue(wd, l0.w2, (const bf16_t*)nullptr, F, d_lo, d_hi, cw, lane, p.nt);
             __builtin_amdgcn_sched_barrier(0);
         }
@@ -765,7 +777,7 @@
                              (H + Hkv + reg_s[0]) * hd + reg_s[1] * xnk, xnq, xnk};
         if (XL) {
             const EngLayer l0 = eng_layer(p.layers, 0);
-            eng_issue(wq, l0.wqkv, l0.attn_norm, D, q_lo, q_hi, cw, lane, p.nt, rmq);
+            eng_issue<true, WSQ>(wq, l0.wqkv, l0.attn_norm, D, q_lo, q_hi, cw, lane, p.nt, rmq);
             __builtin_amdgcn_sched_barrier(0);
         }
         eng_barrier();
@@ -779,15 +791,15 @@
             if (li > 0) { eng_barrier(); if (*dead) break; }
             ENG_STAMP(0);
             if (XL)
-                eng_gemv_qkv_local<NTD, SQ>(wq, xA, D, p.eps, l.bqkv, p.gqkv + (size_t)par * VSTR, tag, q_hi, cw, lane, eo, rmq);
+                eng_gemv_qkv_local<NTD, SQC, ARRS, WSQ>(wq, xA, D, p.eps, l.bqkv, p.gqkv + (size_t)par * VSTR, tag, q_hi, q_t_hi, cw, lane, eoS, rmq);
             else
-                eng_gemv<NTD, 1, SQ, PRO_RMSNORM, EPI_STORE>(wq, xA, D, p.eps, l.bqkv, nullptr, p.gqkv + (size_t)par * VSTR + eng_pub(b, q_lo), tag, nullptr,
-                                                             q_lo, q_hi, cw, lane, eo);
+                eng_gemv_part<NTD, 1, SQC, PRO_RMSNORM, EPI_STORE, false, ARRS, WSQ>(wq, xA, D, p.eps, l.bqkv, nullptr, p.gqkv + (size_t)par * VSTR + eng_pub(b, q_lo),
+                                                                                     tag, nullptr, q_lo, q_hi, q_lo, q_t_hi, cw, lane, eoS);
             __builtin_amdgcn_sched_barrier(0);
             ENG_STAMP(1);
             if (more) {
-                if (XL) eng_issue(wq, ln.wqkv, ln.attn_norm, D, q_lo, q_hi, cw, lane, p.nt, rmq);
-                else eng_issue(wq, ln.wqkv, ln.attn_norm, D, q_lo, q_hi, cw, lane, p.nt);
+                if (XL) eng_issue<true, WSQ>(wq, ln.wqkv, ln.attn_norm, D, q_lo, q_hi, cw, lane, p.nt, rmq);
+                else eng_issue<true, WSQ>(wq, ln.wqkv, ln.attn_norm, D, q_lo, q_hi, cw, lane, p.nt);
             }
             __builtin_amdgcn_sched_barrier(0);
             if (XL || eng_att_role(b, nb, li, natt) >= 0) {
@@ -806,11 +818,12 @@
             __builtin_amdgcn_sched_barrier(0);
             eng_barrier(); if (*dead) break;
             ENG_STAMP(5);
-            eng_gemv<NTD, 2, SF, PRO_RMSNORM, EPI_SWIGLU, S::PK3>(wf, xB, D, p.eps, nullptr, nullptr,
-                                                                   p.gg + (size_t)par * VSTR + (S::PK3 ? 0 : eng_pub(b, f_lo)), tag, nullptr, f_lo, f_hi, cw, lane, eo);
+            eng_gemv_part<NTD, 2, SFC, PRO_RMSNORM, EPI_SWIGLU, S::PK3, ARRS>(wf, xB, D, p.eps, nullptr, nullptr,
+                                                                               p.gg + (size_t)par * VSTR + (S::PK3 ? 0 : eng_pub(b, f_lo)), tag, nullptr,
+                                                                               f_lo, f_hi, f_lo, f_t_hi, cw, lane, eoS);
             __builtin_amdgcn_sched_barrier(0);
             ENG_STAMP(6);
-            if (more) eng_issue(wf, ln.w13, ln.ffn_norm, D, f_lo, f_hi, cw, lane, p.nt);
+            if (more) eng_issue(wf, ln.w13, ln.ffn_norm, D, f_lo, f_c_hi, cw, lane, p.nt);
             __builtin_amdgcn_sched_barrier(0);
             eng_barrier(); if (*dead) break;
             ENG_STAMP(7);
@@ -872,10 +885,23 @@
                 }
             }
         };
-        if (!XL) { kv_plan(0); kv_issue(); }
+        EngW<NTD, 1, SH ? SQC : 1> gq;
+        EngW<NTD, 2, 1> gf;
+        EngOut es{outS, sh_count, 0};
+        if (!XL) {
+            if constexpr (SH) eng_issue<true, WSQ>(gq, eng_layer(p.layers, 0).wqkv, eng_layer(p.layers, 0).attn_norm, D, q_lo, q_hi, wave, lane, p.nt);
+            kv_plan(0); kv_issue();
+        }
         eng_barrier();
         const EngRelay rl{p.rep_stride != 0, reg_s[1], reg_s[2], p.rep_delta0 + (long)reg_s[0] * p.rep_stride};
-        if (XL) { x_role = reg_s[0] * nsplit + reg_s[1]; kv_plan(0); kv_issue(); }
+        const int xnq = G * hd * Hkv / nb, xnk = hd * Hkv / nb;
+        const EngRowQkvX rmq{reg_s[0] * G * hd + reg_s[1] * xnq, (H + reg_s[0]) * hd + reg_s[1] * xnk,
+                             (H + Hkv + reg_s[0]) * hd + reg_s[1] * xnk, xnq, xnk};
+        if (XL) {
+            if constexpr (SH) eng_issue<true, WSQ>(gq, eng_layer(p.layers, 0).wqkv, eng_layer(p.layers, 0).attn_norm, D, q_lo, q_hi, wave, lane, p.nt, rmq);
+            x_role = reg_s[0] * nsplit + reg_s[1]; kv_plan(0); kv_issue();
+        }
+        __builtin_amdgcn_sched_barrier(0);
         float rope_c = 1.f, rope_s = 0.f;
         if (lane < hp) { rope_c = p.rope[((size_t)pos * hp + lane) * 2]; rope_s = p.rope[((size_t)pos * hp + lane) * 2 + 1]; }
         eng_barrier();
@@ -886,6 +912,23 @@
             if (li > 0) {
                 eng_gather_x(rl, p.gx + (size_t)par * VSTR, layD, 0, D, tag, xA, gw, ENG_GW, lane, p.ctl, dead, li * 8 + 0);
                 eng_barrier(); if (*dead) break;
+            }
+            const bool more = li + 1 < p.n_layer;
+            int rl_ = lane;
+            auto gq_issue = [&]() {
+                if (!more) return;
+                const EngLayer ln = eng_layer(p.layers, li + 1);
+                if (XL) eng_issue<true, WSQ>(gq, ln.wqkv, ln.attn_norm, D, q_lo, q_hi, wave, rl_, p.nt, rmq);
+                else eng_issue<true, WSQ>(gq, ln.wqkv, ln.attn_norm, D, q_lo, q_hi, wave, rl_, p.nt);
+            };
+            if constexpr (SH) asm volatile("" : "+v"(rl_), "+v"(grp), "+v"(gl));
+            if constexpr (SH) {
+                if (XL)
+                    eng_gemv_qkv_local<NTD, SQC, ARRS, WSQ>(gq, xA, D, p.eps, l.bqkv, p.gqkv + (size_t)par * VSTR, tag, q_hi, q_hi, wave, rl_, es, rmq);
+                else
+                    eng_gemv_part<NTD, 1, SQC, PRO_RMSNORM, EPI_STORE, false, ARRS, WSQ>(gq, xA, D, p.eps, l.bqkv, nullptr, p.gqkv + (size_t)par * VSTR + eng_pub(b, q_lo),
+                                                                                         tag, nullptr, q_lo, q_hi, q_lo, q_hi, wave, rl_, es);
+                __builtin_amdgcn_sched_barrier(0);
             }
             const int a = role(li);
             if (a >= 0) {
@@ -1201,6 +1244,11 @@
             }
             eng_barrier(); if (*dead) break;
             if (a >= 0) kv_issue();
+            if constexpr (SH) {
+                asm volatile("" : "+v"(rl_));
+                eng_issue(gf, l.w13, l.ffn_norm, D, f_c_hi, f_hi, gw, rl_, p.nt);
+                __builtin_amdgcn_sched_barrier(0);
+            }
             const unsigned long long t_poll0 = p.stamps ? eng_rt() : 0ull;
             eng_gather_x(rl, p.gxb + (size_t)par * VSTR, layD, 0, D, tag, xB, gw, ENG_GW, lane, p.ctl, dead, li * 8 + 4, EngIdent(),
                        (p.stamps && gw == 0) ? p.stamps + ((size_t)b * p.n_layer + li) * 16 + 13 : nullptr);
@@ -1210,9 +1258,16 @@
                 unsigned long long* q = p.stamps + ((size_t)b * p.n_layer + li) * 16;
                 q[10] = t_poll0; q[11] = t_poll1; q[12] = eng_rt();
             }
+            if constexpr (SH) {
+                eng_gemv_part<NTD, 2, 1, PRO_RMSNORM, EPI_SWIGLU, S::PK3, ARRS>(gf, xB, D, p.eps, nullptr, nullptr,
+                                                                             p.gg + (size_t)par * VSTR + (S::PK3 ? 0 : eng_pub(b, f_lo)), tag, nullptr,
+                                                                             f_lo, f_hi, f_c_hi, f_hi, gw, rl_, es);
+                __builtin_amdgcn_sched_barrier(0);
+            }
             if constexpr (S::PK3) eng_gather3_x(rl, p.gg + (size_t)par * VSTR, F, tag, gS, gw, ENG_GW, lane, p.ctl, dead, li * 8 + 5);
             else eng_gather_x(rl, p.gg + (size_t)par * VSTR, layF, 0, F, tag, gS, gw, ENG_GW, lane, p.ctl, dead, li * 8 + 5);
             eng_barrier(); if (*dead) break;
+            if constexpr (SH) { gq_issue(); __builtin_amdgcn_sched_barrier(0); }
         }
     }
 
@@ -1828,6 +1883,7 @@
     int f_lo, f_hi;
     eng_units(F, b, nb, f_lo, f_hi);
     const int f_c_hi = f_hi - FRES;
+    const int f_t_hi = (p.nt & 4) ? min(f_c_hi, f_lo + 2 * ENG_CW) : f_c_hi;
     EngW<NTD, 2, (RF ? RF : 1)> res[RL ? RL : 1];
     if (p.stamps && tid == 0) p.stamps[(size_t)b * p.ncb * p.n_layer * 16 + 15] = eng_rt();
     if (tid == 0) { *dead = eng_fault_here(p.ctl, ENG_FAULT_FAST, b) ? 1 : 0; *out_count = 0; *sub_count = 0; dead[3] = 0; }
@@ -1853,6 +1909,7 @@
         eng_units(QKVN, b, nb, q_lo, q_hi);
         eng_units(D, b, nb, o_lo, o_hi);
         eng_units(V, b, nb, h_lo, h_hi);
+        const int q_t_hi = (p.nt & 8) ? min(q_hi, q_lo + ENG_CW) : q_hi;
         EngW<NTD, 1, SQ> wq;
         EngW<NTA, 1, SO> wo;
         EngW<NTD, 2, SFC> wf;
@@ -1899,8 +1956,8 @@
                 bf16_t* vL = kvS + (size_t)(li * 2 + 1) * p.ncb * KVW;
                 eng_barrier(); if (*dead) { alive = false; break; }
                 ENG_FSTAMP(0);
-                eng_gemv2<NTD, 1, SQ, PRO_RMSNORM, EPI_STORE>(wq, xA, xA1, D, p.eps, l.bqkv, nullptr, nullptr, bq(0, li) + eng_pub(b, q_lo),
-                                                              bq(1, li) + eng_pub(b, q_lo), tag0, tag1, q_lo, q_hi, cw, lane, eo);
+                eng_gemv2_part<NTD, 1, SQ, PRO_RMSNORM, EPI_STORE>(wq, xA, xA1, D, p.eps, l.bqkv, nullptr, nullptr, bq(0, li) + eng_pub(b, q_lo),
+                                                                   bq(1, li) + eng_pub(b, q_lo), tag0, tag1, q_lo, q_hi, q_lo, q_t_hi, cw, lane, eo);
                 __builtin_amdgcn_sched_barrier(0);
                 ENG_FSTAMP(1);
                 if (more && !(li == nL - 1 && p.qkv0_tab != nullptr)) eng_issue<false>(wq, ln.wqkv, ln.attn_norm, D, q_lo, q_hi, cw, lane, p.nt);
@@ -1927,10 +1984,10 @@
                 ENG_FSTAMP(5);
                 if (tail0)
                     eng_gemv2_part<NTD, 2, SFC, PRO_RMSNORM, EPI_SWIGLU, ARRF>(wf, xB, xB1, D, p.eps, nullptr, nullptr, nullptr, bg(0, li) + eng_pub(b, f_lo),
-                                                                               bg(1, li) + eng_pub(b, f_lo), tag0, tag1, f_lo, f_hi, f_lo, f_c_hi, cw, lane, eoF);
+                                                                               bg(1, li) + eng_pub(b, f_lo), tag0, tag1, f_lo, f_hi, f_lo, f_t_hi, cw, lane, eoF);
                 else
                     eng_gemv_part<NTD, 2, SFC, PRO_RMSNORM, EPI_SWIGLU, FS::PK3, ARRF>(wf, xB1, D, p.eps, nullptr, nullptr, bg(1, li) + (FS::PK3 ? 0 : eng_pub(b, f_lo)), tag1, nullptr,
-                                                                                f_lo, f_hi, f_lo, f_c_hi, cw, lane, eoF);
+                                                                                f_lo, f_hi, f_lo, f_t_hi, cw, lane, eoF);
                 __builtin_amdgcn_sched_barrier(0);
                 ENG_FSTAMP(6);
                 if (more) eng_issue<false>(wf, ln.w13, ln.ffn_norm, D, f_lo, f_c_hi, cw, lane, p.nt);
@@ -1978,8 +2035,8 @@
                 eng_barrier(); if (*dead) { alive = false; break; }
                 ENG_FSTAMP(0);
                 if (!(li == 0 && tab0))
-                    eng_gemv<NTD, 1, SQ, PRO_RMSNORM, EPI_STORE>(wq, xA, D, p.eps, l.bqkv, nullptr, bq(par, li) + eng_pub(b, q_lo), tag,
-                                                                 nullptr, q_lo, q_hi, cw, lane, eo);
+                    eng_gemv_part<NTD, 1, SQ, PRO_RMSNORM, EPI_STORE>(wq, xA, D, p.eps, l.bqkv, nullptr, bq(par, li) + eng_pub(b, q_lo), tag,
+                                                                      nullptr, q_lo, q_hi, q_lo, q_t_hi, cw, lane, eo);
                 __builtin_amdgcn_sched_barrier(0);
                 ENG_FSTAMP(1);
                 if (more && !(li == nL - 1 && p.qkv0_tab != nullptr && cb + 1 >= 2))
@@ -2001,7 +2058,7 @@
                 eng_barrier(); if (*dead) { alive = false; break; }
                 ENG_FSTAMP(5);
                 eng_gemv_part<NTD, 2, SFC, PRO_RMSNORM, EPI_SWIGLU, FS::PK3, ARRF>(wf, xB, D, p.eps, nullptr, nullptr, bg(par, li) + (FS::PK3 ? 0 : eng_pub(b, f_lo)), tag, nullptr,
-                                                                            f_lo, f_hi, f_lo, f_c_hi, cw, lane, eoF);
+                                                                            f_lo, f_hi, f_lo, f_t_hi, cw, lane, eoF);
                 __builtin_amdgcn_sched_barrier(0);
                 ENG_FSTAMP(6);
                 if (more) eng_issue<false>(wf, ln.w13, ln.ffn_norm, D, f_lo, f_c_hi, cw, lane, p.nt);
```
